# kolyangg/open-universe

Measured on AMD Instinct MI355X. Metric: sec-audio enhanced/sec/GPU + xRT, UNIVERSE++ 16 kHz 8 s clips @1/2/4/8 GPU, higher is better.
Workload: dtype f32 (conv operands split into f16 hi/lo: 3 f16 MFMA passes, f32 accumulation)

## Files before the change

### include/ouhip.h

```cpp
#ifndef OUHIP_H
#define OUHIP_H

#include <stddef.h>
#include <stdint.h>

#ifdef __cplusplus
extern "C" {
#endif

#define OUHIP_ABI_VERSION 10

int ou_abi_version(void);
const char* ou_last_error(void);


#define OU_TILE_SHAPE_MASK 0xff
#define OU_TILE_TPW_SHIFT 8
#define OU_TILE_TPW_MASK (3 << 8)
#define OU_TILE_WS (1 << 10)
#define OU_TILE_SPLIT_QUERY (1 << 11)
#define OU_TILE_KS_SHIFT 12
#define OU_TILE_KS_MASK (3 << 12)
#define OU_TILE_RS (1 << 14)
#define OU_TILE_SS (1 << 15)
#define OU_TILE_MMAJOR (1 << 16)
#define OU_TILE_FIR (1 << 17)
#define OU_TILE_FIR_EARLY (1 << 8)
#define OU_TILE_FIR_DEEP (1 << 9)
#define OU_TILE_RS_DIAG_SHIFT 8
#define OU_TILE_RS_DIAG_MASK (3 << 8)

typedef struct ou_conv_desc {
    const float* x;
    int64_t x_bstride;
    int64_t x_cstride;
    int32_t cin;
    int32_t in_len;
    int32_t frame;
    int32_t shift;
    const float* in_scale;
    float slope;
    const float* w;
    int32_t m;
    int32_t kt;
    int32_t pad;
    int32_t cc;
    int32_t n_frames;
    int32_t batch;
    float* y;
    int64_t y_bstride, y_cstride;
    int32_t rout;
    int32_t out_len;
    int32_t valid_len;
    const float* bias;
    const float* res1;
    int64_t r1_bstride, r1_cstride;
    float s1;
    const float* film;
    int64_t film_bstride;
    const float* res2;
    int64_t r2_bstride, r2_cstride;
    float s2;
    int32_t tile;
    int32_t prec;
    float w_unscale;
    int32_t f0;
    int32_t* status;
    float* ks_ws;
    int64_t ks_ws_bytes;
    uint16_t* sy;
    int64_t sy_bstride;
    int32_t sy_rows;
    int32_t sy_shift;
    float sy_slope;
    int32_t sy_pad_;
    const uint16_t* xs;
    int64_t xs_bstride;
    int32_t xs_rows;
    int32_t xs_shift;
    int32_t fir;
    int32_t fir_pad_;
    const float* fir_taps;
} ou_conv_desc;

int ou_conv_chunk(int kt, int frame);
int64_t ou_conv_packed_size(int m, int cin_eff, int kt, int cc);
int ou_conv_pack(const float* w_logical, int m, int cin_eff, int kt, int cc,
                 float* packed);
int ou_conv_pack_split(const float* w_logical, int m, int cin_eff, int kt,
                       float* packed, float* w_unscale);
int ou_conv_pack_split_nat(const float* w_logical, int m, int cin_eff, int kt,
                           float* packed, float* w_unscale);
int ou_conv(const ou_conv_desc* d, void* stream);
int ou_conv_pick_tile(const ou_conv_desc* d);
int ou_conv_num_tiles(void);
int ou_conv_tile_ok(int kt, int tile);
int ou_conv_lds_info(int kt, int tile, int* lds_request, int* device_optin_max);

typedef struct ou_gru_desc {
    const float* gi;
    int64_t gi_bstride;
    const float* w_hh;
    const float* b_hh;
    float* y;
    int64_t y_bstride, y_cstride;
    const float* res;
    int64_t res_bstride, res_cstride;
    float res_scale;
    int32_t hidden;
    int32_t steps;
    int32_t batch;
    int32_t flags;
    uint64_t* granules;
    int32_t* status;
    int32_t t_begin, t_end;
    float* hstate;
    int32_t ws_zeroed;
    int32_t _pad;
} ou_gru_desc;

int64_t ou_gru_workspace_bytes(int hidden, int batch);
int ou_gru_ks_max_workgroups(void);
int ou_gru(const ou_gru_desc* d, void* stream);

typedef struct ou_embed_desc {
    const float* sigma;
    int32_t n;
    int32_t kind;
    int32_t dim;
    float te_weight, te_bias;
    const float* rff_freq;
    int32_t n_rff;
    int32_t rows;
    const float* mlp_w[3];
    const float* mlp_b[3];
    float mlp_slope[3];
    const float* w;
    const float* bias;
    float* out;
    float* gbuf;
} ou_embed_desc;

int ou_embed(const ou_embed_desc* d, void* stream);

typedef struct ou_head_desc {
    const float* h;
    int64_t h_bstride;
    int32_t channels, length, batch, mode;
    float slope1, slope2;
    const float* w;
    float bias;
    int32_t edm, _pad;
    float w_skip, w_out, s2, c_score, c_noise, s_next;
    const float* x;
    const float* z;
    float* out;
} ou_head_desc;

int ou_head(const ou_head_desc* d, void* stream);

int ou_normalize(const float* x, float* y, int batch, int64_t n, float level,
                 float eps, void* stream);
int ou_inv_rms(const float* x, float* out, int batch, int64_t n, float denom,
               float eps, void* stream);
int ou_rms(const float* x, float* out, int batch, int64_t n, void* stream);
int ou_power(const float* x, float* y, int batch, int nf, int frames, void* stream);
int ou_pad(const float* x, int64_t x_bstride, float* y, int batch, int n_in,
           int n_out, int left, void* stream);
int ou_scale(const float* z, float* y, int64_t n, float scale, const float* add,
             void* stream);
int ou_finish(const float* x, int64_t x_bstride, int left, float* y, int batch,
              int len, const float* mix_rms, void* stream);
int ou_ensemble_reduce(const float* x, float* y, int ensemble, int64_t n,
                       int mode , void* stream);
int ou_signal_median(const float* x, float* y, int ensemble, int batch, int64_t n, int* counts,
                     void* stream);

int ou_resample(const float* x, int64_t x_bstride, float* y, int64_t y_bstride, int batch, int n_in,
                int n_out, const float* kernel, int phases, int taps, int orig, int width, void* stream);

int ou_flac_info(const uint8_t* data, int64_t n, int32_t* sample_rate, int32_t* channels,
                 int32_t* bits_per_sample, int64_t* frames);
int64_t ou_flac_decode(const uint8_t* data, int64_t n, float* out, int64_t frames);
int64_t ou_flac_encode_bound(int channels, int64_t frames, int bps);
int64_t ou_flac_encode(const float* x, int channels, int64_t frames, int sample_rate, int bps, uint8_t* out,
                       int64_t capacity);

typedef struct ou_snake_desc {
    const float* h;
    int64_t h_bstride;
    int32_t channels, length, batch, _pad0;
    const float* alpha;
    const float* k_up;
    int32_t taps_up, width_up;
    const float* k_down;
    int32_t taps_down, width_down;
    float* out;
} ou_snake_desc;

int ou_snake_aa(const ou_snake_desc* d, void* stream);

typedef struct ou_block_desc {
    const float* h;
    int64_t h_bstride, h_cstride;
    int32_t channels, length;
    int32_t batch, prec;
    const void* w[3];
    const float* bias[3];
    float slope[3];
    float w_unscale[3];
    const float* sc;
    int64_t sc_bstride, sc_cstride;
    float s_sc;
    int32_t dbg;
    const float* film;
    int64_t film_bstride;
    float* cond_out;
    int64_t co_bstride, co_cstride;
    float* y;
    int64_t y_bstride, y_cstride;
    float s_res, s2;
    const float* res2;
    int64_t r2_bstride, r2_cstride;
    int32_t* status;
    const float* x;
    int64_t x_bstride;
    const float* in_scale;
    const float* w_in;
    const float* b_in;
    ou_head_desc head;
    const void* w_down;
    const float* b_down;
    float slope_down, w_down_unscale;
    int32_t rate, down_kt;
    float* e;
    int64_t e_bstride, e_cstride;
    int32_t f0, f1;
    int32_t h0, h1;
    int32_t shift[4];
    uint16_t* sy;
    int64_t sy_bstride;
    int32_t sy_rows, sy_shift;
    float sy_slope;
    int32_t sy_pad_;
    const uint16_t* xs;
    int64_t xs_bstride;
    int32_t xs_rows, xs_pad_;
} ou_block_desc;

int ou_block_supported(int channels, int prec);
int ou_block_frames(int channels);
int64_t ou_block_packed_halves(int channels, int kt);
int ou_block_pack(const float* w, int channels, int kt, void* out, float* w_unscale);
int ou_block_pack_rect(const float* w, int m, int channels, int kt, void* out, float* w_unscale);
int64_t ou_block_packed_f32(int channels, int kt);
int ou_block_pack_f32(const float* w, int channels, int kt, float* out, float* w_unscale);
int ou_block_down_supported(int channels, int rate, int kt, int prec);
int ou_block(const ou_block_desc* d, void* stream);

typedef struct ou_program ou_program;

enum {
    OU_OP_CONV = 1, OU_OP_GRU = 2, OU_OP_EMBED = 3, OU_OP_HEAD = 4,
    OU_OP_NORMALIZE = 5, OU_OP_INV_RMS = 6, OU_OP_POWER = 7, OU_OP_PAD = 8,
    OU_OP_SCALE = 9, OU_OP_FINISH = 10, OU_OP_RMS = 11, OU_OP_SNAKE = 12,
    OU_OP_MEMSET = 13, OU_OP_ENSEMBLE = 14, OU_OP_BLOCK = 15,
    OU_OP_LANE = 16, OU_OP_SIGNAL = 17, OU_OP_WAIT = 18
};

typedef struct ou_memset_desc {
    void* ptr;
    int64_t bytes;
} ou_memset_desc;
typedef struct ou_norm_args {
    const float* x;
    float* y;
    int32_t batch, _pad;
    int64_t n;
    float level, eps;
} ou_norm_args;
typedef struct ou_rms_args {
    const float* x;
    float* out;
    int32_t batch, _pad;
    int64_t n;
    float denom, eps;
} ou_rms_args;
typedef struct ou_power_args {
    const float* x;
    float* y;
    int32_t batch, nf, frames, _pad;
} ou_power_args;
typedef struct ou_pad_args {
    const float* x;
    int64_t x_bstride;
    float* y;
    int32_t batch, n_in, n_out, left;
} ou_pad_args;
typedef struct ou_scale_args {
    const float* z;
    float* y;
    int64_t n;
    float scale, _pad;
    const float* add;
} ou_scale_args;
typedef struct ou_finish_args {
    const float* x;
    int64_t x_bstride;
    int32_t left, batch, len, _pad;
    float* y;
    const float* mix_rms;
} ou_finish_args;
typedef struct ou_sync_args {
    int32_t id;
    int32_t _pad;
} ou_sync_args;
typedef struct ou_ensemble_args {
    const float* x;
    float* y;
    int32_t ensemble, mode;
    int64_t n;
    int32_t batch, _pad;
    int32_t* counts;
} ou_ensemble_args;

ou_program* ou_program_create(void);
void ou_program_destroy(ou_program* p);
int ou_program_add(ou_program* p, int op, const void* desc, size_t desc_bytes);
int ou_program_patch(ou_program* p, int index, int op, const void* desc, size_t desc_bytes);
int ou_program_size(const ou_program* p);
int ou_program_run(ou_program* p, void* stream);
int ou_program_capture(ou_program* p);
int ou_program_validate(const ou_program* p);
int ou_program_capture_segments(ou_program* p);
int ou_program_launch(ou_program* p, void* stream);
int ou_program_op_kind(const ou_program* p, int i);
int ou_program_profile(ou_program* p, void* stream, float* ms);
int ou_program_trace(ou_program* p, void* stream, float* t0, float* t1);

int ou_randn(float* out, int64_t n, uint64_t seed, uint64_t offset, void* stream);
int ou_philox4x32(const uint32_t ctr[4], const uint32_t key[2], uint32_t out[4]);

typedef struct ou_bundle ou_bundle;
typedef struct ou_model ou_model;

typedef struct ou_bundle_io {
    int32_t region;
    int32_t count;
    int64_t offset;
    int32_t batch;
    int32_t length;
} ou_bundle_io;

typedef struct ou_bundle_meta {
    ou_bundle_io mix;
    ou_bundle_io noise;
    ou_bundle_io out;
    ou_bundle_io status;
    int32_t n_regions, n_ops;
    int64_t region_bytes;
    const char* json;
    int64_t json_bytes;
    char arch[16];
} ou_bundle_meta;

int ou_bundle_open(const char* path, ou_bundle** out);
void ou_bundle_close(ou_bundle* b);
int ou_bundle_info(const ou_bundle* b, ou_bundle_meta* meta);
int ou_bundle_region(const ou_bundle* b, int i, int32_t* kind, int64_t* bytes, const void** data);
int ou_bundle_op(const ou_bundle* b, int i, int32_t* kind, int64_t* desc_bytes, const char** label);
int ou_bundle_materialize(const ou_bundle* b, const uint64_t* region_bases, int op, void* desc_out);

int ou_bundle_load(const char* path, int capture, ou_model** out);
int ou_model_enhance_noise(ou_model* m, const float* mix, const float* noise, float* out, void* stream);
int ou_model_enhance(ou_model* m, const float* mix, float* out, uint64_t seed, uint64_t offset, void* stream);
int ou_model_status(ou_model* m);
int ou_model_info(const ou_model* m, ou_bundle_meta* meta);
void ou_model_destroy(ou_model* m);

int ou_long_windows(int64_t T, int window, int overlap, int64_t* n, int64_t* last_start);
int ou_long_fade(int overlap, float* fade );
int ou_window_gather(const float* x, int64_t x_rstride, int rows, int64_t T, int window, int overlap,
                     int64_t first, int count, int64_t win, float* y, int64_t y_rstride, int64_t y_bstride,
                     void* stream);
int ou_overlap_add(const float* w, int64_t w_bstride, int64_t T, int window, int overlap, int64_t first,
                   int count, const float* fade, float* y, void* stream);

typedef struct ou_pool_clip {
    const float* x;
    const float* noise;
    float* y;
    int64_t T, noise_rstride;
} ou_pool_clip;
int ou_pool_slots(const int64_t* T, int n_clips, int window, int overlap, int64_t* n_slots);
int ou_pool_gather(const ou_pool_clip* clips, int n_clips, int window, int overlap, int64_t first, int count,
                   int noise_rows, int64_t noise_win, float* mix, int64_t mix_bstride,
                   float* nz, int64_t nz_rstride, int64_t nz_bstride, void* stream);
int ou_pool_overlap_add(const ou_pool_clip* clips, int n_clips, int window, int overlap, int64_t first, int count,
                        const float* w, int64_t w_bstride, const float* fade, void* stream);

int64_t ou_model_long_noise(const ou_model* m, int64_t n, int overlap, int64_t* len);
int ou_model_enhance_long_noise(ou_model* m, const float* x, int64_t n, int overlap, const float* noise,
                                float* out, void* stream);
int ou_model_enhance_long(ou_model* m, const float* x, int64_t n, int overlap, float* out, uint64_t seed,
                          uint64_t offset, float* workspace, void* stream);

#ifdef __cplusplus
}
#endif
#endif
```

### open_universe_amd/_lib.py

```python
import ctypes
import os
from ctypes import POINTER, c_char, c_char_p, c_float, c_int, c_int32, c_int64, c_size_t, c_uint32, c_uint64, c_void_p

_HERE = os.path.dirname(os.path.abspath(__file__))
LIB_PATH = os.environ.get("OUHIP_LIB", os.path.join(_HERE, "libouhip.so"))
ABI_VERSION = 10

fp = c_void_p

OP_CONV, OP_GRU, OP_EMBED, OP_HEAD = 1, 2, 3, 4
OP_NORMALIZE, OP_INV_RMS, OP_POWER, OP_PAD = 5, 6, 7, 8
OP_SCALE, OP_FINISH, OP_RMS, OP_SNAKE = 9, 10, 11, 12
OP_MEMSET, OP_ENSEMBLE, OP_BLOCK = 13, 14, 15
OP_LANE, OP_SIGNAL, OP_WAIT = 16, 17, 18


class ConvDesc(ctypes.Structure):
    _fields_ = [
        ("x", fp), ("x_bstride", c_int64), ("x_cstride", c_int64),
        ("cin", c_int32), ("in_len", c_int32), ("frame", c_int32), ("shift", c_int32),
        ("in_scale", fp), ("slope", c_float), ("w", fp),
        ("m", c_int32), ("kt", c_int32), ("pad", c_int32), ("cc", c_int32),
        ("n_frames", c_int32), ("batch", c_int32),
        ("y", fp), ("y_bstride", c_int64), ("y_cstride", c_int64),
        ("rout", c_int32), ("out_len", c_int32), ("valid_len", c_int32),
        ("bias", fp),
        ("res1", fp), ("r1_bstride", c_int64), ("r1_cstride", c_int64), ("s1", c_float),
        ("film", fp), ("film_bstride", c_int64),
        ("res2", fp), ("r2_bstride", c_int64), ("r2_cstride", c_int64), ("s2", c_float),
        ("tile", c_int32), ("prec", c_int32), ("w_unscale", c_float), ("f0", c_int32),
        ("status", fp), ("ks_ws", fp), ("ks_ws_bytes", c_int64),
        ("sy", fp), ("sy_bstride", c_int64), ("sy_rows", c_int32), ("sy_shift", c_int32),
        ("sy_slope", c_float), ("sy_pad_", c_int32),
        ("xs", fp), ("xs_bstride", c_int64), ("xs_rows", c_int32), ("xs_shift", c_int32),
        ("fir", c_int32), ("fir_pad_", c_int32), ("fir_taps", fp),
    ]


class GruDesc(ctypes.Structure):
    _fields_ = [
        ("gi", fp), ("gi_bstride", c_int64), ("w_hh", fp), ("b_hh", fp),
        ("y", fp), ("y_bstride", c_int64), ("y_cstride", c_int64),
        ("res", fp), ("res_bstride", c_int64), ("res_cstride", c_int64),
        ("res_scale", c_float), ("hidden", c_int32), ("steps", c_int32), ("batch", c_int32),
        ("flags", c_int32), ("granules", fp), ("status", fp), ("t_begin", c_int32), ("t_end", c_int32),
        ("hstate", fp), ("ws_zeroed", c_int32), ("_pad", c_int32),
    ]


class EmbedDesc(ctypes.Structure):
    _fields_ = [
        ("sigma", fp), ("n", c_int32), ("kind", c_int32), ("dim", c_int32),
        ("te_weight", c_float), ("te_bias", c_float), ("rff_freq", fp), ("n_rff", c_int32),
        ("rows", c_int32), ("mlp_w", fp * 3), ("mlp_b", fp * 3), ("mlp_slope", c_float * 3),
        ("w", fp), ("bias", fp), ("out", fp), ("gbuf", fp),
    ]


class HeadDesc(ctypes.Structure):
    _fields_ = [
        ("h", fp), ("h_bstride", c_int64),
        ("channels", c_int32), ("length", c_int32), ("batch", c_int32), ("mode", c_int32),
        ("slope1", c_float), ("slope2", c_float), ("w", fp), ("bias", c_float),
        ("edm", c_int32), ("_pad", c_int32),
        ("w_skip", c_float), ("w_out", c_float), ("s2", c_float), ("c_score", c_float),
        ("c_noise", c_float), ("s_next", c_float),
        ("x", fp), ("z", fp), ("out", fp),
    ]


class SnakeDesc(ctypes.Structure):
    _fields_ = [
        ("h", fp), ("h_bstride", c_int64),
        ("channels", c_int32), ("length", c_int32), ("batch", c_int32), ("_pad0", c_int32),
        ("alpha", fp), ("k_up", fp), ("taps_up", c_int32), ("width_up", c_int32),
        ("k_down", fp), ("taps_down", c_int32), ("width_down", c_int32), ("out", fp),
    ]


class SyncArgs(ctypes.Structure):
    _fields_ = [("id", c_int32), ("_pad", c_int32)]


class MemsetArgs(ctypes.Structure):
    _fields_ = [("ptr", fp), ("bytes", c_int64)]


class NormArgs(ctypes.Structure):
    _fields_ = [("x", fp), ("y", fp), ("batch", c_int32), ("_pad", c_int32), ("n", c_int64),
                ("level", c_float), ("eps", c_float)]


class RmsArgs(ctypes.Structure):
    _fields_ = [("x", fp), ("out", fp), ("batch", c_int32), ("_pad", c_int32), ("n", c_int64),
                ("denom", c_float), ("eps", c_float)]


class PowerArgs(ctypes.Structure):
    _fields_ = [("x", fp), ("y", fp), ("batch", c_int32), ("nf", c_int32),
                ("frames", c_int32), ("_pad", c_int32)]


class PadArgs(ctypes.Structure):
    _fields_ = [("x", fp), ("x_bstride", c_int64), ("y", fp), ("batch", c_int32),
                ("n_in", c_int32), ("n_out", c_int32), ("left", c_int32)]


class ScaleArgs(ctypes.Structure):
    _fields_ = [("z", fp), ("y", fp), ("n", c_int64), ("scale", c_float), ("_pad", c_float),
                ("add", fp)]


class FinishArgs(ctypes.Structure):
    _fields_ = [("x", fp), ("x_bstride", c_int64), ("left", c_int32), ("batch", c_int32),
                ("len", c_int32), ("_pad", c_int32), ("y", fp), ("mix_rms", fp)]


class EnsembleArgs(ctypes.Structure):
    _fields_ = [("x", fp), ("y", fp), ("ensemble", c_int32), ("mode", c_int32), ("n", c_int64),
                ("batch", c_int32), ("_pad", c_int32), ("counts", c_void_p)]


class BlockDesc(ctypes.Structure):
    _fields_ = [
        ("h", fp), ("h_bstride", c_int64), ("h_cstride", c_int64),
        ("channels", c_int32), ("length", c_int32), ("batch", c_int32), ("prec", c_int32),
        ("w", fp * 3), ("bias", fp * 3), ("slope", c_float * 3), ("w_unscale", c_float * 3),
        ("sc", fp), ("sc_bstride", c_int64), ("sc_cstride", c_int64), ("s_sc", c_float), ("dbg", c_int32),
        ("film", fp), ("film_bstride", c_int64),
        ("cond_out", fp), ("co_bstride", c_int64), ("co_cstride", c_int64),
        ("y", fp), ("y_bstride", c_int64), ("y_cstride", c_int64), ("s_res", c_float), ("s2", c_float),
        ("res2", fp), ("r2_bstride", c_int64), ("r2_cstride", c_int64),
        ("status", fp),
        ("x", fp), ("x_bstride", c_int64), ("in_scale", fp), ("w_in", fp), ("b_in", fp),
        ("head", HeadDesc),
        ("w_down", fp), ("b_down", fp), ("slope_down", c_float), ("w_down_unscale", c_float),
        ("rate", c_int32), ("down_kt", c_int32), ("e", fp), ("e_bstride", c_int64), ("e_cstride", c_int64),
        ("f0", c_int32), ("f1", c_int32), ("h0", c_int32), ("h1", c_int32),
        ("shift", c_int32 * 4),
        ("sy", fp), ("sy_bstride", c_int64), ("sy_rows", c_int32), ("sy_shift", c_int32),
        ("sy_slope", c_float), ("sy_pad_", c_int32),
        ("xs", fp), ("xs_bstride", c_int64), ("xs_rows", c_int32), ("xs_pad_", c_int32),
    ]


class BundleIo(ctypes.Structure):
    _fields_ = [("region", c_int32), ("count", c_int32), ("offset", c_int64),
                ("batch", c_int32), ("length", c_int32)]


class BundleMeta(ctypes.Structure):
    _fields_ = [("mix", BundleIo), ("noise", BundleIo), ("out", BundleIo), ("status", BundleIo),
                ("n_regions", c_int32), ("n_ops", c_int32), ("region_bytes", c_int64),
                ("json", c_char_p), ("json_bytes", c_int64), ("arch", c_char * 16)]


class PoolClip(ctypes.Structure):
    _fields_ = [("x", fp), ("noise", fp), ("y", fp), ("T", c_int64), ("noise_rstride", c_int64)]


OP_STRUCT = {
    OP_CONV: ConvDesc, OP_GRU: GruDesc, OP_EMBED: EmbedDesc, OP_HEAD: HeadDesc,
    OP_NORMALIZE: NormArgs, OP_INV_RMS: RmsArgs, OP_RMS: RmsArgs, OP_POWER: PowerArgs,
    OP_PAD: PadArgs, OP_SCALE: ScaleArgs, OP_FINISH: FinishArgs, OP_SNAKE: SnakeDesc,
    OP_MEMSET: MemsetArgs, OP_ENSEMBLE: EnsembleArgs, OP_BLOCK: BlockDesc,
    OP_LANE: SyncArgs, OP_SIGNAL: SyncArgs, OP_WAIT: SyncArgs,
}

EXPORTS = {
    "ou_abi_version": (c_int, []),
    "ou_last_error": (ctypes.c_char_p, []),
    "ou_conv_chunk": (c_int, [c_int, c_int]),
    "ou_conv_packed_size": (c_int64, [c_int, c_int, c_int, c_int]),
    "ou_conv_pack": (c_int, [POINTER(c_float), c_int, c_int, c_int, c_int, POINTER(c_float)]),
    "ou_conv_pack_split": (c_int, [POINTER(c_float), c_int, c_int, c_int, POINTER(c_float),
                                   POINTER(c_float)]),
    "ou_conv_pack_split_nat": (c_int, [POINTER(c_float), c_int, c_int, c_int, POINTER(c_float),
                                       POINTER(c_float)]),
    "ou_conv": (c_int, [POINTER(ConvDesc), c_void_p]),
    "ou_conv_pick_tile": (c_int, [POINTER(ConvDesc)]),
    "ou_conv_num_tiles": (c_int, []),
    "ou_conv_tile_ok": (c_int, [c_int, c_int]),
    "ou_conv_lds_info": (c_int, [c_int, c_int, POINTER(c_int), POINTER(c_int)]),
    "ou_gru_workspace_bytes": (c_int64, [c_int, c_int]),
    "ou_gru_ks_max_workgroups": (c_int, []),
    "ou_gru": (c_int, [POINTER(GruDesc), c_void_p]),
    "ou_embed": (c_int, [POINTER(EmbedDesc), c_void_p]),
    "ou_head": (c_int, [POINTER(HeadDesc), c_void_p]),
    "ou_normalize": (c_int, [fp, fp, c_int, c_int64, c_float, c_float, c_void_p]),
    "ou_inv_rms": (c_int, [fp, fp, c_int, c_int64, c_float, c_float, c_void_p]),
    "ou_rms": (c_int, [fp, fp, c_int, c_int64, c_void_p]),
    "ou_power": (c_int, [fp, fp, c_int, c_int, c_int, c_void_p]),
    "ou_pad": (c_int, [fp, c_int64, fp, c_int, c_int, c_int, c_int, c_void_p]),
    "ou_scale": (c_int, [fp, fp, c_int64, c_float, fp, c_void_p]),
    "ou_finish": (c_int, [fp, c_int64, c_int, fp, c_int, c_int, fp, c_void_p]),
    "ou_ensemble_reduce": (c_int, [fp, fp, c_int, c_int64, c_int, c_void_p]),
    "ou_signal_median": (c_int, [fp, fp, c_int, c_int, c_int64, c_void_p, c_void_p]),
    "ou_snake_aa": (c_int, [POINTER(SnakeDesc), c_void_p]),
    "ou_block_supported": (c_int, [c_int, c_int]),
    "ou_block_frames": (c_int, [c_int]),
    "ou_block_packed_halves": (c_int64, [c_int, c_int]),
    "ou_block_pack": (c_int, [POINTER(c_float), c_int, c_int, c_void_p, POINTER(c_float)]),
    "ou_block_packed_f32": (c_int64, [c_int, c_int]),
    "ou_block_pack_f32": (c_int, [POINTER(c_float), c_int, c_int, POINTER(c_float), POINTER(c_float)]),
    "ou_block_pack_rect": (c_int, [POINTER(c_float), c_int, c_int, c_int, c_void_p, POINTER(c_float)]),
    "ou_block_down_supported": (c_int, [c_int, c_int, c_int, c_int]),
    "ou_block": (c_int, [POINTER(BlockDesc), c_void_p]),
    "ou_resample": (c_int, [fp, c_int64, fp, c_int64, c_int, c_int, c_int, fp, c_int, c_int, c_int, c_int,
                            c_void_p]),
    "ou_flac_info": (c_int, [c_void_p, c_int64, POINTER(c_int32), POINTER(c_int32), POINTER(c_int32),
                             POINTER(c_int64)]),
    "ou_flac_decode": (c_int64, [c_void_p, c_int64, c_void_p, c_int64]),
    "ou_flac_encode_bound": (c_int64, [c_int, c_int64, c_int]),
    "ou_flac_encode": (c_int64, [c_void_p, c_int, c_int64, c_int, c_int, c_void_p, c_int64]),
    "ou_program_create": (c_void_p, []),
    "ou_program_destroy": (None, [c_void_p]),
    "ou_program_add": (c_int, [c_void_p, c_int, c_void_p, c_size_t]),
    "ou_program_patch": (c_int, [c_void_p, c_int, c_int, c_void_p, c_size_t]),
    "ou_program_size": (c_int, [c_void_p]),
    "ou_program_run": (c_int, [c_void_p, c_void_p]),
    "ou_program_capture": (c_int, [c_void_p]),
    "ou_program_capture_segments": (c_int, [c_void_p]),
    "ou_program_validate": (c_int, [c_void_p]),
    "ou_program_launch": (c_int, [c_void_p, c_void_p]),
    "ou_program_op_kind": (c_int, [c_void_p, c_int]),
    "ou_program_profile": (c_int, [c_void_p, c_void_p, POINTER(c_float)]),
    "ou_program_trace": (c_int, [c_void_p, c_void_p, POINTER(c_float), POINTER(c_float)]),
    "ou_randn": (c_int, [fp, c_int64, c_uint64, c_uint64, c_void_p]),
    "ou_philox4x32": (c_int, [POINTER(c_uint32), POINTER(c_uint32), POINTER(c_uint32)]),
    "ou_bundle_open": (c_int, [c_char_p, POINTER(c_void_p)]),
    "ou_bundle_close": (None, [c_void_p]),
    "ou_bundle_info": (c_int, [c_void_p, POINTER(BundleMeta)]),
    "ou_bundle_region": (c_int, [c_void_p, c_int, POINTER(c_int32), POINTER(c_int64), POINTER(c_void_p)]),
    "ou_bundle_op": (c_int, [c_void_p, c_int, POINTER(c_int32), POINTER(c_int64), POINTER(c_char_p)]),
    "ou_bundle_materialize": (c_int, [c_void_p, POINTER(c_uint64), c_int, c_void_p]),
    "ou_bundle_load": (c_int, [c_char_p, c_int, POINTER(c_void_p)]),
    "ou_model_enhance_noise": (c_int, [c_void_p, fp, fp, fp, c_void_p]),
    "ou_model_enhance": (c_int, [c_void_p, fp, fp, c_uint64, c_uint64, c_void_p]),
    "ou_model_status": (c_int, [c_void_p]),
    "ou_model_info": (c_int, [c_void_p, POINTER(BundleMeta)]),
    "ou_model_destroy": (None, [c_void_p]),
    "ou_long_windows": (c_int, [c_int64, c_int, c_int, POINTER(c_int64), POINTER(c_int64)]),
    "ou_long_fade": (c_int, [c_int, POINTER(c_float)]),
    "ou_window_gather": (c_int, [fp, c_int64, c_int, c_int64, c_int, c_int, c_int64, c_int, c_int64, fp, c_int64,
                                 c_int64, c_void_p]),
    "ou_overlap_add": (c_int, [fp, c_int64, c_int64, c_int, c_int, c_int64, c_int, fp, fp, c_void_p]),
    "ou_pool_slots": (c_int, [POINTER(c_int64), c_int, c_int, c_int, POINTER(c_int64)]),
    "ou_pool_gather": (c_int, [POINTER(PoolClip), c_int, c_int, c_int, c_int64, c_int, c_int, c_int64, fp, c_int64,
                               fp, c_int64, c_int64, c_void_p]),
    "ou_pool_overlap_add": (c_int, [POINTER(PoolClip), c_int, c_int, c_int, c_int64, c_int, fp, c_int64, fp,
                                    c_void_p]),
    "ou_model_long_noise": (c_int64, [c_void_p, c_int64, c_int, POINTER(c_int64)]),
    "ou_model_enhance_long_noise": (c_int, [c_void_p, fp, c_int64, c_int, fp, fp, c_void_p]),
    "ou_model_enhance_long": (c_int, [c_void_p, fp, c_int64, c_int, fp, c_uint64, c_uint64, fp, c_void_p]),
}

_lib = None


class OuHipError(RuntimeError):
    pass


class OuRangeError(OuHipError):
    flags = ()


def load():
    global _lib
    if _lib is not None:
        return _lib
    if not os.path.exists(LIB_PATH):
        raise OuHipError(
            f"{LIB_PATH} not found: build it with `python -c 'import __graft_entry__ as g; "
            "g.build()'` or open_universe_amd/csrc/build.sh")
    lib = ctypes.CDLL(LIB_PATH)
    for name, (res, args) in EXPORTS.items():
        f = getattr(lib, name)
        f.restype = res
        f.argtypes = args
    if lib.ou_abi_version() != ABI_VERSION:
        raise OuHipError("libouhip ABI version mismatch")
    _lib = lib
    return lib


def check(rc, what=""):
    if rc != 0:
        msg = load().ou_last_error()
        raise OuHipError(f"{what}: ouhip error {rc}: {msg.decode() if msg else ''}")


def conv_chunk(kt, frame):
    return load().ou_conv_chunk(kt, frame)


def conv_pack(w_logical, cc):
    import numpy as np

    w = np.ascontiguousarray(w_logical, dtype=np.float32)
    m, cin, kt = w.shape
    n = load().ou_conv_packed_size(m, cin, kt, cc)
    out = np.empty(n, dtype=np.float32)
    check(load().ou_conv_pack(w.ctypes.data_as(POINTER(c_float)), m, cin, kt, cc,
                              out.ctypes.data_as(POINTER(c_float))), "conv_pack")
    return out


def _split_scale(w):
    import numpy as np

    if not np.isfinite(w).all():
        raise OuHipError("split packing: non-finite weight")
    mx = float(np.abs(w).max()) if w.size else 0.0
    e = 0
    if mx > 0.0:
        e = min(100, max(-100, 10 - int(np.frexp(np.float32(mx))[1])))
    return np.float32(2.0**e), float(2.0 ** (6 - e))


def _hi_lo(a):
    import numpy as np

    hi = a.astype(np.float16)
    lo = ((a - hi.astype(np.float32)) * np.float32(2048.0)).astype(np.float16)
    return hi, lo


def conv_pack_split_np(w_logical):
    import numpy as np

    w = np.ascontiguousarray(w_logical, dtype=np.float32)
    m, cin, kt = w.shape
    sc, unscale = _split_scale(w)
    mt = (m + 31) // 32
    cpad = (cin + 63) // 64 * 64
    a = np.zeros((mt * 32, cpad, kt), dtype=np.float32)
    a[:m, :cin] = w * sc
    a = a.reshape(mt, 32, cpad // 16, 8, 2, kt).transpose(0, 2, 5, 4, 1, 3)
    hi, lo = _hi_lo(np.ascontiguousarray(a))
    out = np.stack([hi, lo], axis=2)
    return np.ascontiguousarray(out).reshape(-1).view(np.float32), unscale


def conv_pack_split_nat_np(w_logical):
    import numpy as np

    w = np.ascontiguousarray(w_logical, dtype=np.float32)
    m, cin, kt = w.shape
    sc, unscale = _split_scale(w)
    mt = (m + 31) // 32
    cpad = (cin + 63) // 64 * 64
    a = np.zeros((mt * 32, cpad, kt), dtype=np.float32)
    a[:m, :cin] = w * sc
    a = a.reshape(mt, 32, cpad // 16, 2, 8, kt).transpose(0, 2, 5, 3, 1, 4)
    hi, lo = _hi_lo(np.ascontiguousarray(a))
    out = np.stack([hi, lo], axis=2)
    return np.ascontiguousarray(out).reshape(-1).view(np.float32), unscale


def block_pack_np(w_logical):
    import numpy as np

    w = np.ascontiguousarray(w_logical, dtype=np.float32)
    m, c, kt = w.shape
    assert m % 32 == 0 and c % 16 == 0, w.shape
    sc, unscale = _split_scale(w)
    a = (w * sc).reshape(m // 32, 32, c // 16, 2, 8, kt).transpose(0, 5, 2, 3, 1, 4)
    hi, lo = _hi_lo(np.ascontiguousarray(a))
    out = np.stack([hi, lo], axis=3)
    return np.ascontiguousarray(out).reshape(-1).view(np.int16), unscale


def block_pack_f32_np(w_logical):
    import numpy as np

    w = np.ascontiguousarray(w_logical, dtype=np.float32)
    m, c, kt = w.shape
    assert m % 32 == 0 and c % 16 == 0, w.shape
    a = w.reshape(m // 32, 32, c // 8, 4, 2, kt).transpose(0, 5, 2, 4, 1, 3)
    return np.ascontiguousarray(a).reshape(-1), 64.0


def block_pack_f32(w_logical):
    import numpy as np

    w = np.ascontiguousarray(w_logical, dtype=np.float32)
    c, _, kt = w.shape
    out = np.empty(load().ou_block_packed_f32(c, kt), dtype=np.float32)
    un = c_float(0.0)
    check(load().ou_block_pack_f32(w.ctypes.data_as(POINTER(c_float)), c, kt, out.ctypes.data_as(POINTER(c_float)),
                                   ctypes.byref(un)), "block_pack_f32")
    return out, float(un.value)


def conv_pack_split(w_logical, natural=False):
    import numpy as np

    w = np.ascontiguousarray(w_logical, dtype=np.float32)
    m, cin, kt = w.shape
    n = load().ou_conv_packed_size(m, cin, kt, 0)
    out = np.empty(n, dtype=np.float32)
    un = c_float(0.0)
    fn = load().ou_conv_pack_split_nat if natural else load().ou_conv_pack_split
    check(fn(w.ctypes.data_as(POINTER(c_float)), m, cin, kt, out.ctypes.data_as(POINTER(c_float)),
             ctypes.byref(un)), "conv_pack_split")
    return out, float(un.value)


def block_pack(w_logical):
    import numpy as np

    w = np.ascontiguousarray(w_logical, dtype=np.float32)
    m, c, kt = w.shape
    out = np.empty(2 * m * c * kt, dtype=np.int16)
    un = c_float(0.0)
    check(load().ou_block_pack_rect(w.ctypes.data_as(POINTER(c_float)), m, c, kt, out.ctypes.data,
                                    ctypes.byref(un)), "block_pack")
    return out, float(un.value)


TILE_SHAPE_MASK = 0xff
TILE_TPW_SHIFT, TILE_TPW_MASK = 8, 3 << 8
TILE_WS = 1 << 10
TILE_SPLIT_QUERY = 1 << 11
TILE_KS_SHIFT, TILE_KS_MASK = 12, 3 << 12
TILE_RS = 1 << 14
TILE_SS = 1 << 15
TILE_MMAJOR = 1 << 16
TILE_FIR = 1 << 17
TILE_FIR_EARLY = 1 << 8
TILE_FIR_DEEP = 1 << 9
TILE_RS_DIAG_SHIFT, TILE_RS_DIAG_MASK = 8, 3 << 8
MAJ_BIT, SS_BIT, FIR_BIT = TILE_MMAJOR, TILE_SS, TILE_FIR

_MMAJOR = os.environ.get("OUHIP_MMAJOR", "1") != "0"
_MMAJOR_BYTES = float(os.environ.get("OUHIP_MMAJOR_MB", "128")) * 2**20


def mmajor_order(desc):
    multi = desc.tile & (TILE_TPW_MASK | TILE_WS) and not desc.tile & TILE_FIR
    if not _MMAJOR or multi:
        return False
    in_bytes = 4.0 * desc.batch * desc.cin * desc.frame * desc.n_frames
    return in_bytes > _MMAJOR_BYTES


TUNER = None


ADD_HOOK = None


class Program:

    def __init__(self):
        self.lib = load()
        self.h = self.lib.ou_program_create()
        self.keep = []
        self.cur_lane = 0
        self.captured = False
        self.flops = []
        self.bytes = []
        self.info = []
        self.lanes = []
        self.label = ""
        self.labels = []
        self.descs = []

    def add(self, op, desc):
        assert isinstance(desc, OP_STRUCT[op])
        if op == OP_LANE:
            self.cur_lane = desc.id
        if op in (OP_CONV, OP_BLOCK) and ADD_HOOK is not None:
            ADD_HOOK(self, op, desc)
        if op == OP_CONV and desc.tile < 0 and TUNER is not None:
            desc.tile = TUNER(desc)
        if op == OP_CONV and desc.tile >= 0 and mmajor_order(desc):
            desc.tile |= TILE_MMAJOR
        check(self.lib.ou_program_add(self.h, op, ctypes.byref(desc), ctypes.sizeof(desc)),
              f"program_add(op={op})")
        if ADD_HOOK is not None and hasattr(ADD_HOOK, "note"):
            ADD_HOOK.note(self, len(self.flops), op, desc)
        self.descs.append(desc)
        self.flops.append(float(getattr(desc, "_flops", 0.0)))
        self.bytes.append(float(getattr(desc, "_bytes", 0.0)))
        self.lanes.append(self.cur_lane)
        self.labels.append(self.label)
        if op == OP_CONV:
            self.info.append({"m": desc.m, "cin": desc.cin, "frame": desc.frame, "kt": desc.kt,
                              "n": desc.n_frames, "b": desc.batch, "rout": desc.rout,
                              "tile": desc.tile, "fir": desc.fir})
        elif op == OP_GRU:
            self.info.append({"H": desc.hidden, "T": desc.steps, "b": desc.batch})
        elif op == OP_BLOCK:
            self.info.append({"C": desc.channels, "n": desc.length, "b": desc.batch, "prec": desc.prec,
                              "rate": desc.rate if desc.e else 0, "head": bool(desc.head.w), "in": bool(desc.x)})
        else:
            self.info.append({})

    def lane(self, i):
        self.add(OP_LANE, SyncArgs(id=i))

    def new_event(self):
        self.n_events = getattr(self, "n_events", 0) + 1
        return self.n_events - 1

    def signal(self, ev=None):
        ev = self.new_event() if ev is None else ev
        self.add(OP_SIGNAL, SyncArgs(id=ev))
        return ev

    def wait(self, ev):
        self.add(OP_WAIT, SyncArgs(id=ev))

    def patch(self, index, op, desc):
        check(self.lib.ou_program_patch(self.h, index, op, ctypes.byref(desc), ctypes.sizeof(desc)),
              f"program_patch({index})")

    def __len__(self):
        return self.lib.ou_program_size(self.h)

    def run(self, stream):
        check(self.lib.ou_program_run(self.h, c_void_p(stream)), "program_run")

    def validate(self):
        check(self.lib.ou_program_validate(self.h), "program_validate")

    def capture(self, segments=None):
        import os

        if segments is None:
            segments = os.environ.get("OUHIP_GRAPH_MODE", "whole") == "seg"
        fn = self.lib.ou_program_capture_segments if segments else self.lib.ou_program_capture
        check(fn(self.h), "program_capture")
        self.captured = True

    def launch(self, stream):
        check(self.lib.ou_program_launch(self.h, c_void_p(stream)), "program_launch")

    def op_kinds(self):
        return [self.lib.ou_program_op_kind(self.h, i) for i in range(len(self))]

    def profile(self, stream):
        n = len(self)
        buf = (c_float * n)()
        check(self.lib.ou_program_profile(self.h, c_void_p(stream), buf), "program_profile")
        return list(buf)

    def trace(self, stream):
        n = len(self)
        a, b = (c_float * n)(), (c_float * n)()
        check(self.lib.ou_program_trace(self.h, c_void_p(stream), a, b), "program_trace")
        return [(x, y) if x >= 0 else None for x, y in zip(a, b)]

    def __del__(self):
        try:
            if self.h:
                self.lib.ou_program_destroy(self.h)
                self.h = None
        except Exception:
            pass


def run_now(op, desc, stream):
    lib = load()
    fns = {OP_CONV: lib.ou_conv, OP_GRU: lib.ou_gru, OP_EMBED: lib.ou_embed,
           OP_HEAD: lib.ou_head, OP_SNAKE: lib.ou_snake_aa, OP_BLOCK: lib.ou_block}
    check(fns[op](ctypes.byref(desc), c_void_p(stream)), f"op {op}")
```

### open_universe_amd/csrc/ou_block.hip

```cpp
#include <hip/hip_runtime.h>

#include <algorithm>
#include <cmath>
#include <type_traits>
#include <vector>

#include "../../include/ouhip.h"
#include "ou_common.h"

typedef float floatx16 __attribute__((ext_vector_type(16)));
typedef _Float16 half4_t __attribute__((ext_vector_type(4)));
typedef _Float16 half8_t __attribute__((ext_vector_type(8)));
typedef float f32x4_t __attribute__((ext_vector_type(4)));

namespace {

constexpr int kStageShift = 6;


#ifndef OU_BLOCK_NT32
#define OU_BLOCK_NT32 4
#endif
#ifndef OU_BLOCK_NT64
#define OU_BLOCK_NT64 2
#endif
#ifndef OU_BLOCK_NT128
#define OU_BLOCK_NT128 1
#endif
#ifndef OU_BLOCK_NT48
#define OU_BLOCK_NT48 4
#endif
#ifndef OU_BLOCK_NT96
#define OU_BLOCK_NT96 4
#endif
#ifndef OU_BLOCK_NT192
#define OU_BLOCK_NT192 2
#endif
#ifndef OU_BLOCK_RING1
#define OU_BLOCK_RING1 6
#endif
#ifndef OU_BLOCK_FENCE
#define OU_BLOCK_FENCE 1
#endif
#ifndef OU_BLOCK_BPIPE
#define OU_BLOCK_BPIPE 1
#endif
#ifndef OU_BLOCK_RING_EARLY
#define OU_BLOCK_RING_EARLY 0
#endif
#ifndef OU_BLOCK_HV_EARLY
#define OU_BLOCK_HV_EARLY 0
#endif

template <int C, int NT, int P>
struct BCfg {
    static constexpr int MT = (C + 31) / 32;
    static constexpr int WAVES = 4;
    static constexpr int NTH = 64 * WAVES;
    static constexpr int WM = MT % WAVES == 0 ? WAVES : MT % 2 == 0 ? 2 : 1;
    static constexpr int WN = WAVES / WM;
    static constexpr int MR = MT / WM;
    static constexpr int NR = NT / WN;
    static constexpr int NF = 32 * NT;
    static constexpr int F = NF - 4;
    using E = std::conditional_t<P == 0, float, _Float16>;
    static constexpr int SX = P == 0 ? C + 4 : C + 8;
    static constexpr int R1 = NF + 4;
    static constexpr int R2 = NF + 2;
    static constexpr int NPL = P == 1 ? 2 : 1;
    static constexpr int PA = R1 * SX;
    static constexpr int PB = R2 * SX;
    static constexpr int A_OFF = 0;
    static constexpr int B_OFF = NPL * PA;
    static constexpr int LDS_BYTES = (int)sizeof(E) * (NPL * PA + NPL * PB);
    static constexpr int KS = C / 16;
    static constexpr int RING = MR == 1 ? OU_BLOCK_RING1 : 4;
    static_assert(C % 16 == 0 && WM * WN == WAVES && MT % WM == 0 && NT % WN == 0, "block tiling");
    static_assert((SX * (int)sizeof(E) / 16) % 2 == 1 && (SX * (int)sizeof(E)) % 16 == 0,
                  "LDS row stride must be an odd number of 16-B slots");
};

__device__ __forceinline__ float prelu(float v, float a) { return v >= 0.f ? v : a * v; }

template <int KT, int C, int NT, int P>
__device__ __forceinline__ void ring_load(const half8_t* __restrict__ wp, int wm, int lane, int s,
                                          half8_t (&dst)[BCfg<C, NT, P>::MR][2])
{
    using K = BCfg<C, NT, P>;
    const int k = s / K::KS, ks = s - (s / K::KS) * K::KS;
#pragma unroll
    for (int mr = 0; mr < K::MR; ++mr) {
        const half8_t* p = wp + ((((int64_t)(wm * K::MR + mr) * KT + k) * K::KS + ks) * 2) * 64 + lane;
        dst[mr][0] = p[0];
        if constexpr (P == 1) dst[mr][1] = p[64];
    }
}
template <int KT, int C, int NT, int P>
__device__ __forceinline__ void ring_pro(const void* wp, int wm, int lane,
                                         half8_t (&ra)[BCfg<C, NT, P>::RING][BCfg<C, NT, P>::MR][2])
{
    using K = BCfg<C, NT, P>;
    constexpr int NS = KT * K::KS, D = NS < K::RING ? NS : K::RING;
#pragma unroll
    for (int s = 0; s < D - 1; ++s) ring_load<KT, C, NT, P>((const half8_t*)wp, wm, lane, s, ra[s]);
}

template <int KT, int C, int NT, int P>
__device__ __forceinline__ void stage_mma(const half8_t* __restrict__ wp, const _Float16* xin, int pstride, int wm,
                                          int wn, int lane, int dbg, floatx16 (&acc)[BCfg<C, NT, P>::MR][BCfg<C, NT, P>::NR],
                                          floatx16 (&accx)[BCfg<C, NT, P>::MR][BCfg<C, NT, P>::NR],
                                          half8_t (&ra)[BCfg<C, NT, P>::RING][BCfg<C, NT, P>::MR][2], bool pre)
{
    using K = BCfg<C, NT, P>;
    constexpr int MR = K::MR, NR = K::NR, KS = K::KS, NS = KT * KS;
    const int l32 = lane & 31, h = lane >> 5;
#pragma unroll
    for (int mr = 0; mr < MR; ++mr)
#pragma unroll
        for (int nr = 0; nr < NR; ++nr) {
#pragma unroll
            for (int r = 0; r < 16; ++r) acc[mr][nr][r] = 0.f, accx[mr][nr][r] = 0.f;
        }
    if (dbg & 2) return;
    constexpr int D = NS < K::RING ? NS : K::RING;
    auto load_a = [&](int s, half8_t (&dst)[MR][2]) { ring_load<KT, C, NT, P>(wp, wm, lane, s, dst); };
    if (!pre) {
#pragma unroll
        for (int s = 0; s < D - 1; ++s) load_a(s, ra[s]);
    }
    const _Float16* xb = xin + (wn * NR * 32 + l32) * K::SX + 8 * h;
    half8_t b[2][NR], bl[2][NR];
    auto load_b = [&](int s, half8_t (&bq)[NR], half8_t (&bo)[NR]) {
        const int k = s / KS, ks = s - (s / KS) * KS;
#pragma unroll
        for (int nr = 0; nr < NR; ++nr) {
            const _Float16* q = xb + (nr * 32 + k) * K::SX + 16 * ks;
            bq[nr] = *(const half8_t*)q;
            if constexpr (P == 1) bo[nr] = *(const half8_t*)(q + pstride);
        }
    };
    if constexpr (OU_BLOCK_BPIPE) load_b(0, b[0], bl[0]);
#pragma unroll
    for (int s = 0; s < NS; ++s) {
        if (s + D - 1 < NS) load_a(s + D - 1, ra[(s + D - 1) % D]);
        const int c = OU_BLOCK_BPIPE ? (s & 1) : 0;
        if constexpr (OU_BLOCK_BPIPE) {
            if (s + 1 < NS) load_b(s + 1, b[c ^ 1], bl[c ^ 1]);
        } else {
            load_b(s, b[0], bl[0]);
        }
        if constexpr (OU_BLOCK_FENCE) asm volatile("" ::: "memory");
#pragma unroll
        for (int mr = 0; mr < MR; ++mr)
#pragma unroll
            for (int nr = 0; nr < NR; ++nr) {
                acc[mr][nr] = __builtin_amdgcn_mfma_f32_32x32x16_f16(ra[s % D][mr][0], b[c][nr], acc[mr][nr], 0, 0, 0);
                if constexpr (P == 1) {
                    accx[mr][nr] =
                        __builtin_amdgcn_mfma_f32_32x32x16_f16(ra[s % D][mr][0], bl[c][nr], accx[mr][nr], 0, 0, 0);
                    accx[mr][nr] =
                        __builtin_amdgcn_mfma_f32_32x32x16_f16(ra[s % D][mr][1], b[c][nr], accx[mr][nr], 0, 0, 0);
                }
            }
    }
}

template <int C>
__device__ __forceinline__ int ch_pos(int c)
{
    return (c & 1) * (C / 2) + (c >> 1);
}

template <int KT, int C, int NT>
__device__ __forceinline__ void stage_mma_f32(const f32x4_t* __restrict__ wp, const float* xin, int wm, int wn,
                                              int lane, int dbg,
                                              floatx16 (&acc)[BCfg<C, NT, 0>::MR][BCfg<C, NT, 0>::NR])
{
    using K = BCfg<C, NT, 0>;
    constexpr int MR = K::MR, NR = K::NR, S4 = C / 8, NS = KT * S4;
    const int l32 = lane & 31, h = lane >> 5;
#pragma unroll
    for (int mr = 0; mr < MR; ++mr)
#pragma unroll
        for (int nr = 0; nr < NR; ++nr) {
#pragma unroll
            for (int r = 0; r < 16; ++r) acc[mr][nr][r] = 0.f;
        }
    if (dbg & 2) return;
    constexpr int D = NS < 4 ? NS : 4;
    f32x4_t ra[D][MR];
    auto load_a = [&](int s, f32x4_t (&dst)[MR]) {
        const int k = s / S4, s4 = s - (s / S4) * S4;
#pragma unroll
        for (int mr = 0; mr < MR; ++mr) dst[mr] = wp[(((int64_t)(wm * MR + mr) * KT + k) * S4 + s4) * 64 + lane];
    };
#pragma unroll
    for (int s = 0; s < D - 1; ++s) load_a(s, ra[s]);
    const float* xb = xin + (wn * NR * 32 + l32) * K::SX + h * (C / 2);
#pragma unroll
    for (int s = 0; s < NS; ++s) {
        if (s + D - 1 < NS) load_a(s + D - 1, ra[(s + D - 1) % D]);
        if constexpr (OU_BLOCK_FENCE) asm volatile("" ::: "memory");
        const int k = s / S4, s4 = s - (s / S4) * S4;
        f32x4_t bq[NR];
#pragma unroll
        for (int nr = 0; nr < NR; ++nr) bq[nr] = *(const f32x4_t*)(xb + (nr * 32 + k) * K::SX + 4 * s4);
#pragma unroll
        for (int j = 0; j < 4; ++j)
#pragma unroll
            for (int mr = 0; mr < MR; ++mr)
#pragma unroll
                for (int nr = 0; nr < NR; ++nr)
                    acc[mr][nr] = __builtin_amdgcn_mfma_f32_32x32x2f32(ra[s % D][mr][j], bq[nr][j], acc[mr][nr], 0, 0, 0);
    }
}

template <int KT, int C, int NT, int P>
__device__ __forceinline__ void run_stage(const void* w, const typename BCfg<C, NT, P>::E* xin, int pstride, int wm,
                                          int wn, int lane, int dbg,
                                          floatx16 (&acc)[BCfg<C, NT, P>::MR][BCfg<C, NT, P>::NR],
                                          floatx16 (&accx)[BCfg<C, NT, P>::MR][BCfg<C, NT, P>::NR],
                                          half8_t (&ra)[BCfg<C, NT, P>::RING][BCfg<C, NT, P>::MR][2], bool pre)
{
    if constexpr (P == 0) {
        stage_mma_f32<KT, C, NT>((const f32x4_t*)w, xin, wm, wn, lane, dbg, acc);
#pragma unroll
        for (int mr = 0; mr < BCfg<C, NT, P>::MR; ++mr)
#pragma unroll
            for (int nr = 0; nr < BCfg<C, NT, P>::NR; ++nr) accx[mr][nr] = floatx16{};
    } else {
        stage_mma<KT, C, NT, P>((const half8_t*)w, xin, pstride, wm, wn, lane, dbg, acc, accx, ra, pre);
    }
}

constexpr int kEpiFilm = 1, kEpiSc = 2, kEpiCond = 4, kEpiRes2 = 8;
constexpr int kEpiIn = 16, kEpiHead = 32;
constexpr int kEpiDown = 64;

template <int EPI, int R, int KF>
constexpr int block_off()
{
    return (EPI & kEpiHead) ? 1 : (EPI & kEpiDown) ? R * ((KF - 1) / 2) : 0;
}

template <int C, int NT, int P, int EPI, int R = 1, int KF = 1>
constexpr int block_f()
{
    if constexpr (EPI & kEpiDown) {
        constexpr int halo = 2 * R * ((KF - 1) / 2);
        return (BCfg<C, NT, P>::NF - 4 - halo) / R * R;
    }
    return BCfg<C, NT, P>::NF - 4 - ((EPI & kEpiHead) ? 2 : 0);
}

typedef float float2_t __attribute__((ext_vector_type(2)));
__device__ __forceinline__ float2_t fma2(float2_t a, float2_t b, float2_t c) { return __builtin_elementwise_fma(a, b, c); }
typedef _Float16 half2_t __attribute__((ext_vector_type(2)));

template <int P>
__device__ __forceinline__ void split4(float x0, float x1, float x2, float x3, half4_t& hi, half4_t& lo, float& omax)
{
    const float2_t a = {x0, x1}, b = {x2, x3};
    const half2_t ha = __builtin_convertvector(a, half2_t), hb = __builtin_convertvector(b, half2_t);
    hi = half4_t{ha[0], ha[1], hb[0], hb[1]};
    if constexpr (P == 1) {
        const half2_t la = __builtin_convertvector((a - __builtin_convertvector(ha, float2_t)) * 2048.f, half2_t);
        const half2_t lb = __builtin_convertvector((b - __builtin_convertvector(hb, float2_t)) * 2048.f, half2_t);
        lo = half4_t{la[0], la[1], lb[0], lb[1]};
    }
    const float m = __builtin_fmaxf(__builtin_fmaxf(__builtin_fabsf(x0), __builtin_fabsf(x1)),
                                    __builtin_fmaxf(__builtin_fabsf(x2), __builtin_fabsf(x3)));
    omax = __builtin_fmaxf(omax, m);
}

template <int C, int P, int R, int KF, int F, int SX>
__device__ __forceinline__ void down_stage(const ou_block_desc& d, const _Float16* xa, int pstride, int t0, int T,
                                           int TS, int b, int wave, int lane)
{
    constexpr int KT = KF * R, KS = C / 16, NS = KT * KS;
    constexpr int M4 = 2 * C / 32, NU = F / R, N4 = (NU + 31) / 32;
    constexpr int D = NS < 6 ? NS : 6;
    const int l32 = lane & 31, h = lane >> 5;
    const half8_t* wp = (const half8_t*)d.w_down;
    const int TE = (TS + R - 1) / R;
    const int e0 = t0 / R;
    const float un = d.w_down_unscale * ou_exp2i(d.shift[3] - kStageShift);
    for (int tile = wave; tile < M4 * N4; tile += 4) {
        const int m4 = tile % M4, n4 = tile / M4;
        const int u = n4 * 32 + l32;
        const _Float16* xb = xa + (u < NU ? u * R : 0) * SX + 8 * h;
        floatx16 acc, accx;
#pragma unroll
        for (int r = 0; r < 16; ++r) acc[r] = 0.f, accx[r] = 0.f;
        half8_t ra[D][2];
        auto load_a = [&](int s, half8_t (&dst)[2]) {
            const int k = s / KS, ks = s - (s / KS) * KS;
            const half8_t* p = wp + (((int64_t)(m4 * KT + k) * KS + ks) * 2) * 64 + lane;
            dst[0] = p[0];
            if constexpr (P == 1) dst[1] = p[64];
        };
#pragma unroll
        for (int s = 0; s < D - 1; ++s) load_a(s, ra[s]);
#pragma unroll
        for (int s = 0; s < NS; ++s) {
            if (s + D - 1 < NS) load_a(s + D - 1, ra[(s + D - 1) % D]);
            const int k = s / KS, ks = s - (s / KS) * KS;
            const _Float16* q = xb + k * SX + 16 * ks;
            const half8_t bq = *(const half8_t*)q;
            acc = __builtin_amdgcn_mfma_f32_32x32x16_f16(ra[s % D][0], bq, acc, 0, 0, 0);
            if constexpr (P == 1) {
                const half8_t bl = *(const half8_t*)(q + pstride);
                accx = __builtin_amdgcn_mfma_f32_32x32x16_f16(ra[s % D][0], bl, accx, 0, 0, 0);
                accx = __builtin_amdgcn_mfma_f32_32x32x16_f16(ra[s % D][1], bq, accx, 0, 0, 0);
            }
        }
        const int te = e0 + u;
        if (u >= NU || te >= TE) continue;
        float* eb = d.e + (int64_t)b * d.e_bstride + te;
#pragma unroll
        for (int r = 0; r < 16; ++r) {
            const int m = m4 * 32 + (r & 3) + 8 * (r >> 2) + 4 * h;
            const float bias = d.b_down ? d.b_down[m] : 0.f;
            eb[(int64_t)m * d.e_cstride] = __builtin_fmaf(__builtin_fmaf(accx[r], 1.f / 2048.f, acc[r]), un, bias);
        }
    }
}

template <int C>
constexpr int block_threads()
{
    return C > 0 ? 256 : 0;
}

template <int C>
constexpr int block_min_wgs()
{
    return (C == 96 || C == 192) ? 1 : 2;
}

constexpr int kBlkSentinel = 0x7ffffff0;

template <int C, int NT, int P, int EPI, int R = 1, int KF = 1>
__global__ __launch_bounds__(block_threads<C>(), block_min_wgs<C>()) void block_kernel(ou_block_desc d)
{
    using K = BCfg<C, NT, P>;
    ou_kernarg_prefetch8();
    constexpr int MR = K::MR, NR = K::NR, NF = K::NF, SX = K::SX;
    constexpr int OFF = block_off<EPI, R, KF>();
    constexpr int F = block_f<C, NT, P, EPI, R, KF>();
    const float kIn0 = ou_exp2i(-d.shift[0]), kIn1 = ou_exp2i(-d.shift[1]), kIn2 = ou_exp2i(-d.shift[2]),
                kInD = ou_exp2i(-d.shift[3]);
    OU_DYNAMIC_LDS(half8_t, lds8);
    using E = typename K::E;
    E* lds = (E*)lds8;
    E* xa = lds + K::A_OFF;
    E* xbuf = lds + K::B_OFF;
    const int tid = threadIdx.x, lane = tid & 63, wave = tid >> 6;
    const int wm = wave % K::WM, wn = wave / K::WM;
    const int l32 = lane & 31, h = lane >> 5;
    const int b = blockIdx.y;
    const int T = d.length;
    const int t0 = d.f0 + blockIdx.x * F;
    const int TS = d.f1 > 0 ? min(d.f1, T) : T;
    const int hlo = d.h0, hhi = d.h1 > 0 ? min(d.h1, T) : T;
    const float* __restrict__ hb = d.h + (int64_t)b * d.h_bstride;
    float om0 = 0.f, om1 = 0.f, om2 = 0.f, omd = 0.f;
    float oms = 0.f;
    constexpr bool early = OU_BLOCK_RING_EARLY && P != 0;
    half8_t ring[K::RING][MR][2];
    if constexpr (early) ring_pro<5, C, NT, P>(d.w[0], wm, lane, ring);

    const float* __restrict__ xin = (EPI & kEpiIn) ? d.x + (int64_t)b * d.x_bstride : nullptr;
    const float xsc = (EPI & kEpiIn) ? (d.in_scale ? d.in_scale[b] : 1.f) : 0.f;
    auto xs = [&](int t) { return (t >= 0 && t < T) ? xsc * xin[t] : 0.f; };
    auto in_conv = [&](int c, float xl, float xm, float xr) {
        return __builtin_fmaf(d.w_in[3 * c + 2], xr,
                              __builtin_fmaf(d.w_in[3 * c + 1], xm, __builtin_fmaf(d.w_in[3 * c], xl, d.b_in[c])));
    };

    if (P == 1 && !(EPI & kEpiIn) && d.xs) {
        constexpr int NI = (C / 8) * K::R1;
        constexpr int NIT = (NI + K::NTH - 1) / K::NTH;
        const __amdgpu_buffer_rsrc_t xrs =
            ou_rsrc((const char*)d.xs + (int64_t)b * d.xs_bstride, (int64_t)(C / 32) * d.xs_rows * 128);
        ou_u4_t vh[NIT], vl[NIT];
#pragma unroll
        for (int it = 0; it < NIT; ++it) {
            const int item = min(tid + K::NTH * it, NI - 1);
            const int g = item / K::R1, r = item - g * K::R1;
            const int t = t0 - 4 - OFF + r;
            const bool ok = t >= 0 && t < T && !(d.dbg & 1);
            const int vo = ok ? ((g >> 2) * d.xs_rows + t) * 128 + (g & 3) * 16 : kBlkSentinel;
            vh[it] = __builtin_amdgcn_raw_buffer_load_b128(xrs, vo, 0, 0);
            vl[it] = __builtin_amdgcn_raw_buffer_load_b128(xrs, vo, 64, 0);
        }
#pragma unroll
        for (int it = 0; it < NIT; ++it) {
            const int item = tid + K::NTH * it;
            if (NIT * K::NTH > NI && item >= NI) break;
            const int g = item / K::R1, r = item - g * K::R1;
            E* dst = xa + r * SX + 8 * g;
            *(ou_u4_t*)dst = vh[it];
            *(ou_u4_t*)(dst + K::PA) = vl[it];
        }
    } else {
        constexpr int NI = (C / 8) * K::R1;
        constexpr int NIT = (NI + K::NTH - 1) / K::NTH;
        const float a1 = d.slope[0];
        float v[NIT][8];
        const int hcs = (int)d.h_cstride;
        const __amdgpu_buffer_rsrc_t hrs = ou_rsrc(hb, (int64_t)C * d.h_cstride * 4);
        const int tlo = max(0, hlo), thi = min(T, hhi);
#pragma unroll
        for (int it = 0; it < NIT; ++it) {
            const int item = min(tid + K::NTH * it, NI - 1);
            const int g = item / K::R1, r = item - g * K::R1;
            const int t = t0 - 4 - OFF + r;
            if constexpr (EPI & kEpiIn) {
                const float xl = xs(t - 1), xm = xs(t), xr = xs(t + 1);
#pragma unroll
                for (int i = 0; i < 8; ++i) v[it][i] = in_conv(8 * g + i, xl, xm, xr);
                if (t < tlo || t >= thi || (d.dbg & 1)) {
#pragma unroll
                    for (int i = 0; i < 8; ++i) v[it][i] = 0.f;
                }
            } else {
                const bool ok = t >= tlo && t < thi && !(d.dbg & 1);
                const int vo = ok ? (8 * g * hcs + t) * 4 : kBlkSentinel;
#pragma unroll
                for (int i = 0; i < 8; ++i)
                    v[it][i] = __uint_as_float(__builtin_amdgcn_raw_buffer_load_b32(hrs, vo, i * hcs * 4, 0));
            }
        }
#pragma unroll
        for (int it = 0; it < NIT; ++it) {
            const int item = tid + K::NTH * it;
            if (NIT * K::NTH > NI && item >= NI) break;
            const int g = item / K::R1, r = item - g * K::R1;
            float x[8];
#pragma unroll
            for (int i = 0; i < 8; ++i) x[i] = (v[it][i] >= 0.f ? kIn0 : a1 * kIn0) * v[it][i];
            if constexpr (P == 0) {
                E* row = xa + r * SX;
                *(f32x4_t*)(row + 4 * g) = f32x4_t{x[0], x[2], x[4], x[6]};
                *(f32x4_t*)(row + C / 2 + 4 * g) = f32x4_t{x[1], x[3], x[5], x[7]};
            } else {
                half4_t h0, h1, l0, l1;
                split4<P>(x[0], x[1], x[2], x[3], h0, l0, om0);
                split4<P>(x[4], x[5], x[6], x[7], h1, l1, om0);
                E* dst = xa + r * SX + 8 * g;
                *(half8_t*)dst = half8_t{h0[0], h0[1], h0[2], h0[3], h1[0], h1[1], h1[2], h1[3]};
                if constexpr (P == 1)
                    *(half8_t*)(dst + K::PA) = half8_t{l0[0], l0[1], l0[2], l0[3], l1[0], l1[1], l1[2], l1[3]};
            }
        }
    }
    __syncthreads();

    floatx16 acc[MR][NR], accx[MR][NR];
    auto row = [&](int mr, int r) { return (wm * MR + mr) * 32 + (r & 3) + 8 * (r >> 2) + 4 * h; };
    constexpr bool PADM = C % 32 != 0;
    auto rowc = [&](int mr, int r) { return PADM ? min(row(mr, r), C - 1) : row(mr, r); };
    auto rbase = [&](int mr, int r) { return (wm * MR + mr) * 32 + (r & 3) + 8 * (r >> 2); };
    auto rok = [&](int mr, int r) { return !PADM || row(mr, r) < C; };
    auto gok = [&](int mr, int j) { return !PADM || (wm * MR + mr) * 32 + 8 * j + 4 * h < C; };
    auto put4 = [&](E* row, int c0, const float (&x)[4], int pstride, float& om) {
        if constexpr (P == 0) {
            *(float2_t*)(row + (c0 >> 1)) = float2_t{x[0], x[2]};
            *(float2_t*)(row + C / 2 + (c0 >> 1)) = float2_t{x[1], x[3]};
        } else {
            half4_t hi, lo;
            split4<P>(x[0], x[1], x[2], x[3], hi, lo, om);
            *(half4_t*)(row + c0) = hi;
            if constexpr (P == 1) *(half4_t*)(row + c0 + pstride) = lo;
        }
    };
    auto zero8 = [&](E* row, int c0, int pstride) {
        if constexpr (P == 0) {
            *(f32x4_t*)(row + (c0 >> 1)) = f32x4_t{};
            *(f32x4_t*)(row + C / 2 + (c0 >> 1)) = f32x4_t{};
        } else {
            *(half8_t*)(row + c0) = half8_t{};
            if constexpr (P == 1) *(half8_t*)(row + c0 + pstride) = half8_t{};
        }
    };

    run_stage<5, C, NT, P>(d.w[0], xa, K::PA, wm, wn, lane, d.dbg, acc, accx, ring, early);
    if (early) ring_pro<3, C, NT, P>(d.w[1], wm, lane, ring);
    {
        const float a2 = d.slope[1];
        float bia[MR][16], gam[MR][16], bet[MR][16], scv[MR][NR][16];
        const float* film = d.film + (int64_t)b * d.film_bstride;
#pragma unroll
        for (int mr = 0; mr < MR; ++mr)
#pragma unroll
            for (int r = 0; r < 16; ++r) {
                const int m = rowc(mr, r);
                bia[mr][r] = d.bias[0] ? d.bias[0][m] : 0.f;
                if constexpr (EPI & kEpiFilm) {
                    gam[mr][r] = film[m];
                    bet[mr][r] = film[C + m];
                }
                if constexpr (EPI & kEpiSc) {
#pragma unroll
                    for (int nr = 0; nr < NR; ++nr) {
                        const int t = min(max(t0 - 2 - OFF + (wn * NR + nr) * 32 + l32, 0), T - 1);
                        if constexpr (PADM) {
                            scv[mr][nr][r] = d.sc[(int64_t)b * d.sc_bstride + (int64_t)m * d.sc_cstride + t];
                        } else {
                            const int cs4 = (int)d.sc_cstride * 4;
                            scv[mr][nr][r] = __uint_as_float(__builtin_amdgcn_raw_buffer_load_b32(
                                ou_rsrc(d.sc + (int64_t)b * d.sc_bstride, (int64_t)C * cs4), t * 4 + 4 * h * cs4,
                                rbase(mr, r) * cs4, 0));
                        }
                    }
                }
            }
        const float un = d.w_unscale[0] * ou_exp2i(d.shift[0] - kStageShift);
#pragma unroll
        for (int mr = 0; mr < MR; ++mr)
#pragma unroll
            for (int nr = 0; nr < NR; ++nr) {
                const int u = (wn * NR + nr) * 32 + l32;
                const int t = t0 - 2 - OFF + u;
                const bool inside = t >= 0 && t < T;
                float o[16];
#pragma unroll
                for (int r = 0; r < 16; r += 2) {
                    float2_t v = fma2(fma2(float2_t{accx[mr][nr][r], accx[mr][nr][r + 1]}, 1.f / 2048.f,
                                           float2_t{acc[mr][nr][r], acc[mr][nr][r + 1]}),
                                      un, float2_t{bia[mr][r], bia[mr][r + 1]});
                    if constexpr (EPI & kEpiSc) v = (v + float2_t{scv[mr][nr][r], scv[mr][nr][r + 1]}) * d.s_sc;
                    if constexpr (EPI & kEpiFilm)
                        v = fma2(float2_t{gam[mr][r], gam[mr][r + 1]}, v, float2_t{bet[mr][r], bet[mr][r + 1]});
                    o[r] = inside ? v.x : 0.f, o[r + 1] = inside ? v.y : 0.f;
                }
                if constexpr (EPI & kEpiCond) {
                    const bool st = inside && t >= t0 && t < t0 + F && t < TS;
                    if constexpr (PADM) {
                        if (st) {
                            float* co = d.cond_out + (int64_t)b * d.co_bstride + t;
#pragma unroll
                            for (int r = 0; r < 16; ++r)
                                if (rok(mr, r)) co[(int64_t)row(mr, r) * d.co_cstride] = o[r];
                        }
                    } else {
                        const int cs4 = (int)d.co_cstride * 4;
                        const __amdgpu_buffer_rsrc_t crs =
                            ou_rsrc(d.cond_out + (int64_t)b * d.co_bstride, (int64_t)C * cs4);
                        const int vo = st ? t * 4 + 4 * h * cs4 : kBlkSentinel;
#pragma unroll
                        for (int r = 0; r < 16; ++r)
                            __builtin_amdgcn_raw_buffer_store_b32(__float_as_uint(o[r]), crs, vo, rbase(mr, r) * cs4, 0);
                    }
                }
#pragma unroll
                for (int j = 0; j < 4; ++j) {
                    if (!gok(mr, j)) continue;
                    float x[4];
#pragma unroll
                    for (int i = 0; i < 4; i += 2) {
                        const float2_t q = {o[4 * j + i], o[4 * j + i + 1]};
                        const float2_t xx = q * float2_t{q.x >= 0.f ? kIn1 : a2 * kIn1, q.y >= 0.f ? kIn1 : a2 * kIn1};
                        x[i] = xx.x, x[i + 1] = xx.y;
                    }
                    put4(xbuf + u * SX, (wm * MR + mr) * 32 + 8 * j + 4 * h, x, K::PB, om1);
                }
            }
        for (int e = tid; e < 2 * (C / 8); e += K::NTH) zero8(xbuf + (NF + e / (C / 8)) * SX, 8 * (e % (C / 8)), K::PB);
    }
    __syncthreads();

    run_stage<3, C, NT, P>(d.w[1], xbuf, K::PB, wm, wn, lane, d.dbg, acc, accx, ring, early);
    if (early) ring_pro<3, C, NT, P>(d.w[2], wm, lane, ring);
    {
        const float a3 = d.slope[2], un = d.w_unscale[1] * ou_exp2i(d.shift[1] - kStageShift);
        float bia[MR][16];
#pragma unroll
        for (int mr = 0; mr < MR; ++mr)
#pragma unroll
            for (int r = 0; r < 16; ++r) bia[mr][r] = d.bias[1] ? d.bias[1][rowc(mr, r)] : 0.f;
#pragma unroll
        for (int mr = 0; mr < MR; ++mr)
#pragma unroll
            for (int nr = 0; nr < NR; ++nr) {
                const int v_ = (wn * NR + nr) * 32 + l32;
                const int t = t0 - 1 - OFF + v_;
                const float keep = (t >= 0 && t < T) ? kIn2 : 0.f, akeep = a3 * keep;
#pragma unroll
                for (int j = 0; j < 4; ++j) {
                    if (!gok(mr, j)) continue;
                    float x[4];
#pragma unroll
                    for (int i = 0; i < 4; i += 2) {
                        const int r = 4 * j + i;
                        const float2_t q = fma2(fma2(float2_t{accx[mr][nr][r], accx[mr][nr][r + 1]}, 1.f / 2048.f,
                                                     float2_t{acc[mr][nr][r], acc[mr][nr][r + 1]}),
                                                un, float2_t{bia[mr][r], bia[mr][r + 1]});
                        const float2_t xx = q * float2_t{q.x >= 0.f ? keep : akeep, q.y >= 0.f ? keep : akeep};
                        x[i] = xx.x, x[i + 1] = xx.y;
                    }
                    put4(xa + v_ * SX, (wm * MR + mr) * 32 + 8 * j + 4 * h, x, K::PA, om2);
                }
            }
        for (int e = tid; e < 2 * (C / 8); e += K::NTH) zero8(xa + (NF + e / (C / 8)) * SX, 8 * (e % (C / 8)), K::PA);
    }
    __syncthreads();

    float hv[MR][NR][16], rv[MR][NR][16];
    auto load_res = [&]() {
#pragma unroll
        for (int nr = 0; nr < NR; ++nr) {
            const int w = (wn * NR + nr) * 32 + l32;
            const int t = t0 - OFF + w;
            const int tc = min(max(t, 0), T - 1);
            if constexpr (EPI & kEpiIn) {
                const float xl = xs(t - 1), xm = xs(t), xr = xs(t + 1);
#pragma unroll
                for (int mr = 0; mr < MR; ++mr)
#pragma unroll
                    for (int r = 0; r < 16; ++r) hv[mr][nr][r] = in_conv(rowc(mr, r), xl, xm, xr);
            } else {
                const bool hk = t >= hlo && t < hhi;
                if constexpr (PADM) {
#pragma unroll
                    for (int mr = 0; mr < MR; ++mr)
#pragma unroll
                        for (int r = 0; r < 16; ++r) {
                            const float v = hb[(int64_t)rowc(mr, r) * d.h_cstride + tc];
                            hv[mr][nr][r] = hk ? v : 0.f;
                        }
                } else {
                    const int cs4 = (int)d.h_cstride * 4;
                    const __amdgpu_buffer_rsrc_t rs = ou_rsrc(hb, (int64_t)C * cs4);
                    const int vo = hk ? tc * 4 + 4 * h * cs4 : kBlkSentinel;
#pragma unroll
                    for (int mr = 0; mr < MR; ++mr)
#pragma unroll
                        for (int r = 0; r < 16; ++r)
                            hv[mr][nr][r] =
                                __uint_as_float(__builtin_amdgcn_raw_buffer_load_b32(rs, vo, rbase(mr, r) * cs4, 0));
                }
            }
            if constexpr (EPI & kEpiRes2) {
                if constexpr (PADM) {
#pragma unroll
                    for (int mr = 0; mr < MR; ++mr)
#pragma unroll
                        for (int r = 0; r < 16; ++r)
                            rv[mr][nr][r] =
                                d.res2[(int64_t)b * d.r2_bstride + (int64_t)rowc(mr, r) * d.r2_cstride + tc];
                } else {
                    const int cs4 = (int)d.r2_cstride * 4;
                    const __amdgpu_buffer_rsrc_t rs = ou_rsrc(d.res2 + (int64_t)b * d.r2_bstride, (int64_t)C * cs4);
                    const int vo = tc * 4 + 4 * h * cs4;
#pragma unroll
                    for (int mr = 0; mr < MR; ++mr)
#pragma unroll
                        for (int r = 0; r < 16; ++r)
                            rv[mr][nr][r] =
                                __uint_as_float(__builtin_amdgcn_raw_buffer_load_b32(rs, vo, rbase(mr, r) * cs4, 0));
                }
            }
        }
    };
    if constexpr (OU_BLOCK_HV_EARLY && !(EPI & kEpiIn)) load_res();
    run_stage<3, C, NT, P>(d.w[2], xa, K::PA, wm, wn, lane, d.dbg, acc, accx, ring, early);
    if constexpr (!(OU_BLOCK_HV_EARLY && !(EPI & kEpiIn))) load_res();
    {
        const float un = d.w_unscale[2] * ou_exp2i(d.shift[2] - kStageShift);
        float bia[MR][16];
#pragma unroll
        for (int mr = 0; mr < MR; ++mr)
#pragma unroll
            for (int r = 0; r < 16; ++r) bia[mr][r] = d.bias[2] ? d.bias[2][rowc(mr, r)] : 0.f;
        if constexpr (EPI & kEpiHead) {
            __syncthreads();
            float* Y = (float*)xa;
            constexpr int YS = C + 1;
            const ou_head_desc& hd = d.head;
#pragma unroll
            for (int mr = 0; mr < MR; ++mr)
#pragma unroll
                for (int nr = 0; nr < NR; ++nr) {
                    const int w = (wn * NR + nr) * 32 + l32;
                    const int t = t0 - OFF + w;
                    const bool inside = t >= 0 && t < T && w < F + 2;
#pragma unroll
                    for (int r = 0; r < 16; ++r) {
                        float v = __builtin_fmaf(__builtin_fmaf(accx[mr][nr][r], 1.f / 2048.f, acc[mr][nr][r]), un,
                                                 bia[mr][r]);
                        v = (v + hv[mr][nr][r]) * d.s_res;
                        v = v >= 0.f ? v : v * hd.slope1;
                        v = v >= 0.f ? v : v * hd.slope2;
                        if (w < F + 2 && rok(mr, r)) Y[w * YS + row(mr, r)] = inside ? v : 0.f;
                    }
                }
            __syncthreads();
            for (int f = tid; f < F; f += K::NTH) {
                const int t = t0 + f;
                if (t >= TS) break;
                float net = 0.f;
                for (int c = 0; c < C; ++c)
#pragma unroll
                    for (int k = 0; k < 3; ++k) net = __builtin_fmaf(hd.w[c * 3 + k], Y[(f + k) * YS + c], net);
                net += hd.bias;
                const int64_t o = (int64_t)b * T + t;
                float out;
                if (hd.mode == 0) {
                    out = net;
                } else {
                    const float x = hd.x[o];
                    float score = net;
                    if (hd.edm) {
                        const float est = __fadd_rn(__fmul_rn(hd.w_skip, x), __fmul_rn(hd.w_out, net));
                        score = __fdiv_rn(__fsub_rn(est, x), hd.s2);
                    }
                    out = __fadd_rn(x, __fmul_rn(hd.c_score, score));
                    if (hd.mode == 1) out = __fadd_rn(out, __fmul_rn(hd.c_noise, __fmul_rn(hd.z[o], hd.s_next)));
                }
                hd.out[o] = out;
            }
        } else {
            float* yb = d.y + (int64_t)b * d.y_bstride;
            const __amdgpu_buffer_rsrc_t srs =
                ou_rsrc(d.sy ? (const char*)d.sy + (int64_t)b * d.sy_bstride : (const char*)yb,
                        d.sy ? (int64_t)(C / 32) * d.sy_rows * 128 : 0);
            const float sscale = ou_exp2i(-d.sy_shift);
            const __amdgpu_buffer_rsrc_t yrs = ou_rsrc(yb, (int64_t)C * d.y_cstride * 4);
            if constexpr (EPI & kEpiDown) __syncthreads();
            const float ad = (EPI & kEpiDown) ? d.slope_down : 0.f;
#pragma unroll
            for (int mr = 0; mr < MR; ++mr)
#pragma unroll
                for (int nr = 0; nr < NR; ++nr) {
                    const int w = (wn * NR + nr) * 32 + l32;
                    const int t = t0 - OFF + w;
                    const bool own = w >= OFF && w < OFF + F && t < TS && !((d.dbg & 4) && !(d.dbg & 1024));
                    float vv[16];
                    const int ycs4 = (int)d.y_cstride * 4;
                    const int yvo = own ? t * 4 + 4 * h * ycs4 : kBlkSentinel;
#pragma unroll
                    for (int r = 0; r < 16; r += 2) {
                        float2_t v2 = fma2(fma2(float2_t{accx[mr][nr][r], accx[mr][nr][r + 1]}, 1.f / 2048.f,
                                                float2_t{acc[mr][nr][r], acc[mr][nr][r + 1]}),
                                           un, float2_t{bia[mr][r], bia[mr][r + 1]});
                        v2 = (v2 + float2_t{hv[mr][nr][r], hv[mr][nr][r + 1]}) * d.s_res;
                        if constexpr (EPI & kEpiRes2) v2 = (v2 + float2_t{rv[mr][nr][r], rv[mr][nr][r + 1]}) * d.s2;
                        vv[r] = v2.x, vv[r + 1] = v2.y;
                    }
#pragma unroll
                    for (int r = 0; r < 16; ++r) {
                        const float v = vv[r];
                        if constexpr (PADM) {
                            if (own && rok(mr, r)) yb[(int64_t)row(mr, r) * d.y_cstride + t] = v;
                        } else {
                            __builtin_amdgcn_raw_buffer_store_b32(__float_as_uint(v), yrs, yvo, rbase(mr, r) * ycs4, 0);
                        }
                    }
                    if (P == 1 && d.sy) {
#pragma unroll
                        for (int j = 0; j < 4; ++j) {
                            const int c0 = (wm * MR + mr) * 32 + 8 * j + 4 * h;
                            const int off = own ? ((c0 >> 5) * d.sy_rows + t) * 128 + (c0 & 31) * 2 : kBlkSentinel;
                            ou_split_store4(srs, off, own, vv[4 * j], vv[4 * j + 1], vv[4 * j + 2], vv[4 * j + 3],
                                            sscale, d.sy_slope, oms);
                        }
                    }
                    if constexpr (EPI & kEpiDown) {
                        constexpr int RH = R * (KF - 1 - (KF - 1) / 2);
                        const float keep = (t >= 0 && t < T && w < F + OFF + RH) ? kInD : 0.f;
#pragma unroll
                        for (int j = 0; j < 4; ++j) {
                            float x[4];
#pragma unroll
                            for (int i = 0; i < 4; ++i) {
                                const float q = vv[4 * j + i];
                                x[i] = (q >= 0.f ? keep : ad * keep) * q;
                            }
                            half4_t hi, lo;
                            split4<P>(x[0], x[1], x[2], x[3], hi, lo, omd);
                            if (!gok(mr, j)) continue;
                            _Float16* dst = xa + w * SX + (wm * MR + mr) * 32 + 8 * j + 4 * h;
                            *(half4_t*)dst = hi;
                            if constexpr (P == 1) *(half4_t*)(dst + K::PA) = lo;
                        }
                    }
                }
            if constexpr (EPI & kEpiDown) {
                __syncthreads();
                down_stage<C, P, R, KF, F, SX>(d, xa, K::PA, t0, T, TS, b, wave, lane);
            }
        }
    }
    if constexpr (P != 0) {
        ou_range_flag(d.status, om0, 1, lane);
        ou_range_flag(d.status, om1, 2, lane);
        ou_range_flag(d.status, om2, 8, lane);
        if constexpr ((EPI & kEpiDown) != 0) ou_range_flag(d.status, omd, 16, lane);
        if (d.sy) ou_range_flag(d.status, oms, 32, lane);
    }
}

template <int C, int NT, int P, int EPI, int R = 1, int KF = 1>
int launch(const ou_block_desc& d, hipStream_t s)
{
    using K = BCfg<C, NT, P>;
    static bool attr = false;
    if (!attr) {
        OU_HIP_CHECK(hipFuncSetAttribute((const void*)block_kernel<C, NT, P, EPI, R, KF>,
                                         hipFuncAttributeMaxDynamicSharedMemorySize, K::LDS_BYTES),
                     "block: LDS attribute");
        attr = true;
    }
    constexpr int F = block_f<C, NT, P, EPI, R, KF>();
    static_assert(F > 0 && F % R == 0, "block: frames per workgroup");
    const int f1 = d.f1 > 0 ? min(d.f1, d.length) : d.length;
    if (d.f0 < 0 || d.f0 >= f1 || d.f0 % R || (R > 1 && f1 % R && f1 != d.length))
        return ou_fail(-1, "block: frame range [%d, %d) (rate %d, length %d)", d.f0, f1, R, d.length);
    dim3 grid((f1 - d.f0 + F - 1) / F, d.batch);
    hipLaunchKernelGGL((block_kernel<C, NT, P, EPI, R, KF>), grid, dim3(K::NTH), K::LDS_BYTES, s, d);
    return ou_check_launch("block");
}

constexpr bool down_ok(int C, int rate, int kt)
{
    return (C == 32 && rate == 2 && (kt == 3 || kt == 1)) || (C == 64 && rate == 4 && kt == 1);
}

template <int C, int NT, int P, int EPI>
int launch_down(const ou_block_desc& d, hipStream_t s)
{
    if constexpr (C == 32) {
        if (d.rate == 2 && d.down_kt == 3) return launch<C, NT, P, EPI, 2, 3>(d, s);
        if (d.rate == 2 && d.down_kt == 1) return launch<C, NT, P, EPI, 2, 1>(d, s);
    } else if constexpr (C == 64) {
        if (d.rate == 4 && d.down_kt == 1) return launch<C, NT, P, EPI, 4, 1>(d, s);
    }
    return ou_fail(-1, "block: no fused rate-change conv for %d channels, rate %d, kt %d", C, d.rate, d.down_kt);
}

template <int C, int NT, int P>
int launch_epi(const ou_block_desc& d, hipStream_t s)
{
    const int epi = (d.film ? kEpiFilm : 0) | (d.sc ? kEpiSc : 0) | (d.cond_out ? kEpiCond : 0) |
                    (d.res2 ? kEpiRes2 : 0) | (d.x ? kEpiIn : 0) | (d.head.w ? kEpiHead : 0) |
                    (d.w_down ? kEpiDown : 0);
    if constexpr ((C == 32 || C == 64) && P != 0) {
        switch (epi) {
        case kEpiDown: return launch_down<C, NT, P, kEpiDown>(d, s);
        case kEpiFilm | kEpiDown: return launch_down<C, NT, P, kEpiFilm | kEpiDown>(d, s);
        }
        if constexpr (C == 32)
            if (epi == (kEpiFilm | kEpiIn | kEpiDown)) return launch_down<C, NT, P, kEpiFilm | kEpiIn | kEpiDown>(d, s);
    }
    switch (epi) {
    case 0: return launch<C, NT, P, 0>(d, s);
    case kEpiFilm: return launch<C, NT, P, kEpiFilm>(d, s);
    case kEpiFilm | kEpiSc: return launch<C, NT, P, kEpiFilm | kEpiSc>(d, s);
    case kEpiCond: return launch<C, NT, P, kEpiCond>(d, s);
    case kEpiRes2: return launch<C, NT, P, kEpiRes2>(d, s);
    }
    if constexpr (C == 32 || C == 48) {
        switch (epi) {
        case kEpiFilm | kEpiIn: return launch<C, NT, P, kEpiFilm | kEpiIn>(d, s);
        case kEpiFilm | kEpiSc | kEpiHead: return launch<C, NT, P, kEpiFilm | kEpiSc | kEpiHead>(d, s);
        case kEpiIn: return launch<C, NT, P, kEpiIn>(d, s);
        case kEpiHead: return launch<C, NT, P, kEpiHead>(d, s);
        }
    }
    return ou_fail(-1, "block: unsupported epilogue combination %d at %d channels", epi, C);
}

template <int C>
constexpr int nt_for()
{
    return C == 32 ? OU_BLOCK_NT32 : C == 64 ? OU_BLOCK_NT64 : C == 128 ? OU_BLOCK_NT128
         : C == 48 ? OU_BLOCK_NT48 : C == 96 ? OU_BLOCK_NT96 : C == 192 ? OU_BLOCK_NT192 : 1;
}

template <int P>
int launch_p(const ou_block_desc& d, hipStream_t s)
{
    switch (d.channels) {
    case 32: return launch_epi<32, nt_for<32>(), P>(d, s);
    case 64: return launch_epi<64, nt_for<64>(), P>(d, s);
    case 128: return launch_epi<128, nt_for<128>(), P>(d, s);
    case 48: return launch_epi<48, nt_for<48>(), P>(d, s);
    case 96: return launch_epi<96, nt_for<96>(), P>(d, s);
    case 192: return launch_epi<192, nt_for<192>(), P>(d, s);
    case 256: return launch_epi<256, 1, P>(d, s);
    }
    return ou_fail(-1, "block: unsupported channel count %d", d.channels);
}

}

extern "C" int ou_block_supported(int channels, int prec)
{
    return (prec == 0 || prec == 1 || prec == 2) &&
           (channels == 32 || channels == 64 || channels == 128 || channels == 48 || channels == 96 ||
            channels == 192);
}

extern "C" int ou_block_down_supported(int channels, int rate, int kt, int prec)
{
    return prec != 0 && ou_block_supported(channels, prec) && down_ok(channels, rate, kt);
}

extern "C" int ou_block_frames(int channels)
{
    switch (channels) {
    case 32: return BCfg<32, nt_for<32>(), 1>::F;
    case 64: return BCfg<64, nt_for<64>(), 1>::F;
    case 128: return BCfg<128, nt_for<128>(), 1>::F;
    case 48: return BCfg<48, nt_for<48>(), 1>::F;
    case 96: return BCfg<96, nt_for<96>(), 1>::F;
    case 192: return BCfg<192, nt_for<192>(), 1>::F;
    case 256: return BCfg<256, 1, 1>::F;
    }
    return 0;
}

extern "C" int64_t ou_block_packed_halves(int channels, int kt)
{
    return (int64_t)(channels + 31) / 32 * 32 * channels * kt * 2;
}

extern "C" int ou_block_pack(const float* w, int channels, int kt, void* out, float* w_unscale)
{
    if (channels % 32 == 0 || !w || channels <= 0 || kt <= 0)
        return ou_block_pack_rect(w, channels, channels, kt, out, w_unscale);
    const int m = (channels + 31) / 32 * 32;
    std::vector<float> wp((size_t)m * channels * kt, 0.f);
    std::copy(w, w + (size_t)channels * channels * kt, wp.begin());
    return ou_block_pack_rect(wp.data(), m, channels, kt, out, w_unscale);
}

extern "C" int ou_block_pack_rect(const float* w, int m, int channels, int kt, void* out, float* w_unscale)
{
    if (!w || !out || !w_unscale || m <= 0 || m % 32 || channels <= 0 || channels % 16 || kt <= 0)
        return ou_fail(-1, "block_pack: bad arguments");
    const int C = channels, KS = C / 16, MT = m / 32;
    const int64_t n = (int64_t)m * C * kt;
    float mx = 0.f;
    for (int64_t i = 0; i < n; ++i) {
        if (!std::isfinite(w[i])) return ou_fail(-1, "block_pack: non-finite weight at %lld", (long long)i);
        mx = std::fmax(mx, std::fabs(w[i]));
    }
    int e = 0;
    if (mx > 0.f) {
        int ex = 0;
        std::frexp(mx, &ex);
        e = std::min(100, std::max(-100, 10 - ex));
    }
    const float sc = std::ldexp(1.f, e);
    _Float16* o = (_Float16*)out;
    for (int mt = 0; mt < MT; ++mt)
        for (int k = 0; k < kt; ++k)
            for (int ks = 0; ks < KS; ++ks)
                for (int plane = 0; plane < 2; ++plane)
                    for (int lane = 0; lane < 64; ++lane)
                        for (int i = 0; i < 8; ++i) {
                            const int row = mt * 32 + (lane & 31);
                            const int c = ks * 16 + 8 * (lane >> 5) + i;
                            const float a = w[((int64_t)row * C + c) * kt + k] * sc;
                            const _Float16 hi = (_Float16)a;
                            *o++ = plane == 0 ? hi : (_Float16)((a - (float)hi) * 2048.f);
                        }
    *w_unscale = std::ldexp(1.f, kStageShift - e);
    return 0;
}

extern "C" int64_t ou_block_packed_f32(int channels, int kt)
{
    return (int64_t)(channels + 31) / 32 * 32 * channels * kt;
}

extern "C" int ou_block_pack_f32(const float* w, int channels, int kt, float* out, float* w_unscale)
{
    if (!w || !out || !w_unscale || channels <= 0 || channels % 16 || kt <= 0)
        return ou_fail(-1, "block_pack_f32: bad arguments");
    const int C = channels, MT = (C + 31) / 32, S4 = C / 8;
    for (int mt = 0; mt < MT; ++mt)
        for (int k = 0; k < kt; ++k)
            for (int s4 = 0; s4 < S4; ++s4)
                for (int lane = 0; lane < 64; ++lane)
                    for (int j = 0; j < 4; ++j) {
                        const int row = mt * 32 + (lane & 31);
                        const int c = 2 * (4 * s4 + j) + (lane >> 5);
                        *out++ = row < C ? w[((int64_t)row * C + c) * kt + k] : 0.f;
                    }
    *w_unscale = (float)(1 << kStageShift);
    return 0;
}

extern "C" int ou_block(const ou_block_desc* dp, void* stream)
{
    if (!dp) return ou_fail(-1, "block: null descriptor");
    const ou_block_desc& d = *dp;
    if (!d.h || !d.y || !d.w[0] || !d.w[1] || !d.w[2] || d.length <= 0 || d.batch <= 0 || d.batch > 65535)
        return ou_fail(-1, "block: invalid descriptor");
    if (!ou_block_supported(d.channels, d.prec))
        return ou_fail(-1, "block: channels %d / prec %d not supported", d.channels, d.prec);
    const int64_t lim = kBlkSentinel;
    if ((int64_t)d.channels * d.h_cstride * 4 >= lim || (int64_t)d.channels * d.y_cstride * 4 >= lim ||
        (d.res2 && (int64_t)d.channels * d.r2_cstride * 4 >= lim) ||
        (d.sc && (int64_t)d.channels * d.sc_cstride * 4 >= lim) ||
        (d.cond_out && (int64_t)d.channels * d.co_cstride * 4 >= lim) ||
        (d.e && (int64_t)2 * d.channels * d.e_cstride * 4 >= lim))
        return ou_fail(-1, "block: a per-item tensor of %d x %lld floats exceeds the 32-bit buffer range", d.channels,
                       (long long)d.h_cstride);
    if (d.sy && (d.prec != 1 || d.channels % 32 || d.head.w || d.sy_rows < d.length || d.sy_shift < -100 ||
                 d.sy_shift > 100 || (int64_t)(d.channels / 32) * d.sy_rows * 128 >= lim))
        return ou_fail(-1, "block: a split-image output needs prec 1, channels %% 32 == 0, no head, sy_rows >= length");
    if (d.xs && (d.prec != 1 || d.channels % 32 || d.x || d.f0 || d.f1 || d.h0 || d.h1 || d.xs_rows < d.length ||
                 (int64_t)(d.channels / 32) * d.xs_rows * 128 >= lim))
        return ou_fail(-1, "block: a split-image input needs prec 1, channels %% 32 == 0, the whole signal, no input "
                           "conv, xs_rows >= length");
    hipStream_t s = (hipStream_t)stream;
    return d.prec == 1 ? launch_p<1>(d, s) : d.prec == 2 ? launch_p<2>(d, s) : launch_p<0>(d, s);
}
```

### open_universe_amd/engine.py

```python
import ctypes
import os
import math
from dataclasses import dataclass, field
from typing import List, Optional

import numpy as np
import torch

from . import _lib as L
from . import dsp

NF2 = np.float32(1.0 / math.sqrt(2.0))

_PREC_NAMES = {"f32": 0, "fp32": 0, "0": 0, "split": 1, "split16": 1, "1": 1, "f16": 2, "fp16": 2, "2": 2}


def default_conv_prec():
    import os

    v = os.environ.get("OUHIP_CONV_PREC", "split").strip().lower()
    if v not in _PREC_NAMES:
        raise ValueError(f"OUHIP_CONV_PREC={v!r}: expected f32, split or f16")
    return _PREC_NAMES[v]


_PREP_PREC = None
_PREP_STATUS = 0
_PREP_ENGINE = None
RANGE_SLOTS = 1024
MAX_SHIFT = 40
_PREP_KSWS = (0, 0)
KSWS_BYTES = 64 << 20

_REC = None
_LANE = 0
_SLOT = 0
MAX_LANES = 4
MAX_SLOTS = 2


def set_lane(prog, i):
    global _LANE
    assert 0 <= i < MAX_LANES
    prog.lane(i)
    _LANE = i


SC_LANE = 2


def overlap_enabled():
    import os

    return os.environ.get("OUHIP_OVERLAP", "1") != "0"


def split_images_enabled():
    import os

    return os.environ.get("OUHIP_SPLIT_IMAGES", "1") != "0"


_REC_DEVICE = None

FIR_RATES = (2, 3, 4, 5, 8)
RS_BIT, FIR_BIT, FIR_EARLY, FIR_DEEP = L.TILE_RS, L.TILE_FIR, L.TILE_FIR_EARLY, L.TILE_FIR_DEEP


def fir_mode():
    v = os.environ.get("OUHIP_FIR", "auto").strip().lower()
    if v not in ("auto", "0", "1"):
        raise ValueError(f"OUHIP_FIR={v!r}: expected auto, 0 or 1")
    return v


def fir_enabled():
    return fir_mode() != "0"


def begin_record(prec, device=None):
    global _REC, _REC_DEVICE
    _REC = {"prec": prec}
    _REC_DEVICE = device
    L.ADD_HOOK = split_hook if prec == 1 and split_images_enabled() else None



def end_record():
    global _REC
    _REC = None
    L.ADD_HOOK = None


SPLIT_SHIFT = 6


def _split_consumer(op, d):
    if op == L.OP_CONV:
        wn = getattr(d, "_w_nat", None)
        if wn is None or getattr(d, "_no_split", False) or d.prec != 1 or d.xs or d.in_scale or d.f0 or d.cin % 32:
            return None
        return (d.x, d.x_bstride, d.x_cstride, d.in_len, d.cin, d.slope, d.xs_shift, ("c", getattr(d, "_cw", None), 0))
    fw = getattr(d, "_fw", None)
    if (fw is None or d.prec != 1 or d.xs or d.x or d.f0 or d.f1 or d.h0 or d.h1 or d.channels % 32):
        return None
    return (d.h, d.h_bstride, d.h_cstride, d.length, d.channels, d.slope[0], d.shift[0], ("f", fw, 0))


def _split_producer(op, p):
    if op == L.OP_CONV:
        if p.prec != 1 or p.rout != 1 or p.m % 32 or p.sy or p.f0:
            return None
        return (p.y, p.y_bstride, p.y_cstride, p.out_len, p.m, p.batch)
    if (p.prec != 1 or p.head.w or p.sy or p.channels % 32 or p.f0 or p.f1):
        return None
    return (p.y, p.y_bstride, p.y_cstride, p.length, p.channels, p.batch)


SPLIT_STORE_BPMS = 4e9


def _split_ms(d, per_item, rows, shift, batch):
    tuner = L.TUNER
    if not hasattr(tuner, "pick"):
        return None
    trial = L.ConvDesc.from_buffer_copy(d)
    trial.xs, trial.xs_bstride, trial.xs_rows, trial.xs_shift = d.x, per_item, rows, shift
    trial.w, trial.w_unscale = d._w_nat
    trial.tile = -1
    _, ms_s = tuner.pick(trial)
    return None if ms_s is None else ms_s + batch * per_item / SPLIT_STORE_BPMS


def _split_pays(d, per_item, rows, shift, batch):
    tuner = L.TUNER
    if not hasattr(tuner, "pick"):
        return True
    plain = L.ConvDesc.from_buffer_copy(d)
    plain.tile = -1
    _, ms_p = tuner.pick(plain)
    ms_s = _split_ms(d, per_item, rows, shift, batch)
    if ms_p is None or ms_s is None:
        return True
    return ms_s < ms_p


def _split_note(prog, idx, op, d):
    from .hazards import footprint, overlap

    writers = prog.__dict__.setdefault("split_writers", {})
    if op in (L.OP_LANE, L.OP_SIGNAL, L.OP_WAIT):
        return
    W = footprint(op, d)[1]
    for k in [k for k, (_, _, _, box) in writers.items() if any(overlap(w, box) for w in W)]:
        del writers[k]
    if op in (L.OP_CONV, L.OP_BLOCK) and _split_producer(op, d) is not None:
        y = [w for w in W if w.base == d.y]
        if y:
            writers[d.y] = (idx, op, d, y[0])


def _split_link(prog, op, d):
    cons = _split_consumer(op, d)
    pv = prog.__dict__.get("split_writers", {}).get(d.x if op == L.OP_CONV else d.h)
    if cons is None or pv is None:
        return None
    idx, pop, p, _ = pv
    prod = _split_producer(pop, p)
    x, xb, xc, in_len, C, slope, shift, owner = cons
    if (p is d or prod is None or prod[0] != x or prod[1] != xb or prod[2] != xc or prod[3] < in_len
            or prod[4] != C or prod[5] < d.batch):
        return None
    rows, batch = prod[3], prod[5]
    return idx, pop, p, rows, batch, (C // 32) * rows * 128, cons


def split_hook(prog, op, d):
    link = _split_link(prog, op, d)
    if link is None:
        return
    idx, pop, p, rows, batch, per_item, cons = link
    x, xb, xc, in_len, C, slope, shift, owner = cons
    if op == L.OP_CONV and not _split_pays(d, per_item, rows, shift, batch):
        return
    key = (x, xb, xc, rows, C, batch)
    cache = prog.__dict__.setdefault("split_bufs", {})
    buf = cache.get(key)
    if buf is None:
        buf = cache[key] = empty((batch * per_item // 2,), dtype=torch.int16, device=_REC_DEVICE)
        prog.keep.append(buf)
    prog.__dict__.setdefault("split_links", []).append((idx, len(prog.flops)))
    if p.status and owner[1] is not None:
        prog.__dict__.setdefault("split_consumers", {})[p.status] = owner
    p.sy, p.sy_bstride, p.sy_rows, p.sy_shift, p.sy_slope = buf.data_ptr(), per_item, rows, shift, slope
    prog.patch(idx, pop, p)
    d.xs, d.xs_bstride, d.xs_rows = p.sy, per_item, rows
    if op == L.OP_CONV:
        d.xs_shift = shift
        d.w, d.w_unscale = d._w_nat
        if d.tile >= 0 and not d.tile & L.TILE_SS:
            d.tile = -1


split_hook.note = _split_note


def _np(t):
    return t.detach().to("cpu", torch.float32).numpy()


def fold_weight(sd, prefix):
    if prefix + ".weight_g" in sd:
        g = sd[prefix + ".weight_g"].detach().to("cpu", torch.float32)
        v = sd[prefix + ".weight_v"].detach().to("cpu", torch.float32)
        n = v.reshape(v.shape[0], -1).norm(dim=1).reshape((-1,) + (1,) * (v.dim() - 1))
        return (v * (g / n)).numpy()
    return _np(sd[prefix + ".weight"])


@dataclass
class ConvW:
    m: int
    cin: int
    kt: int
    frame: int
    pad: int
    rout: int
    slope: float
    cc: int
    w: torch.Tensor
    bias: Optional[torch.Tensor]
    shift: int = 0
    ref_macs: float = 0.0
    prec: int = 0
    w_unscale: float = 1.0
    status: int = 0
    ks_ws: tuple = (0, 0)
    cm: bool = False
    w_nat: Optional[torch.Tensor] = None
    w_unscale_nat: float = 1.0
    xshift: int = 6
    fir: Optional["FirW"] = None

    @property
    def cout(self):
        return self.m // self.rout


@dataclass
class FirW:
    mode: int
    rate: int
    w: torch.Tensor
    unscale: float
    taps: torch.Tensor


@dataclass
class ConvSpec:
    w: np.ndarray
    cin: int
    frame: int
    pad: int
    rout: int
    slope: float
    bias: Optional[np.ndarray]
    shift: int = 0
    ref_macs: float = 0.0
    cm: bool = False
    fir: Optional[tuple] = None


def make_conv(spec, device, prec=None):
    if prec is None:
        prec = _PREP_PREC if _PREP_PREC is not None else default_conv_prec()
    w_logical = np.ascontiguousarray(spec.w, dtype=np.float32)
    m, cin_eff, kt = w_logical.shape
    assert cin_eff == spec.cin * spec.frame, (cin_eff, spec.cin, spec.frame)
    if spec.frame > 1:
        w_logical = np.ascontiguousarray(
            w_logical.reshape(m, spec.cin, spec.frame, kt).transpose(0, 2, 1, 3).reshape(m, cin_eff, kt))
    cc = L.conv_chunk(kt, spec.frame)
    if prec in (1, 2):
        packed_np, unscale = L.conv_pack_split_np(w_logical)
    else:
        packed_np, unscale = L.conv_pack(w_logical, cc), 1.0
    packed = torch.from_numpy(packed_np).to(device)
    b = None if spec.bias is None else torch.from_numpy(np.ascontiguousarray(spec.bias, np.float32)).to(device)
    w_nat, unscale_nat = None, 1.0
    if prec == 1 and spec.cin % 32 == 0 and kt in (1, 3, 5) and split_images_enabled():
        nat_np, unscale_nat = L.conv_pack_split_nat_np(w_logical)
        w_nat = torch.from_numpy(nat_np).to(device)
    fir = None
    if spec.fir is not None and prec in (1, 2) and fir_enabled():
        mode, rate, wf, taps = spec.fir
        fp_np, fun = L.conv_pack_split_nat_np(np.ascontiguousarray(wf, np.float32)[:, :, None])
        fir = FirW(int(mode), int(rate), torch.from_numpy(fp_np).to(device), float(fun),
                   torch.from_numpy(np.ascontiguousarray(taps, np.float32)).to(device))
    cw = ConvW(m, spec.cin, kt, spec.frame, spec.pad, spec.rout, float(spec.slope), cc, packed, b,
               spec.shift, spec.ref_macs, int(prec), float(unscale), _PREP_STATUS if prec else 0,
               _PREP_KSWS, cm=bool(spec.cm), w_nat=w_nat, w_unscale_nat=float(unscale_nat), fir=fir)
    if prec:
        cw.status = _range_slot(cw) or cw.status
    return cw


def _range_slot(owner):
    eng = _PREP_ENGINE
    if eng is None or len(eng.range_owners) >= RANGE_SLOTS:
        return 0
    eng.range_owners.append(owner)
    return eng.status.data_ptr() + 4 * (3 + len(eng.range_owners))


def _slope(sd, p):
    return float(sd[p + ".prelu.weight"].reshape(-1)[0])


def _bias(sd, key):
    b = sd.get(key)
    return None if b is None else _np(b)


def spec_same(sd, p, k):
    w = fold_weight(sd, p + ".conv")
    return ConvSpec(w, w.shape[1], 1, (k - 1) // 2, 1, _slope(sd, p), _bias(sd, p + ".conv.bias"),
                    ref_macs=float(w.size))


def spec_plain(sd, p, k, slope=1.0):
    w = fold_weight(sd, p)
    return ConvSpec(w, w.shape[1], 1, (k - 1) // 2, 1, slope, _bias(sd, p + ".bias"),
                    ref_macs=float(w.size))


def fir_chunk(mode, r):
    return r if mode == 1 else (8 if r % 8 == 0 else 4)


def fir_k_order(w, mode, r):
    cout, cin, _ = w.shape
    R = fir_chunk(mode, r)
    return w.reshape(cout, cin // 16, 16, r // R, R).transpose(0, 1, 3, 2, 4).reshape(cout, cin * r)


def spec_down(sd, p, r, antialias):
    w = fold_weight(sd, p + ".conv")
    cout, cin, _ = w.shape
    if antialias:
        fir = dsp.binomial_taps(2 * r + 1).astype(np.float64)
        wf = np.zeros((cout, cin, 3 * r), dtype=np.float64)
        for kk in range(r):
            wf[:, :, kk:kk + 2 * r + 1] += w[:, :, kk:kk + 1].astype(np.float64) * fir[None, None, :]
        wl = wf.reshape(cout, cin, 3, r).transpose(0, 1, 3, 2).reshape(cout, cin * r, 3)
        fir = None
        if cin % 16 == 0 and r in FIR_RATES:
            fir = (1, r, fir_k_order(w, 1, r), dsp.binomial_taps(2 * r + 1))
        return ConvSpec(wl, cin, r, 1, 1, _slope(sd, p), _bias(sd, p + ".bias"),
                        ref_macs=float(cout * cin * r + cin * (2 * r + 1) * r), fir=fir)
    fir = None
    if cin % 16 == 0 and r % 4 == 0:
        fir = (3, r, fir_k_order(w, 3, r), np.ones(1, np.float32))
    return ConvSpec(w.reshape(cout, cin * r, 1), cin, r, 0, 1, _slope(sd, p),
                    _bias(sd, p + ".conv.bias"), ref_macs=float(cout * cin * r), fir=fir)


def spec_up(sd, p, r, antialias):
    w = fold_weight(sd, p + ".conv").astype(np.float64)
    cin, cout, _ = w.shape
    if antialias:
        fir = dsp.binomial_taps(2 * r + 1).astype(np.float64)
        wl = np.zeros((r, cout, cin, 3), dtype=np.float64)
        for ph in range(r):
            for j in range(2 * r + 1):
                s_ = ph + j - r
                d = s_ // r
                e = s_ - d * r
                wl[ph, :, :, d + 1] += fir[j] * w[:, :, e].T
        cm = r >= 2
        if cm:
            wl = wl.transpose(1, 0, 2, 3)
        fir = None
        if cin % 32 == 0 and r in FIR_RATES and cm:
            P = 32 // r
            wu = np.zeros((-(-cout // P) * 32, cin), dtype=np.float64)
            co = np.arange(cout)
            for ph in range(r):
                wu[32 * (co // P) + (co % P) * r + ph] = w[:, :, ph].T
            fir = (2, r, wu, dsp.binomial_taps(2 * r + 1))
        return ConvSpec(np.ascontiguousarray(wl).reshape(r * cout, cin, 3), cin, 1, 1, r, _slope(sd, p),
                        _bias(sd, p + ".bias"), ref_macs=float(cin * cout * r + cout * (2 * r + 1) * r), cm=cm,
                        fir=fir)
    wl = w.transpose(2, 1, 0)
    cm = r >= 2
    if cm:
        wl = wl.transpose(1, 0, 2)
    return ConvSpec(np.ascontiguousarray(wl).reshape(r * cout, cin, 1), cin, 1, 0, r, _slope(sd, p),
                    _bias(sd, p + ".conv.bias"), ref_macs=float(cin * cout * r), cm=cm)


def prep_same(sd, p, k, device):
    return make_conv(spec_same(sd, p, k), device)


def prep_plain(sd, p, k, device, slope=1.0):
    return make_conv(spec_plain(sd, p, k, slope), device)


def prep_down(sd, p, r, antialias, device):
    return make_conv(spec_down(sd, p, r, antialias), device)


def prep_strided(sd, p, r, device):
    return make_conv(spec_down(sd, p, r, False), device)


def prep_up(sd, p, r, antialias, device):
    return make_conv(spec_up(sd, p, r, antialias), device)


@dataclass
class FusedW:
    w: torch.Tensor
    offs: tuple
    unscale: tuple
    prec: int
    shifts: list = field(default_factory=lambda: [6, 6, 6, 6])
    status: int = 0


@dataclass
class DownW:
    w: torch.Tensor
    unscale: float
    bias: Optional[torch.Tensor]
    slope: float
    rate: int
    kt: int


@dataclass
class BlockW:
    C: int
    kind: str
    rate: Optional[int]
    conv1: ConvW
    conv2: ConvW
    conv3: ConvW
    rate_conv: Optional[ConvW] = None
    fused: Optional[FusedW] = None
    down: Optional[DownW] = None


def fuse_blocks_enabled():
    import os

    return os.environ.get("OUHIP_FUSE_BLOCKS", "1") != "0"


ENDS_C = (32, 48)


def fuse_ends_enabled():
    import os

    return os.environ.get("OUHIP_FUSE_ENDS", "1") != "0"


def prep_fused(specs, C, prec, device):
    if not (fuse_blocks_enabled() and L.load().ou_block_supported(C, prec)):
        return None
    parts, offs, uns, off = [], [], [], 0
    for sp in specs:
        w = sp.w
        if w.shape[0] % 32:
            w = np.concatenate([w, np.zeros((-w.shape[0] % 32,) + w.shape[1:], w.dtype)])
        packed, un = L.block_pack_f32_np(w) if prec == 0 else L.block_pack_np(w)
        parts.append(packed)
        offs.append(off)
        uns.append(un)
        off += packed.nbytes
    w = torch.from_numpy(np.concatenate(parts)).to(device)
    fw = FusedW(w, tuple(offs), tuple(uns), prec)
    if prec:
        fw.status = _range_slot(fw) or _PREP_STATUS
    return fw


def fuse_down_enabled():
    import os

    return os.environ.get("OUHIP_FUSE_DOWN", "1") != "0"


def prep_down_fused(spec, C, prec, bias, device):
    m, cr, kt = spec.w.shape
    r = spec.frame
    if not (fuse_down_enabled() and m == 2 * C and cr == C * r
            and L.load().ou_block_down_supported(C, r, kt, prec)):
        return None
    w4 = np.ascontiguousarray(spec.w.reshape(m, C, r, kt).transpose(0, 1, 3, 2).reshape(m, C, kt * r))
    packed, un = L.block_pack_np(w4)
    return DownW(torch.from_numpy(packed).to(device), un, bias, float(spec.slope), r, kt)


def prep_block(sd, p, kind, rate, antialias, device):
    specs = [spec_same(sd, p + ".conv1", 5), spec_same(sd, p + ".conv2", 3), spec_same(sd, p + ".conv3", 3)]
    c1, c2, c3 = (make_conv(sp, device) for sp in specs)
    rc, rc_spec = None, None
    if kind == "down":
        rc_spec = spec_down(sd, p + ".rate_change_conv", rate, antialias)
        rc = make_conv(rc_spec, device)
    elif kind == "up":
        rc = prep_up(sd, p + ".rate_change_conv", rate, antialias, device)
    fused = prep_fused(specs, c1.m, c1.prec, device) if c1.prec in (1, 2) else None
    down = prep_down_fused(rc_spec, c1.m, c1.prec, rc.bias, device) if (fused and rc_spec) else None
    return BlockW(c1.m, kind, rate, c1, c2, c3, rc, fused, down)


@dataclass
class GruW:
    hidden: int
    layers: List


def prep_gru(sd, p, num_layers, device):
    layers = []
    for l in range(num_layers):
        s, sr = f"_l{l}", f"_l{l}_reverse"
        w_ih = np.concatenate([_np(sd[p + ".weight_ih" + s]), _np(sd[p + ".weight_ih" + sr])], 0)
        b_ih = np.concatenate([_np(sd[p + ".bias_ih" + s]), _np(sd[p + ".bias_ih" + sr])], 0)
        proj = make_conv(ConvSpec(w_ih[:, :, None], w_ih.shape[1], 1, 0, 1, 1.0, b_ih,
                                  ref_macs=float(w_ih.size)), device)
        w_hh = torch.stack([sd[p + ".weight_hh" + s], sd[p + ".weight_hh" + sr]]).detach().to(
            "cpu", torch.float32).contiguous()
        b_hh = torch.stack([sd[p + ".bias_hh" + s], sd[p + ".bias_hh" + sr]]).float().contiguous().to(device)
        layers.append((proj, w_hh.to(device), b_hh))
    H = int(sd[p + ".weight_hh_l0"].shape[1])
    return GruW(H, layers)


class Act:

    def __init__(self, t):
        assert t.dtype == torch.float32 and t.dim() == 3
        self.t = t
        self.ptr = t.data_ptr()
        self.bs, self.cs = t.stride(0), t.stride(1)
        self.B, self.C, self.T = t.shape


class ArenaFull(Exception):
    pass


class Arena:

    def __init__(self, device, nbytes):
        self.buf = torch.empty(int(nbytes), dtype=torch.uint8, device=device)
        self.off = 0

    @property
    def nbytes(self):
        return self.buf.numel()

    def take(self, shape, dtype):
        n = math.prod(shape) * torch.empty((), dtype=dtype).element_size()
        off = (self.off + 255) // 256 * 256
        if off + n > self.buf.numel():
            raise ArenaFull(off + n)
        self.off = off + n
        return self.buf[off:off + n].view(dtype).view(shape)


_ARENA = None


def empty(shape, dtype=torch.float32, device=None):
    return _ARENA.take(tuple(shape), dtype) if _ARENA is not None else torch.empty(shape, dtype=dtype, device=device)


def zeros(shape, dtype=torch.float32, device=None):
    return empty(shape, dtype, device).zero_()


def new_act(B, C, T, device):
    return Act(empty((B, C, T), dtype=torch.float32, device=device))


def conv_desc(cw: ConvW, x: Act, y: Act, *, in_len=None, n_frames=None, out_len=None,
              valid_len=None, in_scale=0, res1: Act = None, s1=1.0, film=0, film_bs=0,
              res2: Act = None, s2=1.0, batch=None):
    d = L.ConvDesc()
    d.x, d.x_bstride, d.x_cstride = x.ptr, x.bs, x.cs
    d.cin, d.in_len = cw.cin, x.T if in_len is None else in_len
    d.frame, d.shift = cw.frame, cw.shift
    d.in_scale, d.slope = in_scale or 0, cw.slope
    d.w, d.m, d.kt, d.pad, d.cc = cw.w.data_ptr(), cw.m, cw.kt, cw.pad, cw.cc
    d.prec, d.w_unscale, d.status = cw.prec, cw.w_unscale, cw.status
    d.xs_shift = cw.xshift
    d._w_nat = (cw.w_nat.data_ptr(), cw.w_unscale_nat) if cw.w_nat is not None else None
    d._cw = cw
    d._fir = cw.fir
    d.ks_ws, d.ks_ws_bytes = cw.ks_ws
    if (_LANE or _SLOT) and d.ks_ws:
        d.ks_ws += (_SLOT * MAX_LANES + _LANE) * d.ks_ws_bytes
    if n_frames is None:
        n_frames = -(-d.in_len // cw.frame) if cw.rout == 1 else x.T
    d.n_frames = n_frames
    d.f0 = 0
    d.batch = x.B if batch is None else batch
    d.y, d.y_bstride, d.y_cstride = y.ptr, y.bs, y.cs
    d.rout = -cw.rout if (cw.cm and cw.rout > 1) else cw.rout
    d.out_len = y.T if out_len is None else out_len
    d.valid_len = (1 << 30) if valid_len is None else valid_len
    d.bias = cw.bias.data_ptr() if cw.bias is not None else 0
    if res1 is not None:
        d.res1, d.r1_bstride, d.r1_cstride, d.s1 = res1.ptr, res1.bs, res1.cs, s1
    d.film, d.film_bstride = film or 0, film_bs
    if res2 is not None:
        d.res2, d.r2_bstride, d.r2_cstride, d.s2 = res2.ptr, res2.bs, res2.cs, s2
    d.tile = -1
    d._flops = 2.0 * cw.ref_macs * n_frames * d.batch
    assert d.n_frames > 0
    act = cw.cin * d.in_len + cw.cout * d.out_len * (1 + (res1 is not None) + (res2 is not None))
    d._bytes = 4.0 * (act * d.batch + cw.m * cw.cin * cw.frame * cw.kt)
    assert x.C == cw.cin, ("conv input channels", x.C, cw.cin)
    assert y.C == cw.cout, ("conv output channels", y.C, cw.cout)
    assert 0 < d.in_len <= x.T, ("conv in_len", d.in_len, x.T)
    assert 0 < d.out_len <= y.T, ("conv out_len", d.out_len, y.T)
    assert d.batch <= min(x.B, y.B)
    for r in (res1, res2):
        if r is not None:
            assert r.C == cw.cout and r.T >= d.out_len and r.B >= d.batch, ("residual", r.t.shape)
    return d


def rec_block(prog, bw: BlockW, h: Act, out: Act, tA: Act, tB: Act, film=0, film_bs=0,
              sc: Act = None, res2: Act = None, s2=1.0, cond_out: Act = None, skip_tail=False,
              x_in=None, head=None, e_out: Act = None, after_c1=None):
    c1_out = cond_out if cond_out is not None else tA
    d1 = conv_desc(bw.conv1, h, c1_out, res1=sc, s1=NF2, film=film, film_bs=film_bs)
    if skip_tail:
        add_conv(prog, d1)
        if after_c1 is not None:
            after_c1()
        return
    d2 = conv_desc(bw.conv2, c1_out, tB)
    d3 = conv_desc(bw.conv3, tB, out, res1=h, s1=NF2, res2=res2, s2=s2)
    d_rc = conv_desc(bw.rate_conv, out, e_out) if e_out is not None else None
    if bw.fused is not None and out.ptr != h.ptr:
        fuse_rc = d_rc is not None and bw.down is not None
        descs = (d1, d2, d3) + ((x_in[4],) if x_in is not None else ()) + ((d_rc,) if fuse_rc else ())
        bd = block_desc(bw, h, out, descs, sc=sc, film=film, film_bs=film_bs,
                        cond_out=cond_out, res2=res2, s2=s2,
                        x_in=x_in[:4] if x_in is not None else None, head=head,
                        e_out=e_out if fuse_rc else None)
        prog.add(L.OP_BLOCK, bd)
        if after_c1 is not None:
            after_c1()
        if d_rc is not None and not fuse_rc:
            add_conv(prog, d_rc)
        return
    assert x_in is None and head is None, "input / head fusion needs the fused block"
    add_conv(prog, d1)
    if after_c1 is not None:
        after_c1()
    add_conv(prog, d2)
    add_conv(prog, d3)
    if d_rc is not None:
        add_conv(prog, d_rc)


def fir_desc(d):
    fw = d._fir
    f = L.ConvDesc.from_buffer_copy(d)
    f.kt, f.pad, f.tile = 1, 0, -1
    f.w, f.w_unscale = fw.w.data_ptr(), fw.unscale
    f.fir, f.fir_taps = fw.mode, fw.taps.data_ptr()
    f._flops, f._bytes, f._cw, f._w_nat = d._flops, d._bytes, getattr(d, "_cw", None), None
    return f


def choose_fir(prog, d):
    mode = fir_mode()
    if getattr(d, "_fir", None) is None or mode == "0" or d.prec not in (1, 2) or d.f0 or d.xs:
        return d
    f = fir_desc(d)
    tuner = L.TUNER
    if mode == "1" or not hasattr(tuner, "pick"):
        return f
    _, ms_f = tuner.pick(f)
    _, ms_p = tuner.pick(d)
    folded = [ms_p]
    if L.ADD_HOOK is split_hook:
        link = _split_link(prog, L.OP_CONV, d)
        if link is not None:
            _, _, _, rows, batch, per_item, cons = link
            folded.append(_split_ms(d, per_item, rows, cons[6], batch))
    folded = [t for t in folded if t is not None]
    return f if ms_f is not None and (not folded or ms_f < min(folded)) else d


def add_conv(prog, d):
    prog.add(L.OP_CONV, choose_fir(prog, d))


def block_desc(bw: BlockW, h: Act, out: Act, descs, sc: Act = None, film=0, film_bs=0, cond_out: Act = None,
               res2: Act = None, s2=1.0, x_in=None, head=None, e_out: Act = None):
    fw = bw.fused
    d = L.BlockDesc()
    d.h, d.h_bstride, d.h_cstride = h.ptr, h.bs, h.cs
    d.channels, d.length, d.batch, d.prec = bw.C, h.T, h.B, fw.prec
    assert out.C == bw.C and out.T == h.T and out.B >= h.B, ("block output", out.t.shape, h.t.shape)
    for i, cw in enumerate((bw.conv1, bw.conv2, bw.conv3)):
        d.w[i] = fw.w.data_ptr() + fw.offs[i]
        d.bias[i] = cw.bias.data_ptr() if cw.bias is not None else 0
        d.slope[i] = cw.slope
        d.w_unscale[i] = fw.unscale[i]
    if sc is not None:
        assert sc.C == bw.C and sc.T >= h.T and sc.ptr != out.ptr
        d.sc, d.sc_bstride, d.sc_cstride, d.s_sc = sc.ptr, sc.bs, sc.cs, float(NF2)
    d.film, d.film_bstride = film or 0, film_bs
    if cond_out is not None:
        assert cond_out.C == bw.C and cond_out.T >= h.T and cond_out.ptr != out.ptr
        d.cond_out, d.co_bstride, d.co_cstride = cond_out.ptr, cond_out.bs, cond_out.cs
    d.y, d.y_bstride, d.y_cstride = out.ptr, out.bs, out.cs
    d.s_res, d.s2 = float(NF2), float(s2)
    if res2 is not None:
        assert res2.C == bw.C and res2.T >= h.T and res2.ptr != out.ptr
        d.res2, d.r2_bstride, d.r2_cstride = res2.ptr, res2.bs, res2.cs
    d.status = fw.status or bw.conv1.status or 0
    for i in range(4):
        d.shift[i] = fw.shifts[i]
    d._fw = fw
    if x_in is not None:
        xa, scale, w_in, b_in = x_in
        assert bw.C in ENDS_C and xa.C == 1 and xa.T == h.T and xa.B >= h.B
        d.x, d.x_bstride, d.in_scale = xa.ptr, xa.bs, scale or 0
        d.w_in, d.b_in = w_in.data_ptr(), b_in.data_ptr()
    if head is not None:
        assert bw.C in ENDS_C and head.length == h.T and head.channels == bw.C
        d.head = head
    if e_out is not None:
        dn = bw.down
        assert e_out.C == 2 * bw.C and e_out.T == -(-h.T // dn.rate) and e_out.B >= h.B, ("block e", e_out.t.shape)
        assert e_out.ptr not in (h.ptr, out.ptr)
        d.w_down, d.w_down_unscale = dn.w.data_ptr(), dn.unscale
        d.b_down = dn.bias.data_ptr() if dn.bias is not None else 0
        d.slope_down, d.rate, d.down_kt = dn.slope, dn.rate, dn.kt
        d.e, d.e_bstride, d.e_cstride = e_out.ptr, e_out.bs, e_out.cs
    d._flops = sum(x._flops for x in descs) + (head._flops if head is not None else 0.0)
    d._bytes = sum(x._bytes for x in descs)
    return d


GRU_FLAGS = int(os.environ.get("OUHIP_GRU_FLAGS", "-1"))
_GRU_WS_ZEROED = False


def rec_gru_ws_zero(prog, granules):
    prog.add(L.OP_MEMSET, L.MemsetArgs(ptr=granules.data_ptr(), bytes=granules.numel() * granules.element_size()))


def rec_gru(prog, gw: GruW, layer, x: Act, gi: Act, y: Act, granules, status, res: Act = None,
            res_scale=1.0, xcd=0):
    proj, w_hh, b_hh = gw.layers[layer]
    H = gw.hidden
    assert gi.C == 6 * H and gi.T == x.T and y.C == 2 * H and y.T == x.T and y.B == x.B
    if res is not None:
        assert res.C == 2 * H and res.T == x.T
    assert granules.numel() * 8 >= L.load().ou_gru_workspace_bytes(H, x.B)
    prog.add(L.OP_CONV, conv_desc(proj, x, gi))
    d = L.GruDesc()
    d.gi, d.gi_bstride = gi.ptr, gi.bs
    d.w_hh, d.b_hh = w_hh.data_ptr(), b_hh.data_ptr()
    d.y, d.y_bstride, d.y_cstride = y.ptr, y.bs, y.cs
    if res is not None:
        d.res, d.res_bstride, d.res_cstride, d.res_scale = res.ptr, res.bs, res.cs, res_scale
    d.hidden, d.steps, d.batch = gw.hidden, x.T, x.B
    d.granules, d.status = granules.data_ptr(), status.data_ptr()
    d.flags = GRU_FLAGS if not xcd else (GRU_FLAGS if GRU_FLAGS >= 0 else 0x8000) | ((xcd & 7) << 12)
    d.ws_zeroed = 1 if _GRU_WS_ZEROED else 0
    d._flops = 2.0 * 2 * 3 * H * H * x.T * x.B
    prog.add(L.OP_GRU, d)


def level_lengths(T, rates):
    Ts = [T]
    for r in rates:
        Ts.append(-(-Ts[-1] // r))
    return Ts


class ConvTuner:

    def __init__(self, reps=4, path=None):
        import json
        import os

        self.cache = {}
        self.times = {}
        self.reps = reps
        self.graph = os.environ.get("OUHIP_TUNE_GRAPH", "1") != "0"
        if self.graph:
            self.reps = max(reps, 8)
        self.path = path
        self.timed = 0
        self.by_geom = {}
        if path and os.path.exists(path):
            with open(path) as fh:
                raw = json.load(fh)
            times = raw.pop("__ms__", {})
            self.cache = {tuple(json.loads(k)): v for k, v in raw.items()}
            self.times = {tuple(json.loads(k)): v for k, v in times.items()}
        for kk in self.cache:
            self.by_geom.setdefault(kk[:-1], set()).add(kk[-1])

    def _save(self):
        import json

        if self.path:
            out = {json.dumps(list(k)): v for k, v in self.cache.items()}
            out["__ms__"] = {json.dumps(list(k)): v for k, v in self.times.items()}
            with open(self.path, "w") as fh:
                json.dump(out, fh)

    @staticmethod
    def bucket(n):
        return int(n).bit_length()

    @staticmethod
    def geometry(d):
        b = d.batch
        return (d.m, d.cin, d.frame, d.kt, d.pad, b, d.rout, bool(d.res1), bool(d.film), bool(d.res2),
                bool(d.in_scale), d.prec, bool(d.ks_ws), bool(d.xs), d.fir)

    @classmethod
    def key(cls, d):
        return cls.geometry(d) + (cls.bucket(d.n_frames),)

    @staticmethod
    def fit_workspace(d, tile):
        S = 1 << ((tile & L.TILE_KS_MASK) >> L.TILE_KS_SHIFT)
        if S > 1 and S * (d.n_frames + 256) * (d.m + 256) * d.batch * 4 > d.ks_ws_bytes:
            return tile & ~L.TILE_KS_MASK
        return tile

    def __call__(self, d):
        import ctypes
        import os

        k = self.key(d)
        if k in self.cache:
            return self.fit_workspace(d, self.cache[k])
        g, b = self.geometry(d), self.bucket(d.n_frames)
        near = self.by_geom.get(g)
        if near and os.environ.get("OUHIP_TUNE_EVERY_LENGTH", "0") != "1":
            bb = min(near, key=lambda x: (abs(x - b), x))
            self.cache[k] = self.cache[g + (bb,)]
            if g + (bb,) in self.times:
                self.times[k] = self.times[g + (bb,)] * 2.0 ** (b - bb)
            near.add(b)
            return self.fit_workspace(d, self.cache[k])
        lib = L.load()
        stream = torch.cuda.current_stream().cuda_stream
        best, best_ms = -1, float("inf")
        self.timed += 1
        small = -(-d.n_frames // 64) * -(-d.m // 64) * d.batch <= 1024
        ksl = tuple(k << L.TILE_KS_SHIFT for k in range(4)) if d.ks_ws and small else (0,)
        if d.fir:
            cands = [t | L.TILE_FIR for t in range(16) if lib.ou_conv_tile_ok(d.kt, t | L.TILE_FIR)]
            if d.fir == 2:
                cands += [t | L.TILE_FIR_EARLY for t in cands] + [t | L.TILE_FIR_DEEP for t in cands]
            elif d.fir == 1 and not (d.res1 or d.res2 or d.film):
                cands += [t | L.TILE_FIR_DEEP for t in cands]
        elif d.xs:
            cands = [t | L.TILE_SS for t in range(16) if lib.ou_conv_tile_ok(d.kt, t | L.TILE_SS)]
        elif d.prec in (1, 2):
            cands = [t | k for t in range(lib.ou_conv_num_tiles())
                     if lib.ou_conv_tile_ok(d.kt, t | L.TILE_SPLIT_QUERY) for k in ksl]
            if d.cin % 16 == 0:
                cands += [t | L.TILE_RS | k for t in range(16) if lib.ou_conv_tile_ok(d.kt, t | L.TILE_RS) for k in ksl]
        else:
            variants = (0, 1 << L.TILE_TPW_SHIFT, 2 << L.TILE_TPW_SHIFT, L.TILE_WS)
            cands = [t | v for t in range(lib.ou_conv_num_tiles()) for v in variants
                     if lib.ou_conv_tile_ok(d.kt, t | v)]
            cands += [t | k for t in range(lib.ou_conv_num_tiles()) if lib.ou_conv_tile_ok(d.kt, t)
                      for k in ksl[1:]]
        log = os.environ.get("OUHIP_TUNE_LOG")
        status, d.status = d.status, None
        hook, L.ADD_HOOK = L.ADD_HOOK, None
        try:
            best, best_ms = self._time(d, cands, lib, stream, log)
        finally:
            d.tile = -1
            d.status = status
            L.ADD_HOOK = hook
        self.cache[k] = best
        self.times[k] = best_ms
        self.by_geom.setdefault(k[:-1], set()).add(k[-1])
        if os.environ.get("OUHIP_TUNE_VERBOSE", "1") != "0":
            import sys

            print(f"[ou tune] m={d.m} cin={d.cin} frame={d.frame} kt={d.kt} n={d.n_frames} b={d.batch} "
                  f"rout={d.rout} prec={d.prec} fir={d.fir}: tile 0x{best:x} {best_ms * 1e3:.1f} us "
                  f"({len(cands)} candidates)", file=sys.stderr, flush=True)
        self._save()
        return best

    def _time(self, d, cands, lib, stream, log):
        import ctypes
        import os

        best, best_ms = -1, float("inf")
        for t in cands:
            d.tile = t
            if log:
                with open(log, "a") as fh:
                    fh.write(f"m={d.m} cin={d.cin} frame={d.frame} kt={d.kt} n={d.n_frames} b={d.batch} "
                             f"rout={d.rout} res1={bool(d.res1)} tile={t & L.TILE_SHAPE_MASK} "
                             f"tpw={1 << ((t & L.TILE_TPW_MASK) >> L.TILE_TPW_SHIFT)} "
                             f"ws={t // L.TILE_WS}\n")
                    fh.flush()
                    os.fsync(fh.fileno())
            if lib.ou_conv(ctypes.byref(d), ctypes.c_void_p(stream)) != 0:
                continue
            lib.ou_conv(ctypes.byref(d), ctypes.c_void_p(stream))
            if log:
                torch.cuda.synchronize()
            ms = float("inf")
            if self.graph:
                prog = L.Program()
                for _ in range(self.reps):
                    prog.add(L.OP_CONV, d)
                prog.capture()
                prog.launch(stream)
                for _ in range(2):
                    e0, e1 = torch.cuda.Event(enable_timing=True), torch.cuda.Event(enable_timing=True)
                    e0.record()
                    prog.launch(stream)
                    e1.record()
                    e1.synchronize()
                    ms = min(ms, e0.elapsed_time(e1) / self.reps)
                del prog
            else:
                for _ in range(2):
                    e0, e1 = torch.cuda.Event(enable_timing=True), torch.cuda.Event(enable_timing=True)
                    e0.record()
                    for _ in range(self.reps):
                        lib.ou_conv(ctypes.byref(d), ctypes.c_void_p(stream))
                    e1.record()
                    e1.synchronize()
                    ms = min(ms, e0.elapsed_time(e1) / self.reps)
            if ms < best_ms:
                best, best_ms = t, ms
        return best, best_ms


    def pick(self, d):
        tile = self(d)
        return tile, self.times.get(self.key(d))


_TUNER = None


def enable_autotune(flag=True):
    global _TUNER
    import os

    if flag and os.environ.get("OUHIP_AUTOTUNE", "1") != "0":
        if _TUNER is None:
            _TUNER = ConvTuner(path=os.environ.get("OUHIP_TUNE_CACHE") or None)
        L.TUNER = _TUNER
    else:
        L.TUNER = None


class Engine:
    def __init__(self, model_cfg, sd, device, parts=("score", "cond", "sdl"), _record_only=False,
                 conv_prec=None):
        global _PREP_PREC, _PREP_STATUS, _PREP_KSWS, _PREP_ENGINE
        self.device = torch.device(device)
        self.conv_prec = default_conv_prec() if conv_prec is None else int(conv_prec)
        if self.device.type != "cuda" and not _record_only:
            raise L.OuHipError("open_universe_amd runs on a HIP device (got %s)" % device)
        L.load()
        self.cfg = model_cfg
        self.scfg = model_cfg.get("score_model")
        self.ccfg = model_cfg.get("condition_model")
        self.edm = model_cfg.get("edm")
        self.level_db = (model_cfg.get("normalization_kwargs") or {}).get("level_db", 0.0)
        base = self.scfg if self.scfg is not None else self.ccfg
        self.rates = list(base["rate_factors"])
        self.nch = base["n_channels"]
        self.extra = base.get("extra_conv_block", False)
        if not self.extra:
            raise NotImplementedError("the HIP engine targets extra_conv_block=True configs")
        self.tot_ds = math.prod(self.rates)
        sp = "_edm_model" if self.edm is not None else "score_model"
        dev = self.device
        self.has_sdl = False
        self.status = torch.zeros(4 + RANGE_SLOTS, dtype=torch.int32, device=dev)
        self.range_owners = []
        self.ks_ws = torch.empty(MAX_SLOTS * MAX_LANES * KSWS_BYTES // 4, dtype=torch.float32, device=dev)
        saved = _PREP_PREC, _PREP_STATUS, _PREP_KSWS, _PREP_ENGINE
        _PREP_PREC, _PREP_STATUS, _PREP_ENGINE = self.conv_prec, self.status.data_ptr() + 4, self
        _PREP_KSWS = (self.ks_ws.data_ptr(), KSWS_BYTES)
        try:
            with torch.no_grad():
                if "score" in parts:
                    self._prep_score(sd, sp, dev)
                if "cond" in parts:
                    self._prep_cond(sd, "condition_model", dev)
                if "sdl" in parts:
                    self._prep_sdl(sd, "signal_decoupling_layer", dev)
        finally:
            _PREP_PREC, _PREP_STATUS, _PREP_KSWS, _PREP_ENGINE = saved
        enable_autotune(self.device.type == "cuda")

    def widen_ranges(self, flags, step=8, consumers=None):
        n = 0
        for slot, code in flags:
            if slot < 0 or slot >= len(self.range_owners):
                return 0
            own = self.range_owners[slot]
            w = step * (1 + bin((code >> 8) & 7).count("1"))
            targets = []
            if isinstance(own, FusedW):
                targets = [("f", own, i) for i, bit in enumerate((1, 2, 8, 16)) if code & bit]
            elif code & 1:
                targets.append(("c", own, 0))
            if code & (32 if isinstance(own, FusedW) else 2):
                cons = (consumers or {}).get(own.status)
                if cons is None:
                    return 0
                targets.append(cons)
            for kind, o, i in targets:
                if kind == "f":
                    o.shifts[i] += w
                    if o.shifts[i] > MAX_SHIFT:
                        return 0
                else:
                    o.xshift += w
                    if o.xshift > MAX_SHIFT:
                        return 0
                n += 1
        return n

    def _prep_score(self, sd, p, dev):
        cfg = self.scfg
        aa = cfg.get("use_antialiasing", False)
        rates = self.rates
        n_lvl = len(rates) + (1 if self.extra else 0)
        self.s_input = prep_plain(sd, p + ".input_conv", cfg.get("fb_kernel_size", 3), dev)
        w_in = fold_weight(sd, p + ".input_conv")
        b_in = _bias(sd, p + ".input_conv.bias")
        self.s_in_w = torch.from_numpy(np.ascontiguousarray(w_in.reshape(w_in.shape[0], -1), np.float32)).to(dev)
        self.s_in_b = torch.from_numpy(np.ascontiguousarray(
            b_in if b_in is not None else np.zeros(w_in.shape[0]), np.float32)).to(dev)
        self.s_in_fusable = w_in.shape[1] == 1 and w_in.shape[2] == 3
        self.s_enc = []
        for i in range(n_lvl):
            q = f"{p}.encoder.ds_modules.{i}"
            if i < len(rates):
                self.s_enc.append(prep_block(sd, q, "down", rates[i], aa, dev))
            else:
                self.s_enc.append(prep_block(sd, q, "none", None, aa, dev))
        self.s_gru = prep_gru(sd, p + ".encoder.gru", 1, dev)
        ups = rates[::-1]
        self.s_dec, self.s_sc = [], []
        for l in range(n_lvl):
            q = f"{p}.decoder.up_modules.{l}"
            if self.extra and l == 0:
                self.s_dec.append(prep_block(sd, q, "none", None, aa, dev))
            else:
                self.s_dec.append(prep_block(sd, q, "up", ups[l - (1 if self.extra else 0)], aa, dev))
            self.s_sc.append(prep_plain(sd, f"{p}.decoder.signal_cond_proj.{l}", 1, dev))
        ws, bs, self.film_off = [], [], []
        off = 0
        for name in [f"{p}.encoder.cond_proj.{i}" for i in range(n_lvl)] + \
                    [f"{p}.decoder.noise_cond_proj.{l}" for l in range(n_lvl)]:
            w = fold_weight(sd, name)
            ws.append(w)
            bs.append(_np(sd[name + ".bias"]))
            self.film_off.append(off)
            off += w.shape[0]
        self.film_rows = off
        self.emb_w = torch.from_numpy(np.concatenate(ws, 0)).to(dev).contiguous()
        self.emb_b = torch.from_numpy(np.concatenate(bs, 0)).to(dev).contiguous()
        self.emb_dim = self.emb_w.shape[1]
        te = cfg.get("time_embedding")
        self.emb_kind = 0 if te == "simple" else 1
        if self.emb_kind == 0:
            self.te_w = float(sd[p + ".sigma_block.weight"].reshape(-1)[0])
            self.te_b = float(sd[p + ".sigma_block.bias"].reshape(-1)[0])
        else:
            q = p + ".sigma_block"
            self.rff = sd[q + ".freq"].float().contiguous().to(dev)
            self.mlp = [(sd[f"{q}.layer{i}.lin.weight"].float().contiguous().to(dev),
                         sd[f"{q}.layer{i}.lin.bias"].float().contiguous().to(dev),
                         _slope(sd, f"{q}.layer{i}")) for i in (1, 2, 3)]
        self.head_s1 = float(sd[p + ".prelu.weight"].reshape(-1)[0])
        self.head_s2 = _slope(sd, p + ".output_conv")
        self.head_w = torch.from_numpy(fold_weight(sd, p + ".output_conv.conv").reshape(-1).copy()).to(dev)
        hb = sd.get(p + ".output_conv.conv.bias")
        self.head_b = 0.0 if hb is None else float(hb.reshape(-1)[0])
        assert fold_weight(sd, p + ".output_conv.conv").shape[0] == 1

    def _prep_cond(self, sd, p, dev):
        cfg = self.ccfg
        rates = list(cfg["rate_factors"])
        aa_dec = cfg.get("use_antialiasing", False)
        n_lvl = len(rates) + (1 if cfg.get("extra_conv_block", False) else 0)
        self.c_extra = cfg.get("extra_conv_block", False)
        self.c_gru_res = cfg.get("encoder_gru_residual", False)
        ds = math.prod(rates)
        n_fft = cfg.get("n_mel_oversample", 4) * ds
        self.mel_hop, self.mel_nfft = ds, n_fft
        self.mel_nmels = cfg.get("n_mels", 80)
        nfreq = n_fft // 2 + 1
        self.mel_nfreq = nfreq
        self.mel_pl = (n_fft - ds) // 2
        win = dsp.hann_periodic(n_fft).astype(np.float64)
        n = np.arange(n_fft)
        f = np.arange(nfreq)
        ang = 2.0 * math.pi * np.outer(f, n) / n_fft
        dft = np.concatenate([win * np.cos(ang), win * np.sin(ang)], 0)
        kt = n_fft // ds
        wl = dft.reshape(2 * nfreq, kt, ds).transpose(0, 2, 1)
        self.c_stft = make_conv(ConvSpec(wl, 1, ds, 0, 1, 1.0, None, shift=-self.mel_pl), dev, prec=0)
        fb = dsp.melscale_fbanks(nfreq, 0.0, float(24000 // 2), self.mel_nmels, 24000)
        self.c_fb = make_conv(ConvSpec(fb.T[:, :, None], nfreq, 1, 0, 1, 1.0, None), dev, prec=0)
        self.c_melconv = prep_plain(sd, p + ".input_mel.conv", 3, dev)
        self.c_melblock = prep_block(sd, p + ".input_mel.conv_block", "none", None, False, dev)
        self.c_input = prep_plain(sd, p + ".input_conv", cfg.get("fb_kernel_size", 3), dev)
        self.c_enc, self.c_st = [], []
        st_rates = [rates[-1]]
        for r in rates[-2::-1]:
            st_rates.append(st_rates[-1] * r)
        self.c_st_rates = st_rates[::-1]
        for i in range(n_lvl):
            q = f"{p}.encoder.ds_modules.{i}"
            if i < len(rates):
                self.c_enc.append(prep_block(sd, q, "down", rates[i], False, dev))
            else:
                self.c_enc.append(prep_block(sd, q, "none", None, False, dev))
            if i < len(rates) - 1:
                self.c_st.append(prep_strided(sd, f"{p}.encoder.st_convs.{i}", self.c_st_rates[i], dev))
        self.c_cb1 = prep_block(sd, p + ".encoder.conv_block1", "none", None, False, dev)
        self.c_cb2 = prep_block(sd, p + ".encoder.conv_block2", "none", None, False, dev)
        self.c_gru = prep_gru(sd, p + ".encoder.gru", 2, dev)
        self.c_dec_in = prep_block(sd, p + ".decoder.input_conv_block", "none", None, False, dev)
        ups = rates[::-1]
        self.c_dec = []
        for l in range(n_lvl):
            q = f"{p}.decoder.up_modules.{l}"
            if self.c_extra and l == 0:
                self.c_dec.append(prep_block(sd, q, "none", None, False, dev))
            else:
                self.c_dec.append(prep_block(sd, q, "up", ups[l - (1 if self.c_extra else 0)], aa_dec, dev))

    def _prep_sdl(self, sd, p, dev):
        self.has_sdl = (p + ".conv.weight") in sd
        if not self.has_sdl:
            return
        a = sd[p + ".prelu.act.act.alpha"].float()
        self.sdl_alpha = torch.exp(a).contiguous().to(dev)
        ku, wu = dsp.sinc_resample_kernel(1, 2)
        kd, wd = dsp.sinc_resample_kernel(2, 1)
        self.sdl_kup = torch.from_numpy(ku.reshape(-1).copy()).to(dev)
        self.sdl_kdown = torch.from_numpy(kd.reshape(-1).copy()).to(dev)
        self.sdl_taps = (ku.shape[1], wu, kd.shape[1], wd)
        self.sdl_w = sd[p + ".conv.weight"].float().reshape(-1).contiguous().to(dev)
        self.sdl_b = float(sd[p + ".conv.bias"].reshape(-1)[0])

    def alloc_score(self, B, T):
        dev = self.device
        Ts = level_lengths(T, self.rates)
        n_lvl = len(self.s_enc)
        Cs = [self.nch * 2 ** i for i in range(len(self.rates) + 1)]
        bufs = {"T": Ts, "C": Cs}
        for i in range(n_lvl):
            li = min(i, len(self.rates))
            for k in ("E", "A", "B", "V"):
                bufs[f"{k}{i}"] = new_act(B, Cs[li], Ts[li], dev)
        H = self.s_gru.hidden
        bufs["GI"] = new_act(B, 6 * H, Ts[len(self.rates)], dev)
        bufs["gran"] = zeros((L.load().ou_gru_workspace_bytes(H, B) // 8,), dtype=torch.int64, device=dev)
        return bufs

    def score_levels(self):
        n = len(self.s_enc)
        return [n - 1 - l for l in range(n)]

    def rec_score(self, prog, bufs, x: Act, film_base, film_bs, in_scale=0, sc_list=None, before_level=None,
                  head=None, after_encoder=None, gru_xcd=0):
        n_lvl = len(self.s_enc)
        nr = len(self.rates)
        fb = lambda j: film_base + 4 * self.film_off[j]
        prog.label = "score enc"
        d_in = conv_desc(self.s_input, x, bufs["E0"], in_scale=in_scale)
        fuse_in = (self.s_enc[0].fused is not None and self.s_enc[0].C in ENDS_C and self.s_in_fusable
                   and fuse_ends_enabled())
        if not fuse_in:
            prog.add(L.OP_CONV, d_in)
        for i in range(n_lvl):
            bw = self.s_enc[i]
            prog.label = f"score enc L{i}"
            x_in = (x, in_scale, self.s_in_w, self.s_in_b, d_in) if (i == 0 and fuse_in) else None
            rec_block(prog, bw, bufs[f"E{i}"], bufs[f"V{i}"], bufs[f"A{i}"], bufs[f"B{i}"],
                      film=fb(i), film_bs=film_bs, x_in=x_in,
                      e_out=bufs[f"E{i+1}"] if bw.kind == "down" else None)
        if after_encoder is not None:
            after_encoder()
        top = n_lvl - 1
        prog.label = "score gru"
        rec_gru(prog, self.s_gru, 0, bufs[f"V{top}"], bufs["GI"], bufs[f"V{top}"],
                bufs["gran"], self.status, res=bufs[f"V{top}"], res_scale=NF2, xcd=gru_xcd)
        h = None
        for l in range(n_lvl):
            i = top - l
            bw = self.s_dec[l]
            prog.label = f"score dec L{i}"
            if bw.kind == "up":
                li = min(i, nr)
                add_conv(prog, conv_desc(bw.rate_conv, h, bufs[f"V{i}"], n_frames=h.T,
                                         out_len=bufs["T"][li], valid_len=bw.rate * h.T,
                                         res1=bufs[f"V{i}"], s1=NF2))
            if before_level is not None:
                before_level(l)
            last = l == n_lvl - 1
            fuse_head = (last and head is not None and bw.fused is not None and bw.C in ENDS_C
                         and fuse_ends_enabled())
            rec_block(prog, bw, bufs[f"V{i}"], bufs[f"A{i}"], bufs[f"A{i}"], bufs[f"B{i}"],
                      film=fb(n_lvl + l), film_bs=film_bs, sc=sc_list[l], head=head if fuse_head else None)
            h = bufs[f"A{i}"]
            if last and head is not None:
                if not fuse_head:
                    head.h, head.h_bstride = h.ptr, h.bs
                    prog.add(L.OP_HEAD, head)
                return None
        return h

    def rec_sc(self, prog, conds, scs):
        for l, (c, s) in enumerate(zip(conds, scs)):
            prog.add(L.OP_CONV, conv_desc(self.s_sc[l], c, s))

    def alloc_sc(self, B, T):
        Ts = level_lengths(T, self.rates)
        n_lvl = len(self.s_enc)
        out = []
        for l in range(n_lvl):
            i = n_lvl - 1 - l
            li = min(i, len(self.rates))
            out.append(new_act(B, self.s_dec[l].C, Ts[li], self.device))
        return out

    def rec_embed(self, prog, sigma_dev, n, film_out, gbuf):
        d = L.EmbedDesc()
        d.sigma, d.n, d.kind, d.dim = sigma_dev.data_ptr(), n, self.emb_kind, self.emb_dim
        if self.emb_kind == 0:
            d.te_weight, d.te_bias = self.te_w, self.te_b
        else:
            d.rff_freq, d.n_rff = self.rff.data_ptr(), self.rff.numel()
            for k, (w, b, s) in enumerate(self.mlp):
                d.mlp_w[k], d.mlp_b[k], d.mlp_slope[k] = w.data_ptr(), b.data_ptr(), s
        d.rows = self.film_rows
        d.w, d.bias, d.out, d.gbuf = self.emb_w.data_ptr(), self.emb_b.data_ptr(), film_out.data_ptr(), gbuf.data_ptr()
        d._flops = 2.0 * self.film_rows * self.emb_dim * n
        prog.add(L.OP_EMBED, d)

    def head_desc(self, h: Optional[Act], out_ptr, B, T, mode=0, x_ptr=0, z_ptr=0, coef=None):
        d = L.HeadDesc()
        C = self.s_dec[-1].C
        if h is not None:
            d.h, d.h_bstride = h.ptr, h.bs
            C = h.C
        d.channels, d.length, d.batch, d.mode = C, T, B, mode
        d.slope1, d.slope2 = self.head_s1, self.head_s2
        d.w, d.bias = self.head_w.data_ptr(), self.head_b
        d.edm = 1 if self.edm is not None else 0
        if coef:
            for k, v in coef.items():
                setattr(d, k, float(v))
        d.x, d.z, d.out = x_ptr, z_ptr, out_ptr
        d._flops = 2.0 * C * 3 * T * B
        return d

    def alloc_cond(self, B, T, need_aux=False):
        dev = self.device
        rates = list(self.ccfg["rate_factors"])
        Ts = level_lengths(T, rates)
        Cs = [self.ccfg["n_channels"] * 2 ** i for i in range(len(rates) + 1)]
        U = -(-T // self.mel_hop)
        bufs = {"T": Ts, "C": Cs, "U": U}
        bufs["SPEC"] = new_act(B, 2 * self.mel_nfreq, U, dev)
        bufs["POW"] = new_act(B, self.mel_nfreq, U, dev)
        bufs["MEL"] = new_act(B, self.mel_nmels, U, dev)
        bufs["INV"] = empty((B,), dtype=torch.float32, device=dev)
        CL = Cs[-1]
        for k in ("M0", "MA", "MB", "XMEL", "SUM", "OUT", "LA", "LB", "CB1", "G1", "G2", "H", "D0", "Y4"):
            bufs[k] = new_act(B, CL, U, dev)
        n_lvl = len(self.c_enc)
        for i in range(len(rates)):
            for k in ("E", "A", "B", "V"):
                bufs[f"{k}{i}"] = new_act(B, Cs[i], Ts[i], dev)
        bufs[f"E{len(rates)}"] = new_act(B, CL, Ts[len(rates)], dev)
        H = self.c_gru.hidden
        bufs["GI"] = new_act(B, 6 * H, U, dev)
        bufs["gran"] = zeros((L.load().ou_gru_workspace_bytes(H, B) // 8,), dtype=torch.int64, device=dev)
        conds, ys = [], []
        for l in range(n_lvl):
            i = n_lvl - 1 - l
            li = min(i, len(rates))
            C = self.c_dec[l].C
            conds.append(new_act(B, C, Ts[li], dev))
            ys.append(new_act(B, C, Ts[li], dev))
        bufs["COND"] = conds
        bufs["Y"] = ys
        bufs["HUP"] = [new_act(B, self.c_dec[l].C, Ts[min(n_lvl - 1 - l, len(rates))], dev) for l in range(n_lvl)]
        bufs["TB"] = [new_act(B, self.c_dec[l].C, Ts[min(n_lvl - 1 - l, len(rates))], dev) for l in range(n_lvl)]
        return bufs

    def rec_cond(self, prog, bufs, x: Act, need_aux=False, after_level=None, st_lane=None):
        rates = list(self.ccfg["rate_factors"])
        nr = len(rates)
        n_lvl = len(self.c_enc)
        B, U = x.B, bufs["U"]
        mel_lane = 2 if st_lane is not None and nr >= 2 else None
        if mel_lane is not None and mel_lane not in (st_lane, 0):
            ev_m = prog.signal()
        if mel_lane is not None:
            side = _LANE
            set_lane(prog, mel_lane)
            if mel_lane not in (st_lane, 0):
                prog.wait(ev_m)
        prog.label = "cond mel"
        prog.add(L.OP_CONV, conv_desc(self.c_stft, x, bufs["SPEC"], n_frames=U))
        pa = L.PowerArgs(x=bufs["SPEC"].ptr, y=bufs["POW"].ptr, batch=B, nf=self.mel_nfreq, frames=U)
        prog.add(L.OP_POWER, pa)
        prog.add(L.OP_CONV, conv_desc(self.c_fb, bufs["POW"], bufs["MEL"]))
        ra = L.RmsArgs(x=bufs["MEL"].ptr, out=bufs["INV"].data_ptr(), batch=B,
                       n=self.mel_nmels * U, denom=float(U), eps=1e-5)
        prog.add(L.OP_INV_RMS, ra)
        prog.add(L.OP_CONV, conv_desc(self.c_melconv, bufs["MEL"], bufs["M0"], in_scale=bufs["INV"].data_ptr()))
        rec_block(prog, self.c_melblock, bufs["M0"], bufs["XMEL"], bufs["MA"], bufs["MB"])
        ev_mel = None
        if mel_lane is not None:
            if mel_lane not in (st_lane, 0):
                ev_mel = prog.signal()
            set_lane(prog, side)
        prog.label = "cond enc L0"
        prog.add(L.OP_CONV, conv_desc(self.c_input, x, bufs["E0"]))
        nsum = 0
        for i in range(n_lvl):
            bw = self.c_enc[i]
            prog.label = f"cond enc L{i}"
            if i < nr:
                rec_block(prog, bw, bufs[f"E{i}"], bufs[f"V{i}"], bufs[f"A{i}"], bufs[f"B{i}"],
                          e_out=bufs[f"E{i+1}"])
                if i < nr - 1:
                    last_st = i == nr - 2
                    if nr - 1 == 1:
                        res_a, res_b = bufs["XMEL"], None
                    elif nsum == 0:
                        res_a, res_b = None, None
                    else:
                        res_a, res_b = bufs["SUM"], (bufs["XMEL"] if last_st else None)
                    if st_lane is not None:
                        side = _LANE
                        ev = prog.signal()
                        set_lane(prog, st_lane)
                        prog.wait(ev)
                        if ev_mel is not None and (res_a is bufs["XMEL"] or res_b is not None):
                            prog.wait(ev_mel)
                    prog.label = f"cond st{i}"
                    dst = conv_desc(self.c_st[i], bufs[f"V{i}"], bufs["SUM"], n_frames=U, res1=res_a, s1=1.0,
                                    res2=res_b, s2=1.0)
                    dst._no_split = True
                    add_conv(prog, dst)
                    prog.label = f"cond enc L{i}"
                    if st_lane is not None:
                        set_lane(prog, side)
                    nsum += 1
            else:
                if st_lane is not None and nsum:
                    side = _LANE
                    set_lane(prog, st_lane)
                    ev = prog.signal()
                    set_lane(prog, side)
                    prog.wait(ev)
                n_out = nsum + 1
                nf = np.float32(1.0 / math.sqrt(n_out + 1))
                rec_block(prog, bw, bufs[f"E{i}"], bufs["OUT"], bufs["LA"], bufs["LB"],
                          res2=bufs["SUM"], s2=nf)
        if not self.c_extra:
            raise NotImplementedError("conditioner without extra_conv_block")
        prog.label = "cond cb1"
        rec_block(prog, self.c_cb1, bufs["OUT"], bufs["CB1"], bufs["LA"], bufs["LB"])
        prog.label = "cond gru1"
        rec_gru(prog, self.c_gru, 0, bufs["CB1"], bufs["GI"], bufs["G1"], bufs["gran"], self.status)
        res = bufs["CB1"] if self.c_gru_res else None
        prog.label = "cond gru2"
        rec_gru(prog, self.c_gru, 1, bufs["G1"], bufs["GI"], bufs["G2"], bufs["gran"], self.status,
                res=res, res_scale=NF2)
        prog.label = "cond cb2"
        rec_block(prog, self.c_cb2, bufs["G2"], bufs["H"], bufs["LA"], bufs["LB"])
        prog.label = "cond dec in"
        rec_block(prog, self.c_dec_in, bufs["H"], bufs["D0"], bufs["LA"], bufs["LB"])
        h = bufs["D0"]
        for l in range(n_lvl):
            bw = self.c_dec[l]
            i = n_lvl - 1 - l
            li = min(i, nr)
            prog.label = f"cond dec L{i}"
            if bw.kind == "up":
                hup = bufs["HUP"][l]
                prog.add(L.OP_CONV, conv_desc(bw.rate_conv, h, hup, n_frames=h.T,
                                              out_len=bufs["T"][li], valid_len=bw.rate * h.T))
                h = hup
            last = l == n_lvl - 1
            hook = (lambda l=l: after_level(l, bufs["COND"][l])) if after_level is not None else None
            rec_block(prog, bw, h, bufs["Y"][l], None, bufs["TB"][l], cond_out=bufs["COND"][l],
                      skip_tail=last and not need_aux, after_c1=hook)
            h = bufs["Y"][l]
        return bufs["COND"], bufs["Y"][-1]

    def rec_aux(self, prog, y: Act, tmp: Act, out_ptr, B, T):
        d = L.SnakeDesc()
        d.h, d.h_bstride = y.ptr, y.bs
        d.channels, d.length, d.batch = y.C, T, B
        tu, wu, td, wd = self.sdl_taps
        d.alpha, d.k_up, d.taps_up, d.width_up = self.sdl_alpha.data_ptr(), self.sdl_kup.data_ptr(), tu, wu
        d.k_down, d.taps_down, d.width_down, d.out = self.sdl_kdown.data_ptr(), td, wd, tmp.ptr
        prog.add(L.OP_SNAKE, d)
        h = L.HeadDesc()
        h.h, h.h_bstride, h.channels, h.length, h.batch, h.mode = tmp.ptr, tmp.bs, tmp.C, T, B, 0
        h.slope1 = h.slope2 = 1.0
        h.w, h.bias, h.out = self.sdl_w.data_ptr(), self.sdl_b, out_ptr
        prog.add(L.OP_HEAD, h)
```

### open_universe_amd/hazards.py

```python
from dataclasses import dataclass

from . import _lib as L


@dataclass(frozen=True)
class Box:
    base: int
    bs: int
    cs: int
    nb: int
    nc: int
    t0: int
    t1: int

    @property
    def lo(self):
        return self.base + self.t0

    @property
    def hi(self):
        return self.base + (self.nb - 1) * self.bs + (self.nc - 1) * self.cs + self.t1


def _box(ptr, bs, cs, nb, nc, t0, t1):
    ptr = ptr or 0
    if not ptr or nb <= 0 or nc <= 0 or t1 <= t0:
        return None
    return Box(int(ptr), int(bs), int(cs), int(nb), int(nc), int(t0), int(t1))


def _span(ptr, nbytes):
    return _box(ptr, 0, 0, 1, 1, 0, nbytes)


def overlap(a: Box, b: Box) -> bool:
    if a.hi <= b.lo or b.hi <= a.lo:
        return False
    if a.nb * a.nc > b.nb * b.nc:
        a, b = b, a
    if a.nb * a.nc > 1 << 16:
        return True
    n = a.t1 - a.t0
    for ia in range(a.nb):
        for ca in range(a.nc):
            s0 = a.base + ia * a.bs + ca * a.cs + a.t0
            if _span_hits(s0, s0 + n, b):
                return True
    return False


def _span_hits(s0, s1, b: Box) -> bool:
    if s1 <= b.lo or b.hi <= s0:
        return False
    for ib in range(b.nb):
        base = b.base + ib * b.bs
        if b.nc == 1 or b.cs == 0:
            if s0 < base + b.t1 and base + b.t0 < s1:
                return True
            continue
        c_lo = max(0, -(-(s0 - base - b.t1 + 1) // b.cs))
        c_hi = min(b.nc - 1, (s1 - 1 - base - b.t0) // b.cs)
        if c_lo <= c_hi:
            return True
    return False


def _conv(d):
    R, W = [], []
    cout = d.m // abs(d.rout)
    R.append(_box(d.x, 4 * d.x_bstride, 4 * d.x_cstride, d.batch, d.cin, 0, 4 * d.in_len))
    R.append(_span(d.in_scale, 4 * d.batch))
    r = abs(d.rout)
    a = d.f0 * r
    b = min((d.f0 + d.n_frames) * r, d.out_len)
    for p, bs, cs in ((d.res1, d.r1_bstride, d.r1_cstride), (d.res2, d.r2_bstride, d.r2_cstride)):
        R.append(_box(p, 4 * bs, 4 * cs, d.batch, cout, 4 * a, 4 * b))
    R.append(_span(d.film, 4 * ((d.batch - 1) * d.film_bstride + 2 * cout)))
    W.append(_box(d.y, 4 * d.y_bstride, 4 * d.y_cstride, d.batch, cout, 4 * a, 4 * b))
    if d.xs:
        R.append(_box(d.xs, d.xs_bstride, 0, d.batch, 1, 0, (d.cin // 32) * d.xs_rows * 128))
    if d.sy:
        W.append(_box(d.sy, d.sy_bstride, 0, d.batch, 1, 0, (d.m // 32) * d.sy_rows * 128))
    if d.tile >= 0 and d.tile & L.TILE_KS_MASK and not d.tile & L.TILE_SS:
        W.append(_span(d.ks_ws, d.ks_ws_bytes))
    return R, W


def _block(d):
    R, W = [], []
    C, T = d.channels, d.length
    f0, f1 = d.f0, d.f1 or T
    h0, h1 = d.h0, d.h1 or T
    if d.x:
        R.append(_box(d.x, 4 * d.x_bstride, 0, d.batch, 1, 0, 4 * T))
        R.append(_span(d.in_scale, 4 * d.batch))
    else:
        R.append(_box(d.h, 4 * d.h_bstride, 4 * d.h_cstride, d.batch, C, 4 * max(0, h0), 4 * min(T, h1)))
    lo, hi = max(0, f0 - 8), min(T, f1 + 8)
    R.append(_box(d.sc, 4 * d.sc_bstride, 4 * d.sc_cstride, d.batch, C, 4 * lo, 4 * hi))
    R.append(_span(d.film, 4 * ((d.batch - 1) * d.film_bstride + 2 * C)))
    R.append(_box(d.res2, 4 * d.r2_bstride, 4 * d.r2_cstride, d.batch, C, 4 * f0, 4 * f1))
    if d.xs:
        R.append(_box(d.xs, d.xs_bstride, 0, d.batch, 1, 0, (C // 32) * d.xs_rows * 128))
    W.append(_box(d.cond_out, 4 * d.co_bstride, 4 * d.co_cstride, d.batch, C, 4 * f0, 4 * f1))
    if d.head.w:
        hd = d.head
        for p in (hd.x, hd.z):
            R.append(_box(p, 4 * T, 0, d.batch, 1, 4 * f0, 4 * f1))
        W.append(_box(hd.out, 4 * T, 0, d.batch, 1, 4 * f0, 4 * f1))
    else:
        W.append(_box(d.y, 4 * d.y_bstride, 4 * d.y_cstride, d.batch, C, 4 * f0, 4 * f1))
    if d.e:
        r = max(1, d.rate)
        W.append(_box(d.e, 4 * d.e_bstride, 4 * d.e_cstride, d.batch, 2 * C, 4 * (f0 // r), 4 * (-(-f1 // r))))
    if d.sy:
        W.append(_box(d.sy, d.sy_bstride, 0, d.batch, 1, 0, (C // 32) * d.sy_rows * 128))
    return R, W


def _gru(d, lib):
    H, T = d.hidden, d.steps
    R = [_box(d.gi, 4 * d.gi_bstride, 0, d.batch, 1, 0, 4 * 6 * H * T),
         _box(d.res, 4 * d.res_bstride, 4 * d.res_cstride, d.batch, 2 * H, 0, 4 * T)]
    W = [_box(d.y, 4 * d.y_bstride, 4 * d.y_cstride, d.batch, 2 * H, 0, 4 * T),
         _span(d.granules, lib.ou_gru_workspace_bytes(H, d.batch)),
         _span(d.hstate, 4 * d.batch * 2 * H)]
    return R, W


def footprint(op, d, lib=None):
    lib = lib or L.load()
    if op == L.OP_CONV:
        R, W = _conv(d)
    elif op == L.OP_BLOCK:
        R, W = _block(d)
    elif op == L.OP_GRU:
        R, W = _gru(d, lib)
    elif op == L.OP_HEAD:
        R = [_box(d.h, 4 * d.h_bstride, 0, d.batch, 1, 0, 4 * d.channels * d.length),
             _box(d.x, 4 * d.length, 0, d.batch, 1, 0, 4 * d.length),
             _box(d.z, 4 * d.length, 0, d.batch, 1, 0, 4 * d.length)]
        W = [_box(d.out, 4 * d.length, 0, d.batch, 1, 0, 4 * d.length)]
    elif op == L.OP_EMBED:
        R = [_span(d.sigma, 4 * d.n)]
        W = [_span(d.out, 4 * d.n * d.rows), _span(d.gbuf, 4 * d.n * d.dim)]
    elif op == L.OP_MEMSET:
        R, W = [], [_span(d.ptr, d.bytes)]
    elif op == L.OP_NORMALIZE:
        R, W = [_span(d.x, 4 * d.batch * d.n)], [_span(d.y, 4 * d.batch * d.n)]
    elif op in (L.OP_RMS, L.OP_INV_RMS):
        R, W = [_span(d.x, 4 * d.batch * d.n)], [_span(d.out, 4 * d.batch)]
    elif op == L.OP_POWER:
        R = [_span(d.x, 4 * d.batch * 2 * d.nf * d.frames)]
        W = [_span(d.y, 4 * d.batch * d.nf * d.frames)]
    elif op == L.OP_PAD:
        R = [_box(d.x, 4 * d.x_bstride, 0, d.batch, 1, 0, 4 * d.n_in)]
        W = [_span(d.y, 4 * d.batch * d.n_out)]
    elif op == L.OP_SCALE:
        R, W = [_span(d.z, 4 * d.n), _span(d.add, 4 * d.n)], [_span(d.y, 4 * d.n)]
    elif op == L.OP_FINISH:
        R = [_box(d.x, 4 * d.x_bstride, 0, d.batch, 1, 0, 4 * (d.left + d.len)), _span(d.mix_rms, 4 * d.batch)]
        W = [_span(d.y, 4 * d.batch * d.len)]
    elif op == L.OP_ENSEMBLE:
        R = [_span(d.x, 4 * d.ensemble * d.n)]
        W = [_span(d.y, 4 * d.n), _span(d.counts, 4 * 32 * max(1, d.batch))]
    elif op == L.OP_SNAKE:
        R = [_box(d.h, 4 * d.h_bstride, 0, d.batch, 1, 0, 4 * d.channels * d.length)]
        W = [_span(d.out, 4 * d.batch * d.channels * d.length)]
    else:
        R, W = [], []
    return [b for b in R if b is not None], [b for b in W if b is not None]


def happens_before(prog):
    clocks = {}
    events = {}
    lane = 0
    out = []
    for op, d in zip(prog.op_kinds(), prog.descs):
        if op == L.OP_LANE:
            lane = d.id
            out.append(None)
            continue
        vc = clocks.setdefault(lane, {})
        if op == L.OP_SIGNAL:
            events[d.id] = dict(vc)
            out.append(None)
            continue
        if op == L.OP_WAIT:
            for k, v in events[d.id].items():
                if vc.get(k, 0) < v:
                    vc[k] = v
            out.append(None)
            continue
        vc[lane] = vc.get(lane, 0) + 1
        out.append((lane, vc[lane], dict(vc)))
    return out


def find_hazards(prog, limit=20):
    lib = L.load()
    hb = happens_before(prog)
    kinds = prog.op_kinds()
    fps = {}
    for i, (op, d) in enumerate(zip(kinds, prog.descs)):
        if hb[i] is not None:
            fps[i] = footprint(op, d, lib)
    found = []
    idx = sorted(fps)
    for jj, j in enumerate(idx):
        lane_j, _, vc_j = hb[j]
        Rj, Wj = fps[j]
        if not Rj and not Wj:
            continue
        for i in idx[:jj]:
            lane_i, k_i, _ = hb[i]
            if lane_i == lane_j or vc_j.get(lane_i, 0) >= k_i:
                continue
            Ri, Wi = fps[i]
            kind = None
            if any(overlap(a, b) for a in Wi for b in Wj):
                kind = "write-write"
            elif any(overlap(a, b) for a in Wi for b in Rj):
                kind = "write-read"
            elif any(overlap(a, b) for a in Ri for b in Wj):
                kind = "read-write"
            if kind:
                found.append((i, j, kind, prog.labels[i], prog.labels[j]))
                if len(found) >= limit:
                    return found
    return found


def live_ranges(*roots):
    import torch

    seen, out, stack = set(), [], list(roots)
    while stack:
        o = stack.pop()
        if id(o) in seen or o is None or isinstance(o, (int, float, str, bytes, bool)):
            continue
        seen.add(id(o))
        if isinstance(o, torch.Tensor):
            st = o.untyped_storage()
            if st.nbytes():
                out.append((st.data_ptr(), st.data_ptr() + st.nbytes()))
            continue
        if isinstance(o, dict):
            stack.extend(o.values())
        elif isinstance(o, (list, tuple, set)):
            stack.extend(o)
        elif hasattr(o, "__dict__") and not isinstance(o, type):
            stack.extend(vars(o).values())
    out.sort()
    return out


def dangling(prog, *roots, limit=20):
    import bisect

    lib = L.load()
    live = live_ranges(prog, *roots)
    starts = [a for a, _ in live]
    bad = []
    for i, (op, d) in enumerate(zip(prog.op_kinds(), prog.descs)):
        if op in (L.OP_LANE, L.OP_SIGNAL, L.OP_WAIT):
            continue
        R, W = footprint(op, d, lib)
        for b in R + W:
            k = bisect.bisect_right(starts, b.lo) - 1
            if k < 0 or not any(live[j][0] <= b.lo and b.hi <= live[j][1] for j in range(max(0, k - 4), k + 1)):
                bad.append((i, prog.labels[i], b))
                break
        if len(bad) >= limit:
            break
    return bad
```

Baseline: 804.5.

## Fuse decoder up-sampling transposed conv into preceding residual block kernel

Adds an up-sampling epilogue to the fused block kernel. It computes the next level's rate-change conv (phase-split MFMA GEMM plus optional FIR taps, bias, residual add and scale) straight from the block output held in LDS, and writes the up-sampled activation directly. This removes a separate conv launch and the round trip of storing and reloading the block output; the output store is also skipped when only the up-sampled tensor is needed. In exchange it uses more LDS per workgroup, raises the launch-bounds occupancy target, and adds new kernel template instances for the 128/rate-4 and 64/rate-2 cases.

```diff
diff --git a/include/ouhip.h b/include/ouhip.h
--- a/include/ouhip.h
+++ b/include/ouhip.h
@@ -8,7 +8,7 @@
 extern "C" {
 #endif
 
-#define OUHIP_ABI_VERSION 10
+#define OUHIP_ABI_VERSION 11
 
 int ou_abi_version(void);
 const char* ou_last_error(void);
@@ -246,6 +246,18 @@
     const uint16_t* xs;
     int64_t xs_bstride;
     int32_t xs_rows, xs_pad_;
+    const void* w_up;
+    const float* b_up;
+    const float* up_taps;
+    float slope_up, w_up_unscale;
+    int32_t up_rate, up_pad_;
+    float* u;
+    int64_t u_bstride, u_cstride;
+    int32_t u_len, u_valid;
+    const float* u_res;
+    int64_t ur_bstride, ur_cstride;
+    float s_u;
+    int32_t u_pad2_;
 } ou_block_desc;
 
 int ou_block_supported(int channels, int prec);
@@ -256,6 +268,7 @@
 int64_t ou_block_packed_f32(int channels, int kt);
 int ou_block_pack_f32(const float* w, int channels, int kt, float* out, float* w_unscale);
 int ou_block_down_supported(int channels, int rate, int kt, int prec);
+int ou_block_up_supported(int channels, int rate, int prec);
 int ou_block(const ou_block_desc* d, void* stream);
 
 typedef struct ou_program ou_program;
diff --git a/open_universe_amd/_lib.py b/open_universe_amd/_lib.py
--- a/open_universe_amd/_lib.py
+++ b/open_universe_amd/_lib.py
@@ -4,7 +4,7 @@
 
 _HERE = os.path.dirname(os.path.abspath(__file__))
 LIB_PATH = os.environ.get("OUHIP_LIB", os.path.join(_HERE, "libouhip.so"))
-ABI_VERSION = 10
+ABI_VERSION = 11
 
 fp = c_void_p
 
@@ -141,6 +141,10 @@
         ("sy", fp), ("sy_bstride", c_int64), ("sy_rows", c_int32), ("sy_shift", c_int32),
         ("sy_slope", c_float), ("sy_pad_", c_int32),
         ("xs", fp), ("xs_bstride", c_int64), ("xs_rows", c_int32), ("xs_pad_", c_int32),
+        ("w_up", fp), ("b_up", fp), ("up_taps", fp), ("slope_up", c_float), ("w_up_unscale", c_float),
+        ("up_rate", c_int32), ("up_pad_", c_int32),
+        ("u", fp), ("u_bstride", c_int64), ("u_cstride", c_int64), ("u_len", c_int32), ("u_valid", c_int32),
+        ("u_res", fp), ("ur_bstride", c_int64), ("ur_cstride", c_int64), ("s_u", c_float), ("u_pad2_", c_int32),
     ]
 
 
@@ -205,6 +209,7 @@
     "ou_block_pack_f32": (c_int, [POINTER(c_float), c_int, c_int, POINTER(c_float), POINTER(c_float)]),
     "ou_block_pack_rect": (c_int, [POINTER(c_float), c_int, c_int, c_int, c_void_p, POINTER(c_float)]),
     "ou_block_down_supported": (c_int, [c_int, c_int, c_int, c_int]),
+    "ou_block_up_supported": (c_int, [c_int, c_int, c_int]),
     "ou_block": (c_int, [POINTER(BlockDesc), c_void_p]),
     "ou_resample": (c_int, [fp, c_int64, fp, c_int64, c_int, c_int, c_int, fp, c_int, c_int, c_int, c_int,
                             c_void_p]),
diff --git a/open_universe_amd/csrc/ou_block.hip b/open_universe_amd/csrc/ou_block.hip
--- a/open_universe_amd/csrc/ou_block.hip
+++ b/open_universe_amd/csrc/ou_block.hip
@@ -236,11 +236,12 @@
 constexpr int kEpiFilm = 1, kEpiSc = 2, kEpiCond = 4, kEpiRes2 = 8;
 constexpr int kEpiIn = 16, kEpiHead = 32;
 constexpr int kEpiDown = 64;
+constexpr int kEpiUp = 128;
 
 template <int EPI, int R, int KF>
 constexpr int block_off()
 {
-    return (EPI & kEpiHead) ? 1 : (EPI & kEpiDown) ? R * ((KF - 1) / 2) : 0;
+    return (EPI & (kEpiHead | kEpiUp)) ? 1 : (EPI & kEpiDown) ? R * ((KF - 1) / 2) : 0;
 }
 
 template <int C, int NT, int P, int EPI, int R = 1, int KF = 1>
@@ -250,7 +251,24 @@
         constexpr int halo = 2 * R * ((KF - 1) / 2);
         return (BCfg<C, NT, P>::NF - 4 - halo) / R * R;
     }
-    return BCfg<C, NT, P>::NF - 4 - ((EPI & kEpiHead) ? 2 : 0);
+    return BCfg<C, NT, P>::NF - 4 - ((EPI & (kEpiHead | kEpiUp)) ? 2 : 0);
+}
+
+template <int C, int NT, int R>
+constexpr int up_yrs()
+{
+    return (32 * NT - 4) * R + 4;
+}
+
+template <int C, int NT, int P, int EPI, int R>
+constexpr int block_lds()
+{
+    using K = BCfg<C, NT, P>;
+    if constexpr (EPI & kEpiUp) {
+        constexpr int up = (int)sizeof(typename K::E) * K::B_OFF + (C / 2) * up_yrs<C, NT, R>() * 4;
+        return up > K::LDS_BYTES ? up : K::LDS_BYTES;
+    }
+    return K::LDS_BYTES;
 }
 
 typedef float float2_t __attribute__((ext_vector_type(2)));
@@ -326,22 +344,146 @@
     }
 }
 
+constexpr int kBlkSentinel = 0x7ffffff0;
+
+template <int C, int NT, int P, int R, int F, int SX>
+__device__ __forceinline__ void up_stage(const ou_block_desc& d, const _Float16* xa, int pstride, float* Y, int t0,
+                                         int TS, int b, int wave, int lane, int tid)
+{
+    constexpr int KS = C / 16, CO = C / 2, CPT = 32 / R, M4 = CO / CPT, N4 = NT;
+    constexpr int YRS = up_yrs<C, NT, R>();
+    constexpr int D = KS < 6 ? KS : 6;
+    static_assert(32 % R == 0 && CO % CPT == 0, "up stage: whole channels per m-tile");
+    const int l32 = lane & 31, h = lane >> 5;
+    const half8_t* wp = (const half8_t*)d.w_up;
+    const float un = d.w_up_unscale * ou_exp2i(d.shift[3] - kStageShift);
+
+    constexpr int NTAP = 2 * R + 1;
+    constexpr int NW = (4 + 2 * R + 3) / 4 * 4;
+    constexpr int NSG = (F * R + 3) / 4;
+    constexpr int NIT = CO * NSG;
+    constexpr int UEI = (NIT + 255) / 256;
+    static_assert(4 * (NSG - 1) + NW <= YRS && YRS % 4 == 0 && (F + 2) * R <= YRS,
+                  "up stage: FIR window inside the sample image");
+    const bool fir = d.up_taps != nullptr, has_r = d.u_res != nullptr;
+    const int vlen = d.u_valid;
+    const int tend = min(min(t0 + F, TS) * R, d.u_len);
+    const int ucs = (int)d.u_cstride, rcs = (int)d.ur_cstride;
+    const __amdgpu_buffer_rsrc_t us = ou_rsrc(d.u + (int64_t)b * d.u_bstride, (int64_t)CO * ucs * 4);
+    const __amdgpu_buffer_rsrc_t rs =
+        ou_rsrc(has_r ? d.u_res + (int64_t)b * d.ur_bstride : d.u, has_r ? (int64_t)CO * rcs * 4 : 0);
+    const bool v4 = ((t0 * R) & 3) == 0 && ((uintptr_t)d.u % 16) == 0 && d.u_bstride % 4 == 0 && ucs % 4 == 0 &&
+                    (!has_r || (((uintptr_t)d.u_res % 16) == 0 && d.ur_bstride % 4 == 0 && rcs % 4 == 0));
+
+    for (int tile = wave; tile < M4 * N4; tile += 4) {
+        const int m4 = tile % M4, n4 = tile / M4;
+        const int w = n4 * 32 + l32;
+        const _Float16* xb = xa + w * SX + 8 * h;
+        floatx16 acc, accx;
+#pragma unroll
+        for (int r = 0; r < 16; ++r) acc[r] = 0.f, accx[r] = 0.f;
+        half8_t ra[D][2];
+        auto load_a = [&](int s, half8_t (&dst)[2]) {
+            const half8_t* p = wp + (((int64_t)m4 * KS + s) * 2) * 64 + lane;
+            dst[0] = p[0];
+            if constexpr (P == 1) dst[1] = p[64];
+        };
+#pragma unroll
+        for (int s = 0; s < D - 1; ++s) load_a(s, ra[s]);
+#pragma unroll
+        for (int s = 0; s < KS; ++s) {
+            if (s + D - 1 < KS) load_a(s + D - 1, ra[(s + D - 1) % D]);
+            const _Float16* q = xb + 16 * s;
+            const half8_t bq = *(const half8_t*)q;
+            acc = __builtin_amdgcn_mfma_f32_32x32x16_f16(ra[s % D][0], bq, acc, 0, 0, 0);
+            if constexpr (P == 1) {
+                const half8_t bl = *(const half8_t*)(q + pstride);
+                accx = __builtin_amdgcn_mfma_f32_32x32x16_f16(ra[s % D][0], bl, accx, 0, 0, 0);
+                accx = __builtin_amdgcn_mfma_f32_32x32x16_f16(ra[s % D][1], bq, accx, 0, 0, 0);
+            }
+        }
+#pragma unroll
+        for (int r = 0; r < 16; ++r) {
+            const int ml = (r & 3) + 8 * (r >> 2) + 4 * h;
+            const int cl = ml / R, ph = ml - (ml / R) * R;
+            if (w < F + 2) Y[(m4 * CPT + cl) * YRS + w * R + ph] = __builtin_fmaf(accx[r], 1.f / 2048.f, acc[r]) * un;
+        }
+    }
+    float rv[UEI][4];
+#pragma unroll
+    for (int e = 0; e < UEI; ++e) {
+        const int it = min(tid + 256 * e, NIT - 1);
+        const int co = it / NSG, sig = 4 * (it - (it / NSG) * NSG);
+        const int s0 = t0 * R + sig;
+        if (v4 && sig + 3 < F * R && s0 + 3 < tend) {
+            const ou_u4_t a1 = __builtin_amdgcn_raw_buffer_load_b128(rs, (co * rcs + s0) * 4, 0, 0);
+#pragma unroll
+            for (int k = 0; k < 4; ++k) rv[e][k] = __uint_as_float(a1[k]);
+        } else {
+#pragma unroll
+            for (int k = 0; k < 4; ++k)
+                rv[e][k] = __uint_as_float(__builtin_amdgcn_raw_buffer_load_b32(
+                    rs, (sig + k < F * R && s0 + k < tend) ? (co * rcs + s0 + k) * 4 : kBlkSentinel, 0, 0));
+        }
+    }
+    __syncthreads();
+
+    float tap[NTAP];
+#pragma unroll
+    for (int j = 0; j < NTAP; ++j) tap[j] = fir ? d.up_taps[j] : 0.f;
+#pragma unroll
+    for (int e = 0; e < UEI; ++e) {
+        const int it = tid + 256 * e;
+        if (NIT % 256 != 0 && it >= NIT) break;
+        const int co = it / NSG, sig = 4 * (it - (it / NSG) * NSG);
+        const int s0 = t0 * R + sig;
+        float win[NW];
+        const float* yr = Y + co * YRS + sig;
+#pragma unroll
+        for (int k = 0; k < NW; k += 4) {
+            const f32x4_t q4 = *(const f32x4_t*)(yr + k);
+            win[k] = q4[0], win[k + 1] = q4[1], win[k + 2] = q4[2], win[k + 3] = q4[3];
+        }
+        const float bias = d.b_up ? d.b_up[co] : 0.f;
+        float o[4];
+#pragma unroll
+        for (int k = 0; k < 4; ++k) {
+            float f = 0.f;
+#pragma unroll
+            for (int j = 0; j < NTAP; ++j) f = __builtin_fmaf(tap[j], win[k + j], f);
+            if (!fir) f = win[k + R];
+            o[k] = s0 + k >= vlen ? 0.f : f + bias;
+        }
+#pragma unroll
+        for (int k = 0; k < 4; ++k) o[k] = (o[k] + rv[e][k]) * d.s_u;
+        if (v4 && sig + 3 < F * R && s0 + 3 < tend) {
+            __builtin_amdgcn_raw_buffer_store_b128(
+                ou_u4_t{__float_as_uint(o[0]), __float_as_uint(o[1]), __float_as_uint(o[2]), __float_as_uint(o[3])}, us,
+                (co * ucs + s0) * 4, 0, 0);
+            continue;
+        }
+#pragma unroll
+        for (int k = 0; k < 4; ++k)
+            __builtin_amdgcn_raw_buffer_store_b32(
+                __float_as_uint(o[k]), us,
+                (sig + k < F * R && s0 + k < tend) ? (co * ucs + s0 + k) * 4 : kBlkSentinel, 0, 0);
+    }
+}
+
 template <int C>
 constexpr int block_threads()
 {
     return C > 0 ? 256 : 0;
 }
 
-template <int C>
+template <int C, int EPI = 0>
 constexpr int block_min_wgs()
 {
-    return (C == 96 || C == 192) ? 1 : 2;
-}
-
-constexpr int kBlkSentinel = 0x7ffffff0;
+    return (C == 96 || C == 192) ? 1 : (EPI & kEpiUp) ? 3 : 2;
+}
 
 template <int C, int NT, int P, int EPI, int R = 1, int KF = 1>
-__global__ __launch_bounds__(block_threads<C>(), block_min_wgs<C>()) void block_kernel(ou_block_desc d)
+__global__ __launch_bounds__(block_threads<C>(), (block_min_wgs<C, EPI>())) void block_kernel(ou_block_desc d)
 {
     using K = BCfg<C, NT, P>;
     ou_kernarg_prefetch8();
@@ -727,9 +869,10 @@
                 ou_rsrc(d.sy ? (const char*)d.sy + (int64_t)b * d.sy_bstride : (const char*)yb,
                         d.sy ? (int64_t)(C / 32) * d.sy_rows * 128 : 0);
             const float sscale = ou_exp2i(-d.sy_shift);
-            const __amdgpu_buffer_rsrc_t yrs = ou_rsrc(yb, (int64_t)C * d.y_cstride * 4);
-            if constexpr (EPI & kEpiDown) __syncthreads();
-            const float ad = (EPI & kEpiDown) ? d.slope_down : 0.f;
+            const __amdgpu_buffer_rsrc_t yrs =
+                ou_rsrc(yb, ((EPI & kEpiUp) && !d.y) ? 0 : (int64_t)C * d.y_cstride * 4);
+            if constexpr (EPI & (kEpiDown | kEpiUp)) __syncthreads();
+            const float ad = (EPI & kEpiDown) ? d.slope_down : (EPI & kEpiUp) ? d.slope_up : 0.f;
 #pragma unroll
             for (int mr = 0; mr < MR; ++mr)
 #pragma unroll
@@ -767,8 +910,8 @@
                                             sscale, d.sy_slope, oms);
                         }
                     }
-                    if constexpr (EPI & kEpiDown) {
-                        constexpr int RH = R * (KF - 1 - (KF - 1) / 2);
+                    if constexpr (EPI & (kEpiDown | kEpiUp)) {
+                        constexpr int RH = (EPI & kEpiUp) ? 1 : R * (KF - 1 - (KF - 1) / 2);
                         const float keep = (t >= 0 && t < T && w < F + OFF + RH) ? kInD : 0.f;
 #pragma unroll
                         for (int j = 0; j < 4; ++j) {
@@ -791,13 +934,17 @@
                 __syncthreads();
                 down_stage<C, P, R, KF, F, SX>(d, xa, K::PA, t0, T, TS, b, wave, lane);
             }
+            if constexpr (EPI & kEpiUp) {
+                __syncthreads();
+                up_stage<C, NT, P, R, F, SX>(d, xa, K::PA, (float*)xbuf, t0, TS, b, wave, lane, tid);
+            }
         }
     }
     if constexpr (P != 0) {
         ou_range_flag(d.status, om0, 1, lane);
         ou_range_flag(d.status, om1, 2, lane);
         ou_range_flag(d.status, om2, 8, lane);
-        if constexpr ((EPI & kEpiDown) != 0) ou_range_flag(d.status, omd, 16, lane);
+        if constexpr ((EPI & (kEpiDown | kEpiUp)) != 0) ou_range_flag(d.status, omd, 16, lane);
         if (d.sy) ou_range_flag(d.status, oms, 32, lane);
     }
 }
@@ -806,20 +953,21 @@
 int launch(const ou_block_desc& d, hipStream_t s)
 {
     using K = BCfg<C, NT, P>;
+    constexpr int LDS = block_lds<C, NT, P, EPI, R>();
     static bool attr = false;
     if (!attr) {
         OU_HIP_CHECK(hipFuncSetAttribute((const void*)block_kernel<C, NT, P, EPI, R, KF>,
-                                         hipFuncAttributeMaxDynamicSharedMemorySize, K::LDS_BYTES),
+                                         hipFuncAttributeMaxDynamicSharedMemorySize, LDS),
                      "block: LDS attribute");
         attr = true;
     }
     constexpr int F = block_f<C, NT, P, EPI, R, KF>();
-    static_assert(F > 0 && F % R == 0, "block: frames per workgroup");
+    static_assert(F > 0 && (F % R == 0 || (EPI & kEpiUp)), "block: frames per workgroup");
     const int f1 = d.f1 > 0 ? min(d.f1, d.length) : d.length;
     if (d.f0 < 0 || d.f0 >= f1 || d.f0 % R || (R > 1 && f1 % R && f1 != d.length))
         return ou_fail(-1, "block: frame range [%d, %d) (rate %d, length %d)", d.f0, f1, R, d.length);
     dim3 grid((f1 - d.f0 + F - 1) / F, d.batch);
-    hipLaunchKernelGGL((block_kernel<C, NT, P, EPI, R, KF>), grid, dim3(K::NTH), K::LDS_BYTES, s, d);
+    hipLaunchKernelGGL((block_kernel<C, NT, P, EPI, R, KF>), grid, dim3(K::NTH), LDS, s, d);
     return ou_check_launch("block");
 }
 
@@ -840,12 +988,35 @@
     return ou_fail(-1, "block: no fused rate-change conv for %d channels, rate %d, kt %d", C, d.rate, d.down_kt);
 }
 
+constexpr bool up_ok(int C, int rate)
+{
+    return (C == 128 && rate == 4) || (C == 64 && rate == 2);
+}
+
+template <int C, int NT, int P, int EPI>
+int launch_up(const ou_block_desc& d, hipStream_t s)
+{
+    if constexpr (C == 128) {
+        if (d.up_rate == 4) return launch<C, NT, P, EPI, 4>(d, s);
+    } else if constexpr (C == 64) {
+        if (d.up_rate == 2) return launch<C, NT, P, EPI, 2>(d, s);
+    }
+    return ou_fail(-1, "block: no fused up-sampling conv for %d channels, rate %d", C, d.up_rate);
+}
+
 template <int C, int NT, int P>
 int launch_epi(const ou_block_desc& d, hipStream_t s)
 {
     const int epi = (d.film ? kEpiFilm : 0) | (d.sc ? kEpiSc : 0) | (d.cond_out ? kEpiCond : 0) |
                     (d.res2 ? kEpiRes2 : 0) | (d.x ? kEpiIn : 0) | (d.head.w ? kEpiHead : 0) |
-                    (d.w_down ? kEpiDown : 0);
+                    (d.w_down ? kEpiDown : 0) | (d.w_up ? kEpiUp : 0);
+    if constexpr ((C == 64 || C == 128) && P != 0) {
+        switch (epi) {
+        case kEpiUp: return launch_up<C, NT, P, kEpiUp>(d, s);
+        case kEpiFilm | kEpiUp: return launch_up<C, NT, P, kEpiFilm | kEpiUp>(d, s);
+        case kEpiFilm | kEpiSc | kEpiUp: return launch_up<C, NT, P, kEpiFilm | kEpiSc | kEpiUp>(d, s);
+        }
+    }
     if constexpr ((C == 32 || C == 64) && P != 0) {
         switch (epi) {
         case kEpiDown: return launch_down<C, NT, P, kEpiDown>(d, s);
@@ -906,6 +1077,11 @@
 extern "C" int ou_block_down_supported(int channels, int rate, int kt, int prec)
 {
     return prec != 0 && ou_block_supported(channels, prec) && down_ok(channels, rate, kt);
+}
+
+extern "C" int ou_block_up_supported(int channels, int rate, int prec)
+{
+    return (prec == 1 || prec == 2) && ou_block_supported(channels, prec) && up_ok(channels, rate);
 }
 
 extern "C" int ou_block_frames(int channels)
@@ -999,8 +1175,24 @@
 {
     if (!dp) return ou_fail(-1, "block: null descriptor");
     const ou_block_desc& d = *dp;
-    if (!d.h || !d.y || !d.w[0] || !d.w[1] || !d.w[2] || d.length <= 0 || d.batch <= 0 || d.batch > 65535)
+    if (!d.h || (!d.y && !d.w_up) || !d.w[0] || !d.w[1] || !d.w[2] || d.length <= 0 || d.batch <= 0 ||
+        d.batch > 65535)
         return ou_fail(-1, "block: invalid descriptor");
+    if (d.w_up) {
+        const int co = d.channels / 2;
+        if (!ou_block_up_supported(d.channels, d.up_rate, d.prec))
+            return ou_fail(-1, "block: no fused up-sampling conv for %d channels, rate %d, prec %d", d.channels,
+                           d.up_rate, d.prec);
+        if (!d.u || d.sy || d.head.w || d.w_down || d.f0 || d.f1 || d.h0 || d.h1 || d.u_len <= 0 ||
+            d.u_len > (int64_t)d.up_rate * d.length || d.u_cstride < d.u_len || (d.u_res && d.ur_cstride < d.u_len) ||
+            !(d.w_up_unscale > 0.f) || (int64_t)co * d.u_cstride * 4 >= kBlkSentinel ||
+            (d.u_res && (int64_t)co * d.ur_cstride * 4 >= kBlkSentinel))
+            return ou_fail(-1, "block: the up-sampling stage needs u, the whole signal, 0 < u_len <= rate * length "
+                               "<= row strides, and no sy / head / w_down");
+        const void* no[4] = {d.h, d.sc, d.y, d.res2};
+        for (const void* p : no)
+            if (p && p == (const void*)d.u) return ou_fail(-1, "block: u aliases h, sc, y or res2");
+    }
     if (!ou_block_supported(d.channels, d.prec))
         return ou_fail(-1, "block: channels %d / prec %d not supported", d.channels, d.prec);
     const int64_t lim = kBlkSentinel;
diff --git a/open_universe_amd/engine.py b/open_universe_amd/engine.py
--- a/open_universe_amd/engine.py
+++ b/open_universe_amd/engine.py
@@ -112,7 +112,7 @@
         if p.prec != 1 or p.rout != 1 or p.m % 32 or p.sy or p.f0:
             return None
         return (p.y, p.y_bstride, p.y_cstride, p.out_len, p.m, p.batch)
-    if (p.prec != 1 or p.head.w or p.sy or p.channels % 32 or p.f0 or p.f1):
+    if (p.prec != 1 or p.head.w or p.sy or p.channels % 32 or p.f0 or p.f1 or p.w_up):
         return None
     return (p.y, p.y_bstride, p.y_cstride, p.length, p.channels, p.batch)
 
@@ -450,6 +450,18 @@
     rate_conv: Optional[ConvW] = None
     fused: Optional[FusedW] = None
     down: Optional[DownW] = None
+    up: Optional["UpW"] = None
+
+
+@dataclass
+class UpW:
+    w: torch.Tensor
+    unscale: float
+    bias: Optional[torch.Tensor]
+    slope: float
+    rate: int
+    cin: int
+    taps: Optional[torch.Tensor]
 
 
 def fuse_blocks_enabled():
@@ -504,18 +516,48 @@
     return DownW(torch.from_numpy(packed).to(device), un, bias, float(spec.slope), r, kt)
 
 
+def fuse_up_enabled():
+    import os
+
+    return os.environ.get("OUHIP_FUSE_UP", "1") != "0"
+
+
+def prep_up_fused(spec, prec, bias, device):
+    r, cin = spec.rout, spec.cin
+    cout = spec.w.shape[0] // r
+    if not (fuse_up_enabled() and fuse_blocks_enabled() and spec.cm and spec.frame == 1 and 2 * cout == cin
+            and 32 % r == 0 and cout % (32 // r) == 0 and L.load().ou_block_up_supported(cin, r, prec)):
+        return None
+    if spec.fir is not None and spec.fir[0] == 2:
+        wu, taps = np.asarray(spec.fir[2]), np.ascontiguousarray(spec.fir[3], np.float32)
+    elif spec.w.shape[2] == 1:
+        P = 32 // r
+        m = np.arange(r * cout)
+        co, ph = m // r, m % r
+        wu = np.zeros((r * cout, cin), np.float64)
+        wu[32 * (co // P) + (co % P) * r + ph] = spec.w[:, :, 0]
+        taps = None
+    else:
+        return None
+    packed, un = L.block_pack_np(np.ascontiguousarray(wu, np.float32)[:, :, None])
+    return UpW(torch.from_numpy(packed).to(device), un, bias, float(spec.slope), r, cin,
+               None if taps is None else torch.from_numpy(taps).to(device))
+
+
 def prep_block(sd, p, kind, rate, antialias, device):
     specs = [spec_same(sd, p + ".conv1", 5), spec_same(sd, p + ".conv2", 3), spec_same(sd, p + ".conv3", 3)]
     c1, c2, c3 = (make_conv(sp, device) for sp in specs)
-    rc, rc_spec = None, None
+    rc, rc_spec, up = None, None, None
     if kind == "down":
         rc_spec = spec_down(sd, p + ".rate_change_conv", rate, antialias)
         rc = make_conv(rc_spec, device)
     elif kind == "up":
-        rc = prep_up(sd, p + ".rate_change_conv", rate, antialias, device)
+        up_spec = spec_up(sd, p + ".rate_change_conv", rate, antialias)
+        rc = make_conv(up_spec, device)
+        up = prep_up_fused(up_spec, rc.prec, rc.bias, device) if rc.prec in (1, 2) else None
     fused = prep_fused(specs, c1.m, c1.prec, device) if c1.prec in (1, 2) else None
     down = prep_down_fused(rc_spec, c1.m, c1.prec, rc.bias, device) if (fused and rc_spec) else None
-    return BlockW(c1.m, kind, rate, c1, c2, c3, rc, fused, down)
+    return BlockW(c1.m, kind, rate, c1, c2, c3, rc, fused, down, up)
 
 
 @dataclass
@@ -638,7 +680,7 @@
 
 def rec_block(prog, bw: BlockW, h: Act, out: Act, tA: Act, tB: Act, film=0, film_bs=0,
               sc: Act = None, res2: Act = None, s2=1.0, cond_out: Act = None, skip_tail=False,
-              x_in=None, head=None, e_out: Act = None, after_c1=None):
+              x_in=None, head=None, e_out: Act = None, after_c1=None, up=None, store_out=True):
     c1_out = cond_out if cond_out is not None else tA
     d1 = conv_desc(bw.conv1, h, c1_out, res1=sc, s1=NF2, film=film, film_bs=film_bs)
     if skip_tail:
@@ -652,16 +694,21 @@
     if bw.fused is not None and out.ptr != h.ptr:
         fuse_rc = d_rc is not None and bw.down is not None
         descs = (d1, d2, d3) + ((x_in[4],) if x_in is not None else ()) + ((d_rc,) if fuse_rc else ())
+        fuse_up = (up is not None and up[0] is not None and up[0].cin == bw.C and head is None and not fuse_rc
+                   and fuse_up_enabled())
+        if fuse_up:
+            descs = descs + (up[1],)
         bd = block_desc(bw, h, out, descs, sc=sc, film=film, film_bs=film_bs,
                         cond_out=cond_out, res2=res2, s2=s2,
                         x_in=x_in[:4] if x_in is not None else None, head=head,
-                        e_out=e_out if fuse_rc else None)
+                        e_out=e_out if fuse_rc else None, up=up if fuse_up else None,
+                        store_out=store_out or not fuse_up)
         prog.add(L.OP_BLOCK, bd)
         if after_c1 is not None:
             after_c1()
         if d_rc is not None and not fuse_rc:
             add_conv(prog, d_rc)
-        return
+        return fuse_up
     assert x_in is None and head is None, "input / head fusion needs the fused block"
     add_conv(prog, d1)
     if after_c1 is not None:
@@ -670,6 +717,7 @@
     add_conv(prog, d3)
     if d_rc is not None:
         add_conv(prog, d_rc)
+    return False
 
 
 def fir_desc(d):
@@ -707,7 +755,7 @@
 
 
 def block_desc(bw: BlockW, h: Act, out: Act, descs, sc: Act = None, film=0, film_bs=0, cond_out: Act = None,
-               res2: Act = None, s2=1.0, x_in=None, head=None, e_out: Act = None):
+               res2: Act = None, s2=1.0, x_in=None, head=None, e_out: Act = None, up=None, store_out=True):
     fw = bw.fused
     d = L.BlockDesc()
     d.h, d.h_bstride, d.h_cstride = h.ptr, h.bs, h.cs
@@ -750,6 +798,24 @@
         d.b_down = dn.bias.data_ptr() if dn.bias is not None else 0
         d.slope_down, d.rate, d.down_kt = dn.slope, dn.rate, dn.kt
         d.e, d.e_bstride, d.e_cstride = e_out.ptr, e_out.bs, e_out.cs
+    if up is not None:
+        uw, du = up
+        assert uw.cin == bw.C and du.x == out.ptr and du.in_len == h.T and du.n_frames == h.T and du.batch == h.B
+        assert du.m == uw.rate * (bw.C // 2) and 0 < du.out_len <= uw.rate * h.T and not du.res2 and not du.film
+        assert du.y not in (h.ptr, out.ptr) and du.y_cstride >= du.out_len
+        d.w_up, d.w_up_unscale = uw.w.data_ptr(), uw.unscale
+        d.b_up = uw.bias.data_ptr() if uw.bias is not None else 0
+        d.up_taps = uw.taps.data_ptr() if uw.taps is not None else 0
+        d.slope_up, d.up_rate = uw.slope, uw.rate
+        d.u, d.u_bstride, d.u_cstride = du.y, du.y_bstride, du.y_cstride
+        d.u_len, d.u_valid = du.out_len, min(du.valid_len, 1 << 30)
+        if du.res1:
+            assert du.r1_cstride >= du.out_len
+            d.u_res, d.ur_bstride, d.ur_cstride, d.s_u = du.res1, du.r1_bstride, du.r1_cstride, du.s1
+        else:
+            d.s_u = 1.0
+        if not store_out:
+            d.y, d.y_bstride, d.y_cstride = 0, 0, 0
     d._flops = sum(x._flops for x in descs) + (head._flops if head is not None else 0.0)
     d._bytes = sum(x._bytes for x in descs)
     return d
@@ -1220,11 +1286,12 @@
         rec_gru(prog, self.s_gru, 0, bufs[f"V{top}"], bufs["GI"], bufs[f"V{top}"],
                 bufs["gran"], self.status, res=bufs[f"V{top}"], res_scale=NF2, xcd=gru_xcd)
         h = None
+        up_fused = False
         for l in range(n_lvl):
             i = top - l
             bw = self.s_dec[l]
             prog.label = f"score dec L{i}"
-            if bw.kind == "up":
+            if bw.kind == "up" and not up_fused:
                 li = min(i, nr)
                 add_conv(prog, conv_desc(bw.rate_conv, h, bufs[f"V{i}"], n_frames=h.T,
                                          out_len=bufs["T"][li], valid_len=bw.rate * h.T,
@@ -1234,9 +1301,16 @@
             last = l == n_lvl - 1
             fuse_head = (last and head is not None and bw.fused is not None and bw.C in ENDS_C
                          and fuse_ends_enabled())
-            rec_block(prog, bw, bufs[f"V{i}"], bufs[f"A{i}"], bufs[f"A{i}"], bufs[f"B{i}"],
-                      film=fb(n_lvl + l), film_bs=film_bs, sc=sc_list[l], head=head if fuse_head else None)
             h = bufs[f"A{i}"]
+            nxt = self.s_dec[l + 1] if l + 1 < n_lvl else None
+            up = None
+            if nxt is not None and nxt.kind == "up" and nxt.up is not None:
+                v = bufs[f"V{i - 1}"]
+                up = (nxt.up, conv_desc(nxt.rate_conv, h, v, n_frames=h.T, out_len=bufs["T"][min(i - 1, nr)],
+                                        valid_len=nxt.rate * h.T, res1=v, s1=NF2))
+            up_fused = rec_block(prog, bw, bufs[f"V{i}"], h, h, bufs[f"B{i}"],
+                                 film=fb(n_lvl + l), film_bs=film_bs, sc=sc_list[l],
+                                 head=head if fuse_head else None, up=up, store_out=False)
             if last and head is not None:
                 if not fuse_head:
                     head.h, head.h_bstride = h.ptr, h.bs
diff --git a/open_universe_amd/hazards.py b/open_universe_amd/hazards.py
--- a/open_universe_amd/hazards.py
+++ b/open_universe_amd/hazards.py
@@ -115,6 +115,9 @@
         W.append(_box(d.e, 4 * d.e_bstride, 4 * d.e_cstride, d.batch, 2 * C, 4 * (f0 // r), 4 * (-(-f1 // r))))
     if d.sy:
         W.append(_box(d.sy, d.sy_bstride, 0, d.batch, 1, 0, (C // 32) * d.sy_rows * 128))
+    if d.w_up:
+        R.append(_box(d.u_res, 4 * d.ur_bstride, 4 * d.ur_cstride, d.batch, C // 2, 0, 4 * d.u_len))
+        W.append(_box(d.u, 4 * d.u_bstride, 4 * d.u_cstride, d.batch, C // 2, 0, 4 * d.u_len))
     return R, W
 
 
```

New measurement: 819.3 (median of 6 runs). 1.8% higher.
